# RishabhSri14/Human-Body-Reconstruction

Measured on NVIDIA B200. Metric: train_rays_per_sec, higher is better.
Workload: dtype bf16 MLP operands (f32 accumulate) / f32 encoder+compositor

## Files before the change

human_body_reconstruction_b200/_lib.py:

```python
from __future__ import annotations

import ctypes as C
import os
import subprocess
import sys
import threading

import torch

_HERE = os.path.dirname(os.path.abspath(__file__))
ROOT = os.path.dirname(_HERE)
CSRC = os.path.join(_HERE, "csrc")
SO_PATH = os.path.join(_HERE, "libhbr_b200.so")
INCLUDE = os.path.join(ROOT, "include")

NVCC_FLAGS = [
    "-gencode", "arch=compute_100a,code=sm_100a", "-O3", "-lineinfo", "-std=c++17",
    "--fmad=true",
    "-Xcompiler", "-fPIC", "-Xcompiler", "-O3", "-Xptxas", "-v",
]

HBR_MAX_LEVELS = 32
HBR_MAX_PEERS, HBR_PEER_MAX_CTAS, HBR_PEER_HANDLE_BYTES = 8, 128, 64
HBR_PEER_FLAG_BYTES = HBR_PEER_MAX_CTAS * HBR_MAX_PEERS * 4
# ... 48 lines not shown

def _build_locked(bdir: str, force: bool, verbose: bool) -> str:
    nvcc = os.environ.get("NVCC", "/usr/local/cuda/bin/nvcc")
    objs, procs = [], []
    for src in sources():
        obj = os.path.join(bdir, os.path.basename(src)[:-3] + ".o")
        objs.append(obj)
        if (not force) and os.path.exists(obj) and os.path.getmtime(obj) > max(os.path.getmtime(d) for d in _deps()):
            continue
        cmd = [nvcc, *NVCC_FLAGS, *os.environ.get("HBR_EXTRA_NVCC", "").split(), "-I", INCLUDE, "-c", src, "-o", obj]
        procs.append((src, subprocess.Popen(cmd, stdout=subprocess.PIPE, stderr=subprocess.STDOUT, text=True)))
    log = []
    for src, p in procs:
        out, _ = p.communicate()
        log.append(f"== {os.path.basename(src)}\n{out}")
        if p.returncode != 0:
            raise RuntimeError(f"nvcc failed for {src}:\n{out}")
    with open(os.path.join(bdir, "ptxas.log"), "a" if not force else "w") as f:
        f.write("\n".join(log))
    if verbose:
        print("\n".join(log))
    tmp_so = os.path.join(bdir, f"libhbr_b200.{os.getpid()}.so.tmp")
    cmd = [nvcc, "-shared", "-o", tmp_so, *objs, "-lcudart"]
    r = subprocess.run(cmd, stdout=subprocess.PIPE, stderr=subprocess.STDOUT, text=True)
    if r.returncode != 0:
        raise RuntimeError(f"link failed:\n{r.stdout}")
    os.replace(tmp_so, SO_PATH)
    return SO_PATH


def build_debug(force: bool = False) -> str:
    dbg = os.path.join(CSRC, "debug")
    srcs = sorted(os.path.join(dbg, f) for f in os.listdir(dbg) if f.endswith(".cu")) + [os.path.join(CSRC, "abi.cu")]
    deps = _deps() + [os.path.join(dbg, f) for f in os.listdir(dbg)]
    if not force and os.path.exists(DEBUG_SO_PATH) and os.path.getmtime(DEBUG_SO_PATH) > max(os.path.getmtime(d) for d in deps):
        return DEBUG_SO_PATH
    nvcc = os.environ.get("NVCC", "/usr/local/cuda/bin/nvcc")
    cmd = [nvcc, *[f for f in NVCC_FLAGS if f not in ("-Xptxas", "-v")], "-I", INCLUDE, "-shared", "-o", DEBUG_SO_PATH, *srcs,
           "-lcudart"]
    r = subprocess.run(cmd, stdout=subprocess.PIPE, stderr=subprocess.STDOUT, text=True)
    if r.returncode != 0:
        raise RuntimeError(f"nvcc failed for the debug library:\n{r.stdout}")
    return DEBUG_SO_PATH


_lib = None
_debug_lib = None
_lock = threading.Lock()

_i64, _i32, _f32, _vp = C.c_int64, C.c_int, C.c_float, C.c_void_p
_geom_p, _dims_p = C.POINTER(HashGeom), C.POINTER(MlpDims)

SIGNATURES = {
    "hbr_abi_version": ([], C.c_int),
    "hbr_last_error": ([], C.c_char_p),
    "hbr_mlp_param_count": ([_dims_p], _i64),
    "hbr_mlp_act_floats": ([], _i64),
    "hbr_hash_encode_fwd": ([_vp, _i32, _i64, _vp, _geom_p, _vp, _i64, _vp], C.c_int),
    "hbr_hash_encode_bwd": ([_vp, _i32, _i64, _vp, _i64, _geom_p, _vp, _i32, _i32, _vp], C.c_int),
    "hbr_hash_encode_dx": ([_vp, _i32, _i64, _vp, _geom_p, _vp, _i64, _vp, _vp], C.c_int),
    "hbr_hash_indices": ([_vp, _i32, _i64, _geom_p, _vp, _vp, _vp], C.c_int),
    "hbr_dir_encode": ([_vp, _i32, _i64, _i32, _i32, _vp, _vp], C.c_int),
    "hbr_mlp_fwd_f32": ([_vp, _i64, _vp, _i64, _i64, _vp, _dims_p, _vp, _vp, _vp], C.c_int),
    "hbr_mlp_bwd_f32": ([_vp, _i64, _vp, _i64, _i64, _vp, _dims_p, _vp, _vp, _vp, _vp, _i64, _vp, _vp, _vp], C.c_int),
    "hbr_mlp_tc_scratch_bytes": ([_dims_p], _i64),
    "hbr_mlp_fwd_tc": ([_vp, _i32, _i64, _vp, _i64, _i64, _vp, _dims_p, _i32, _vp, _vp, _i32, _vp, _vp, _vp], C.c_int),
    "hbr_mlp_bwd_tc": ([_vp, _i32, _i64, _vp, _i64, _i64, _vp, _dims_p, _i32, _vp, _vp, _vp, _i64, _vp, _vp, _f32, _vp, _i32, _i32,
                        _vp, _vp, _vp], C.c_int),
    "hbr_occupancy_update": ([_vp, _i64, _vp, _i64, _vp, _i32, C.POINTER(C.c_float), _f32, _vp, _vp], C.c_int),
    "hbr_compact_samples": ([_vp, _vp, _vp, _i64, _i64, _i64, _vp, _i32, C.POINTER(C.c_float), _f32, _vp, _vp, _vp, _vp, _vp],
                            C.c_int),
    "hbr_hash_encode_fwd_pts": ([_vp, _i64, _vp, _vp, _geom_p, _vp, _i64, _i32, _vp], C.c_int),
    "hbr_hash_encode_bwd_pts": ([_vp, _i64, _vp, _vp, _i64, _geom_p, _vp, _i32, _i32, _vp], C.c_int),
    "hbr_mlp_tc_prepare": ([_vp, _dims_p, _i32, _vp, _vp], C.c_int),
    "hbr_mlp_tc_reduce_grads": ([_dims_p, _i64, _vp, _vp, _vp], C.c_int),
    "hbr_strat_depths": ([_vp, _vp, _f32, _f32, _i64, _vp, _vp], C.c_int),
    "hbr_mse_pair_fwd": ([_vp, _vp, _vp, _i64, _f32, _vp, _vp], C.c_int),
    "hbr_mse_pair_bwd": ([_vp, _vp, _vp, _i64, _f32, _vp, _vp, _vp, _vp], C.c_int),
    "hbr_hash_encode_fwd_rays": ([_vp, _vp, _vp, _i64, _i64, _i64, _vp, _geom_p, _vp, _i64, _i32, _vp], C.c_int),
    "hbr_field_bwd_rays_tc": ([_vp, _vp, _vp, _vp, _i64, _i64, _i64, _geom_p, _vp, _vp, _dims_p, _i32, _vp, _vp, _vp, _vp, _vp, _f32,
                               _vp, _i32, _i32, _vp], C.c_int),
    "hbr_field_fwd_rays_tc": ([_vp, _vp, _vp, _i64, _i64, _i64, _vp, _geom_p, _vp, _vp, _dims_p, _i32, _vp, _vp, _vp, _i32, _vp],
                              C.c_int),
    "hbr_hash_encode_bwd_rays": ([_vp, _vp, _vp, _i64, _i64, _i64, _vp, _i64, _geom_p, _vp, _i32, _i32, _vp], C.c_int),
    "hbr_field_fwd_tc": ([_vp, _i64, _vp, _geom_p, _vp, _i64, _vp, _dims_p, _i32, _vp, _vp, _vp, _vp], C.c_int),
    "hbr_field_bwd_tc": ([_vp, _i64, _geom_p, _vp, _i64, _vp, _dims_p, _i32, _vp, _vp, _vp, _vp, _vp, _vp, _f32, _vp, _vp],
                         C.c_int),
    "hbr_adam_step": ([_vp, _vp, _vp, _vp, _i64, C.c_double, C.c_double, C.c_double, C.c_double, C.c_double, _i32, _i64,
                       C.c_double, _vp, _vp], C.c_int),
    "hbr_adam_tick": ([_vp, _vp, _vp], C.c_int),
    "hbr_adam_step_dev": ([_vp, _vp, _vp, _vp, _i64, _vp, C.c_double, C.c_double, C.c_double, C.c_double, _i32, _vp, C.c_double,
                           _vp, _vp, _vp], C.c_int),
    "hbr_ray_gen": ([_vp, _i64, _i32, _i32, _f32, _f32, _f32, _f32, _vp, _i64, _i64, _vp, _i32, _vp, _vp, _vp, _vp, _vp, _vp],
                    C.c_int),
    "hbr_ray_bbox": ([_vp, _i64, _i32, _i32, _f32, _f32, _f32, _f32, _f32, _f32, _vp, _vp], C.c_int),
    "hbr_peer_alloc": ([C.POINTER(_vp), _i64], C.c_int),
    "hbr_peer_free": ([_vp], C.c_int),
    "hbr_peer_export": ([_vp, C.POINTER(C.c_ubyte)], C.c_int),
    "hbr_peer_import": ([C.POINTER(C.c_ubyte), C.POINTER(_vp)], C.c_int),
    "hbr_peer_release": ([_vp], C.c_int),
    "hbr_allreduce_peer": ([C.POINTER(_vp), C.POINTER(_vp), _vp, _i32, _i32, _i64, _f32, _i32, _vp, _vp], C.c_int),
    "hbr_hash_bwd_stream_tiles": ([_i64], _i64),
    "hbr_hash_encode_bwd_stream": ([_vp, _i32, _i64, _vp, _i64, _geom_p, _vp, C.POINTER(C.c_int), _i32, _vp, _vp], C.c_int),
    "hbr_hash_encode_bwd_rays_stream": ([_vp, _vp, _vp, _i64, _i64, _i64, _vp, _i64, _geom_p, _vp, C.POINTER(C.c_int), _i32, _vp,
                                         _vp], C.c_int),
    "hbr_hash_bwd_lm_ctas": ([_i64], _i64),
    "hbr_hash_encode_bwd_lm": ([_vp, _i32, _i64, _vp, _geom_p, _vp, C.POINTER(C.c_int), _i32, _vp, _vp], C.c_int),
    "hbr_hash_encode_bwd_rays_lm": ([_vp, _vp, _vp, _i64, _i64, _i64, _vp, _geom_p, _vp, C.POINTER(C.c_int), _i32, _vp, _vp],
                                    C.c_int),
    "hbr_allreduce_peer_stream": ([C.POINTER(_vp), C.POINTER(_vp), _vp, _i32, _i32, _i32, C.POINTER(_i64), C.POINTER(_i64),
                                   C.POINTER(C.c_uint), C.POINTER(C.c_int), _vp, _f32, _i32, _vp, _vp], C.c_int),
    "hbr_ray_points": ([_vp, _vp, _vp, _i64, _i64, _i64, _vp, _vp], C.c_int),
    "hbr_occupancy_mask": ([_vp, _i64, _vp, _i32, C.POINTER(C.c_float), _f32, _vp, _vp], C.c_int),
    "hbr_composite_fwd": ([_vp, _i64, _vp, _i64, _vp, _i64, _vp, _f32, _vp, _vp, _i64, _i64, _vp, _vp, _f32, _vp], C.c_int),
    "hbr_composite_bwd": ([_vp, _i64, _vp, _i64, _vp, _i64, _vp, _f32, _vp, _vp, _i64, _i64, _vp, _vp, _i64, _vp, _i64, _f32, _vp],
                          C.c_int),
    "hbr_composite_maps_fwd": ([_vp, _i64, _vp, _i64, _vp, _i64, _vp, _f32, _vp, _vp, _i64, _i64, _vp, _vp, _vp, _vp, _f32, _vp],
                               C.c_int),
    "hbr_composite_maps_bwd": ([_vp, _i64, _vp, _i64, _vp, _i64, _vp, _f32, _vp, _vp, _i64, _i64, _vp, _vp, _vp, _vp, _i64, _vp,
                                _i64, _f32, _vp], C.c_int),
    "hbr_hier_sample": ([_vp, _vp, _vp, _vp, _i64, _i64, _i32, _vp, _vp], C.c_int),
    "hbr_composite_sdf_fwd": ([_vp, _i64, _vp, _i64, _i32, _vp, _i64, _i64, _vp, _vp, _vp], C.c_int),
    "hbr_composite_sdf_bwd": ([_vp, _i64, _vp, _i64, _i32, _vp, _i64, _i64, _vp, _vp, _vp, _i64, _vp, _i64, _vp, _vp], C.c_int),
    "hbr_sdf_stencil_points": ([_vp, _i64, _f32, C.POINTER(C.c_float), C.POINTER(C.c_float), _vp, _vp], C.c_int),
    "hbr_sdf_eikonal_fwd": ([_vp, _i64, _f32, _vp, _vp, _vp], C.c_int),
    "hbr_sdf_eikonal_bwd": ([_vp, _i64, _f32, _vp, _vp, _vp], C.c_int),
    "hbr_grid_points": ([C.POINTER(C.c_double), C.POINTER(C.c_double), _i32, _i64, _i64, _vp, _vp], C.c_int),
    "hbr_grid_density": ([C.POINTER(C.c_double), C.POINTER(C.c_double), _i32, _i64, _i64, _vp, _geom_p, _vp, _dims_p,
                          _vp, _vp, _vp, _vp, _i64, _i32, _vp], C.c_int),
    "hbr_mlp_density_tf32x3": ([_vp, _i64, _vp, _dims_p, _vp, _vp], C.c_int),
    "hbr_mc_count": ([_vp, _i32, _i32, _i32, _f32, _i32, _i32, _vp, _vp], C.c_int),
    "hbr_mc_emit": ([_vp, _i32, _i32, _i32, _f32, _i32, _i32, _vp, _vp, _i64, _vp, _i64, _vp, _vp], C.c_int),
    "hbr_grid_interp": ([_vp, _i32, _i32, _i32, _i32, _vp, _i64, _vp, _vp], C.c_int),
}

DEBUG_SIGNATURES = {
    "hbr_debug_umma": ([_i32, _i32, _vp, _vp, _vp, _i32, _i32, _vp], C.c_int),
    "hbr_debug_umma_bench": ([_i32, _i32, _i32, _i32, _i32, _vp, _vp], C.c_int),
    "hbr_debug_umma_chain_bench": ([_i32, _i32, _i32, _vp, _vp], C.c_int),
    "hbr_debug_mlp_trace": ([_vp, _vp, _i64, _i64, _vp, _vp, _vp, _vp], C.c_int),
    "hbr_debug_mlp_trace_bwd": ([_vp, _vp, _i64, _i64, _vp, _vp, _vp, _vp, _vp, _vp, _vp, _vp], C.c_int),
}


KERNELS_PER_CALL = {
    "hbr_hash_encode_fwd": 1, "hbr_hash_encode_bwd": 1, "hbr_hash_encode_dx": 1, "hbr_hash_encode_fwd_rays": 1, "hbr_hash_encode_bwd_rays": 1, "hbr_hash_indices": 1, "hbr_dir_encode": 1,
    "hbr_mlp_fwd_f32": 1, "hbr_mlp_bwd_f32": 2, "hbr_mlp_fwd_tc": 2, "hbr_mlp_bwd_tc": 3, "hbr_field_fwd_tc": 2, "hbr_field_bwd_tc": 3, "hbr_field_bwd_rays_tc": 3, "hbr_field_fwd_rays_tc": 1, "hbr_adam_step": 1, "hbr_adam_tick": 1, "hbr_adam_step_dev": 1, "hbr_allreduce_peer": 1, "hbr_allreduce_peer_stream": 1, "hbr_hash_encode_bwd_stream": 1, "hbr_hash_encode_bwd_rays_stream": 1, "hbr_hash_encode_bwd_lm": 1, "hbr_hash_encode_bwd_rays_lm": 1, "hbr_ray_gen": 1, "hbr_ray_bbox": 1, "hbr_ray_points": 1, "hbr_occupancy_mask": 1, "hbr_occupancy_update": 2, "hbr_compact_samples": 1, "hbr_hash_encode_fwd_pts": 1, "hbr_hash_encode_bwd_pts": 1,
    "hbr_composite_fwd": 1, "hbr_composite_bwd": 1, "hbr_composite_maps_fwd": 1, "hbr_composite_maps_bwd": 1, "hbr_strat_depths": 1, "hbr_mse_pair_fwd": 1, "hbr_mse_pair_bwd": 1, "hbr_mlp_tc_prepare": 1, "hbr_mlp_tc_reduce_grads": 1, "hbr_hier_sample": 1, "hbr_grid_points": 1,
    "hbr_composite_sdf_fwd": 1, "hbr_composite_sdf_bwd": 1, "hbr_sdf_stencil_points": 1, "hbr_sdf_eikonal_fwd": 1, "hbr_sdf_eikonal_bwd": 1,
    "hbr_grid_density": 3, "hbr_mlp_density_tf32x3": 1, "hbr_mc_count": 1, "hbr_mc_emit": 2, "hbr_grid_interp": 1,
}


class _Stats:

    def __init__(self):
        self.launches = 0
        self.calls = {}
        self.timing = False
        self.events = []
        self.graph_events = []

    def reset(self):
        self.launches = 0
        self.calls = {}
        self.events = []
        self.graph_events = []

    def graph_times(self):
        out = {}
        for name, a, b in self.graph_events:
            out.setdefault(name, []).append(a.elapsed_time(b))
        return out

    def summary(self):
        acc = {}
        for name, a, b in self.events:
            c, s = acc.get(name, (0, 0.0))
            acc[name] = (c + 1, s + a.elapsed_time(b))
        return {k: (c, s / c) for k, (c, s) in acc.items()}


STATS = _Stats()


class _Counted:
    __slots__ = ("fn", "name", "k")

    def __init__(self, fn, name):
        self.fn, self.name, self.k = fn, name, KERNELS_PER_CALL.get(name, 0)

    def __call__(self, *a):
        st = STATS
        st.launches += self.k
        st.calls[self.name] = st.calls.get(self.name, 0) + 1
        if st.timing and self.k:
            ext = torch.cuda.is_current_stream_capturing()
            e0 = torch.cuda.Event(enable_timing=True, external=ext)
            e1 = torch.cuda.Event(enable_timing=True, external=ext)
            s = torch.cuda.current_stream()
            e0.record(s)
            rc = self.fn(*a)
            e1.record(s)
            (st.graph_events if ext else st.events).append((self.name, e0, e1))
            return rc
        return self.fn(*a)


class _Lib:
    pass


def lib():
    global _lib
    if _lib is not None:
        return _lib
    with _lock:
        if _lib is None:
            if _stale():
                if os.environ.get("HBR_NO_BUILD") == "1":
                    raise RuntimeError("libhbr_b200.so is missing/stale and HBR_NO_BUILD=1")
                build()
            l = C.CDLL(SO_PATH)
            wrapped = _Lib()
            for name, (args, res) in SIGNATURES.items():
                fn = getattr(l, name)
                fn.argtypes = args
                fn.restype = res
                setattr(wrapped, name, _Counted(fn, name) if name in KERNELS_PER_CALL else fn)
            if l.hbr_abi_version() != HBR_ABI_VERSION:
# ... 42 lines not shown
```

human_body_reconstruction_b200/csrc/composite.cu:

```cuda
#include "common.cuh"
#include <math_constants.h>

namespace hbr {

constexpr int kRaysPerCta = 8;

__global__ void ray_points_kernel(const float* __restrict__ o, const float* __restrict__ d, const float* __restrict__ t,
                                  long long t_rs, long long R, long long S, float* __restrict__ pts) {
  const long long i = (long long)blockIdx.x * blockDim.x + threadIdx.x;
  if (i >= R * S) return;
  const long long r = i / S, s = i - r * S;
  const float tt = __ldg(t + r * t_rs + s);
#pragma unroll
  for (int k = 0; k < 3; ++k) pts[i * 3 + k] = __fadd_rn(__ldg(o + r * 3 + k), __fmul_rn(__ldg(d + r * 3 + k), tt));
}

struct Mu3 { float v[3]; };
__global__ void occupancy_kernel(const float* __restrict__ pts, long long n, const uint8_t* __restrict__ grid, int G,
                                 Mu3 mu, float sigma, uint8_t* __restrict__ mask) {
  const long long i = (long long)blockIdx.x * blockDim.x + threadIdx.x;
  if (i >= n) return;
  long long q[3];
#pragma unroll
  for (int k = 0; k < 3; ++k) {
    const float u = __fmul_rn(__fdiv_rn(__fsub_rn(__ldg(pts + i * 3 + k), mu.v[k]), sigma), (float)G);
    long long c = __float2ll_rz(u);
    if (c < 0) c += G;
    c = c < 0 ? 0 : (c >= G ? G - 1 : c);
    q[k] = c;
  }
  mask[i] = grid[(q[0] * G + q[1]) * G + q[2]] ? 1 : 0;
}

template <typename XT>
__global__ void dir_encode_kernel(const XT* __restrict__ d, long long n, int dim, int nf, float* __restrict__ out) {
  const long long i = (long long)blockIdx.x * blockDim.x + threadIdx.x;
  const long long total = n * dim * nf;
  if (i >= total) return;
  const int k = (int)(i % nf);
  const long long rc = i / nf;
  float s, c;
  if (sizeof(XT) == 2) {
    const float x = __half2float(reinterpret_cast<const __half*>(d)[rc]);
    const float two_x = __half2float(__float2half_rn(2.f * x));
    const float a = __half2float(__float2half_rn(two_x * (float)k));
    s = __half2float(__float2half_rn(sinf(a)));
    c = __half2float(__float2half_rn(cosf(a)));
  } else {
    const float x = reinterpret_cast<const float*>(d)[rc];
    const float a = __fmul_rn(__fmul_rn(2.f, x), (float)k);
    s = sinf(a);
    c = cosf(a);
  }
  float* o = out + rc * (2 * nf);
  o[k] = s;
  o[nf + k] = c;
}

struct SampleIn {
  float delta, sig, p;
  bool keep;
};

__device__ __forceinline__ long long sample_row(const int32_t* __restrict__ rowmap, long long gs, int s, int S) {
  return rowmap == nullptr ? gs : (s < S ? (long long)__ldg(rowmap + gs) : -1);
}

__device__ __forceinline__ SampleIn load_sample(const float* __restrict__ tr, const float* __restrict__ sigma,
                                                long long sig_st, const uint8_t* __restrict__ mask, long long gs,
                                                int s, int S, float dnr, bool& live, long long row) {
  SampleIn q;
  live = s < S && row >= 0 && (mask == nullptr || mask[gs]);
  float delta = 0.f;
  if (s + 1 < S) delta = __fsub_rn(__ldg(tr + s + 1), __ldg(tr + s));
  q.delta = __fmul_rn(delta, dnr);
  const float raw = live ? __ldg(sigma + row * sig_st) : 0.f;
  q.keep = !(raw < -10.f);
  q.sig = q.keep ? raw : -10.f;
  q.p = s < S ? __fmul_rn(q.sig, q.delta) : 0.f;
  return q;
}

template <bool MAPS>
__global__ void __launch_bounds__(kRaysPerCta * 32)
composite_fwd_kernel(const float* __restrict__ t, long long t_rs, const float* __restrict__ rgb, long long rgb_st,
                     const float* __restrict__ sigma, long long sig_st, const float* __restrict__ dn, float dn_scalar,
                     const uint8_t* __restrict__ mask, const int32_t* __restrict__ rowmap, long long R, int S,
                     float* __restrict__ C, float* __restrict__ w_out, float ert_tau, float* __restrict__ depth,
                     float* __restrict__ opac) {
  const int lane = threadIdx.x & 31;
  const long long ray = (long long)blockIdx.x * kRaysPerCta + (threadIdx.x >> 5);
  if (ray >= R) return;
  const float* tr = t + ray * t_rs;
  const float dnr = dn ? __ldg(dn + ray) : dn_scalar;
  float carry = 0.f, c0 = 0.f, c1 = 0.f, c2 = 0.f, dsum = 0.f, asum = 0.f;
  for (int s0 = 0; s0 < S; s0 += 32) {
    const int s = s0 + lane;
    const long long gs = ray * S + s;
    bool live;
    const long long row = sample_row(rowmap, gs, s, S);
    const SampleIn q = load_sample(tr, sigma, sig_st, mask, gs, s, S, dnr, live, row);
    const float incl = carry + warp_incl_scan(q.p, lane);
    float prev = __shfl_up_sync(kFull, incl, 1);
    if (lane == 0) prev = carry;
    const float T = s == 0 ? 1.f : expf(-prev);
    const float alpha = 1.f - expf(-q.p);
    const float w = s < S ? __fmul_rn(T, alpha) : 0.f;
    if (s < S) {
      if (w_out) w_out[gs] = w;
      if (MAPS) {
        dsum += w * __ldg(tr + s);
        asum += w;
      }
      if (live) {
        const float* c = rgb + row * rgb_st;
        c0 += w * __ldg(c + 0);
        c1 += w * __ldg(c + 1);
        c2 += w * __ldg(c + 2);
      }
    }
    carry = __shfl_sync(kFull, incl, 31);
    if (carry > ert_tau) {
      if (w_out)
        for (int s2 = s0 + 32 + lane; s2 < S; s2 += 32) w_out[ray * S + s2] = 0.f;
      break;
    }
  }
  c0 = warp_sum(c0); c1 = warp_sum(c1); c2 = warp_sum(c2);
  if (lane == 0) { C[ray * 3 + 0] = c0; C[ray * 3 + 1] = c1; C[ray * 3 + 2] = c2; }
  if (MAPS) {
    dsum = warp_sum(dsum); asum = warp_sum(asum);
    if (lane == 0) {
      if (depth) depth[ray] = dsum;
      if (opac) opac[ray] = asum;
    }
  }
}

template <int NCH, bool MAPS>
__global__ void __launch_bounds__(kRaysPerCta * 32)
composite_bwd_kernel(const float* __restrict__ t, long long t_rs, const float* __restrict__ rgb, long long rgb_st,
                     const float* __restrict__ sigma, long long sig_st, const float* __restrict__ dn, float dn_scalar,
                     const uint8_t* __restrict__ mask, const int32_t* __restrict__ rowmap, long long R, int S,
                     const float* __restrict__ gC, float* __restrict__ drgb, long long drgb_st, float* __restrict__ dsig,
                     long long dsig_st, float ert_tau, const float* __restrict__ gD, const float* __restrict__ gA) {
  const int lane = threadIdx.x & 31;
  const long long ray = (long long)blockIdx.x * kRaysPerCta + (threadIdx.x >> 5);
  if (ray >= R) return;
  const float* tr = t + ray * t_rs;
  const float dnr = dn ? __ldg(dn + ray) : dn_scalar;
  float g0 = 0.f, g1 = 0.f, g2 = 0.f, gd = 0.f, ga = 0.f;
  if (!MAPS || gC) { g0 = __ldg(gC + ray * 3 + 0); g1 = __ldg(gC + ray * 3 + 1); g2 = __ldg(gC + ray * 3 + 2); }
  if (MAPS) {
    if (gD) gd = __ldg(gD + ray);
    if (gA) ga = __ldg(gA + ray);
  }
  const bool packed = drgb_st == 4 && dsig_st == 4 && dsig == drgb + 3;

  float Tk[NCH], ek[NCH], ck[NCH], dk[NCH];
  float carry = 0.f;
  bool done = false;
#pragma unroll
  for (int i = 0; i < NCH; ++i) {
    const int s = i * 32 + lane;
    Tk[i] = 0.f; ek[i] = 1.f; ck[i] = 0.f; dk[i] = 0.f;
    if (i * 32 < S && !done) {
      const long long gs = ray * S + s;
      bool live;
      const long long row = sample_row(rowmap, gs, s, S);
      const SampleIn q = load_sample(tr, sigma, sig_st, mask, gs, s, S, dnr, live, row);
      const float incl = carry + warp_incl_scan(q.p, lane);
      float prev = __shfl_up_sync(kFull, incl, 1);
      if (lane == 0) prev = carry;
      carry = __shfl_sync(kFull, incl, 31);
      if (s < S) {
        Tk[i] = s == 0 ? 1.f : expf(-prev);
        ek[i] = expf(-q.p);
        if (live) {
          const float* c = rgb + row * rgb_st;
          ck[i] = g0 * __ldg(c + 0) + g1 * __ldg(c + 1) + g2 * __ldg(c + 2);
          dk[i] = q.keep ? q.delta : 0.f;
        }
        if (MAPS) ck[i] = __fadd_rn(__fmaf_rn(gd, __ldg(tr + s), ck[i]), ga);
      }
      done = carry > ert_tau;
    }
  }
  float rcarry = 0.f;
#pragma unroll
  for (int i = NCH - 1; i >= 0; --i) {
    if (i * 32 < S) {
      const int s = i * 32 + lane;
      const long long gs = ray * S + s;
      const float w = Tk[i] * (1.f - ek[i]);
      const float wc = w * ck[i];
      const float rin = warp_rincl_scan(wc, lane);
      float after = __shfl_down_sync(kFull, rin, 1);
      if (lane == 31) after = 0.f;
      const float suffix = rcarry + after;
      rcarry += __shfl_sync(kFull, rin, 0);
      if (s < S) {
        const long long row = sample_row(rowmap, gs, s, S);
        const bool live = row >= 0 && (mask == nullptr || mask[gs]);
        const float dp = Tk[i] * ek[i] * ck[i] - suffix;
        const float ds = live ? dk[i] * dp : 0.f;
        const float r0 = live ? w * g0 : 0.f, r1 = live ? w * g1 : 0.f, r2 = live ? w * g2 : 0.f;
        if (row >= 0) {
          if (packed) {
            *reinterpret_cast<float4*>(drgb + row * 4) = make_float4(r0, r1, r2, ds);
          } else {
            float* o = drgb + row * drgb_st;
            o[0] = r0; o[1] = r1; o[2] = r2;
            dsig[row * dsig_st] = ds;
          }
        }
      }
    }
  }
}

constexpr int kHierWarps = 4;

__global__ void __launch_bounds__(kHierWarps * 32)
hier_sample_kernel(float* __restrict__ w, const float* __restrict__ t, const float* __restrict__ u,
                   const float* __restrict__ cand, long long R, int S, int P2, int clamp_in_place,
                   float* __restrict__ t_fine) {
  extern __shared__ float sm[];
  const int warp = threadIdx.x >> 5, lane = threadIdx.x & 31;
  float* cdf = sm + (size_t)warp * (S + P2);
  float* arr = cdf + S;
  const long long ray = (long long)blockIdx.x * kHierWarps + warp;
  if (ray >= R) return;
  float* wr = w + ray * S;
  float part = 0.f;
  for (int s = lane; s < S; s += 32) {
    float v = wr[s];
    if (v < 0.f) { v = 0.f; if (clamp_in_place) wr[s] = 0.f; }
    v = __fadd_rn(v, 1e-5f);
    cdf[s] = v;
    part += v;
  }
  const float total = warp_sum(part);
  __syncwarp();
  for (int s = lane; s < S; s += 32) cdf[s] = __fdiv_rn(cdf[s], total);
  __syncwarp();
  if (lane == 0) {
    float acc = 0.f;
    for (int s = 0; s < S; ++s) { acc = __fadd_rn(acc, cdf[s]); cdf[s] = acc; }
  }
  __syncwarp();
  for (int s = lane; s < P2; s += 32) {
    float v = CUDART_INF_F;
    if (s < S) {
      v = __ldg(t + s);
    } else if (s < 2 * S) {
      const float uu = __ldg(u + ray * S + (s - S));
      int lo = 0, hi = S;
      while (lo < hi) {
        const int mid = (lo + hi) >> 1;
        if (cdf[mid] <= uu) lo = mid + 1; else hi = mid;
      }
      v = __ldg(cand + min(lo, S - 1));
    }
    arr[s] = v;
  }
  __syncwarp();
  for (int k = 2; k <= P2; k <<= 1) {
    for (int j = k >> 1; j > 0; j >>= 1) {
      for (int i = lane; i < P2; i += 32) {
        const int ixj = i ^ j;
        if (ixj > i) {
          const float a = arr[i], b = arr[ixj];
          const bool asc = (i & k) == 0;
          if ((a > b) == asc) { arr[i] = b; arr[ixj] = a; }
        }
      }
      __syncwarp();
    }
  }
  for (int s = lane; s < 2 * S; s += 32) t_fine[ray * 2 * S + s] = arr[s];
}

}

using namespace hbr;

extern "C" int hbr_ray_points(const float* o, const float* d, const float* t, int64_t t_rs, int64_t R, int64_t S,
                              float* pts, void* stream) {
  HBR_REQUIRE(R >= 0 && S >= 0, "negative size");
// ... 126 lines not shown
```

human_body_reconstruction_b200/csrc/debug/mlp_tc_debug.cu:

```cuda
#define HBR_DEBUG_ENTRY 1
#include "../mlp_layout.cuh"
#include "../tc_common.cuh"
#include "hbr_debug.h"

#define HBR_OP tc::OpBf16
#define HBR_OPNS bf16
#include "../mlp_tc_impl.cuh"
#undef HBR_OP
#undef HBR_OPNS
#define HBR_OP tc::OpF16
#define HBR_OPNS f16
#include "../mlp_tc_impl.cuh"
#undef HBR_OP
#undef HBR_OPNS

using namespace hbr;
using namespace hbr::bf16;

extern "C" int hbr_debug_umma(int mode, int operand, const float* A, const float* B, float* D, int N, int K, void* stream) {
  HBR_REQUIRE(mode >= 0 && mode <= 2, "mode %d", mode);
  HBR_REQUIRE(operand == HBR_BF16 || operand == HBR_F16, "operand %d", operand);
  HBR_REQUIRE(N % 16 == 0 && N >= 16 && N <= 64 && K % 16 == 0 && K >= 16 && K <= 128, "N=%d K=%d", N, K);
  HBR_REQUIRE(mode != 2 || K == 128, "mode 2 needs K=128");
  auto kern = operand == HBR_F16 ? f16::umma_debug_kernel : bf16::umma_debug_kernel;
  HBR_CUDA(cudaFuncSetAttribute(kern, cudaFuncAttributeMaxDynamicSharedMemorySize, 65536));
  kern<<<1, 128, 65536, as_stream(stream)>>>(mode, A, B, D, N, K);
  HBR_LAUNCH_CHECK();
  return HBR_OK;
}

extern "C" int hbr_debug_umma_bench(int M, int N, int reps, int nacc, int mn_major, long long* cycles, void* stream) {
  HBR_REQUIRE((M == 64 || M == 128) && N >= 8 && N <= 256 && N % 8 == 0 && nacc >= 1 && nacc * N <= 512 && reps >= 1,
              "bad shape");
  HBR_CUDA(cudaFuncSetAttribute(umma_bench_kernel, cudaFuncAttributeMaxDynamicSharedMemorySize, 65536));
  umma_bench_kernel<<<1, 128, 65536, as_stream(stream)>>>(M, N, reps, nacc, mn_major, cycles);
  HBR_LAUNCH_CHECK();
  return HBR_OK;
}

extern "C" int hbr_debug_umma_chain_bench(int kind, int reps, int nacc, long long* cycles, void* stream) {
  HBR_REQUIRE(kind >= 0 && kind <= 3 && reps >= 1 && nacc >= 1 && nacc <= 6, "bad arguments");
  HBR_CUDA(cudaFuncSetAttribute(umma_chain_bench_kernel, cudaFuncAttributeMaxDynamicSharedMemorySize, 98304));
  umma_chain_bench_kernel<<<1, 128, 98304, as_stream(stream)>>>(kind, reps, nacc, cycles);
  HBR_LAUNCH_CHECK();
  return HBR_OK;
}

extern "C" int hbr_debug_mlp_trace_bwd(const float* feat, const float* dirs, int64_t dir_group, int64_t n,
                                       const float* params, const float* out, const float* dout, float* dfeat,
                                       float* dparams, void* scratch, long long* trace, void* stream) {
  using SC = Scratch<32, 48>;
  constexpr int smem = BwdSmem<32, 48, 2>::total;
  HBR_CUDA(cudaFuncSetAttribute(mlp_bwd_tc_kernel<32, 48, 2, true>, cudaFuncAttributeMaxDynamicSharedMemorySize, smem));
  const int grid = (int)min64(ceil_div(ceil_div(n, kTile), 2), sm_count());
  uint8_t* sc = static_cast<uint8_t*>(scratch);
  if (sc != nullptr) mlp_prep_kernel<32, 48><<<kPrepCtas, 256, 0, as_stream(stream)>>>(params, 32, 24, sc);
  mlp_bwd_tc_kernel<32, 48, 2, true><<<grid, 2 * kTile + 32, smem, as_stream(stream)>>>(
      feat, 32, dirs, dir_group, n, params, 32, 24, out, dout, dfeat, 32, nullptr, dparams, sc,
      sc != nullptr ? reinterpret_cast<float*>(sc + SC::off_grad) : nullptr, trace, EncArgs{}, HashGeom{}, 1.f, 0, nullptr, nullptr);
  HBR_LAUNCH_CHECK();
  return HBR_OK;
}

extern "C" int hbr_debug_mlp_trace(const float* feat, const float* dirs, int64_t dir_group, int64_t n, const float* params,
                                   float* out, long long* trace, void* stream) {
  constexpr int smem = FwdSmem<32, 48, 4>::total;
  HBR_CUDA(cudaFuncSetAttribute(mlp_fwd_tc_kernel<32, 48, 4, true>, cudaFuncAttributeMaxDynamicSharedMemorySize, smem));
  const int grid = (int)min64(ceil_div(ceil_div(n, kTile), 4), sm_count());
  mlp_fwd_tc_kernel<32, 48, 4, true><<<grid, 4 * kTile, smem, as_stream(stream)>>>(
      feat, 32, dirs, dir_group, n, params, 32, 24, out, nullptr, trace, EncArgs{}, HashGeom{}, 0, nullptr, nullptr);
  HBR_LAUNCH_CHECK();
  return HBR_OK;
}
```

human_body_reconstruction_b200/csrc/mlp_tc.cu:

```cuda
#include "mlp_layout.cuh"
#include "tc_common.cuh"

#define HBR_OP tc::OpBf16
#define HBR_OPNS bf16
#include "mlp_tc_impl.cuh"
#undef HBR_OP
#undef HBR_OPNS
#define HBR_OP tc::OpF16
#define HBR_OPNS f16
#include "mlp_tc_impl.cuh"
#undef HBR_OP
#undef HBR_OPNS

using namespace hbr;
using bf16::narrow_shape;
using bf16::Scratch;
using tc::EncArgs;

static int check_operand(int operand, float grad_scale) {
  HBR_REQUIRE(operand == HBR_BF16 || operand == HBR_F16, "operand format %d (HBR_BF16 or HBR_F16)", operand);
  HBR_REQUIRE(grad_scale > 0.f && grad_scale < 3.0e38f, "grad_scale %g", (double)grad_scale);
  return HBR_OK;
}
#define HBR_BY_OPERAND(...) (operand == HBR_F16 ? f16::__VA_ARGS__ : bf16::__VA_ARGS__)
// ... 112 lines not shown
    return f16::launch_fwd_tc<32, 48, 4, true>(nullptr, 32, dirs, dir_group, n, params, 32, dims->d_view, out,
                                               static_cast<uint8_t*>(scratch), e, to_device_geom(*geom), 0, 0, nullptr, nullptr, as_stream(stream));
  }
  EncArgs e{};
  e.x = x; e.table = table; e.feat16 = static_cast<uint16_t*>(feat16);
  return bf16::launch_fwd_tc<32, 48, 4, true>(nullptr, 32, dirs, dir_group, n, params, 32, dims->d_view, out,
                                              static_cast<uint8_t*>(scratch), e, to_device_geom(*geom), 0, 0, nullptr, nullptr, as_stream(stream));
}

extern "C" int hbr_field_bwd_tc(const float* x, int64_t n, const hbr_hash_geom* geom, const float* dirs, int64_t dir_group,
                                const float* params, const hbr_mlp_dims* dims, int operand, const void* feat16,
                                const float* out, const float* dout, float* dtable, float* ddirs, float* dparams,
                                float grad_scale, void* scratch, void* stream) {
  if (int rc = check_field(geom, dims)) return rc;
  if (int rc = check_operand(operand, grad_scale)) return rc;
  if (n == 0) return HBR_OK;
  HBR_REQUIRE(x && dirs && params && feat16 && out && dout && dtable, "NULL pointer");
  HBR_REQUIRE(dir_group >= 1, "dir_group");
  HBR_REQUIRE((uintptr_t)out % 16 == 0 && (uintptr_t)dout % 16 == 0 && (uintptr_t)dtable % 16 == 0 &&
                  (uintptr_t)feat16 % 16 == 0 && (uintptr_t)scratch % 256 == 0, "alignment");
  uint16_t* f16p = const_cast<uint16_t*>(static_cast<const uint16_t*>(feat16));
  if (operand == HBR_F16) {
    EncArgs e{};
    e.x = x; e.dtable = dtable; e.feat16 = f16p;
    return f16::launch_bwd_tc<32, 48, 2, true>(nullptr, 32, dirs, dir_group, n, params, 32, dims->d_view, out, dout, nullptr, 32,
                                               ddirs, dparams, static_cast<uint8_t*>(scratch), e, to_device_geom(*geom),
                                               grad_scale, 0, 0, 0, nullptr, nullptr, as_stream(stream));
  }
  EncArgs e{};
  e.x = x; e.dtable = dtable; e.feat16 = f16p;
  return bf16::launch_bwd_tc<32, 48, 2, true>(nullptr, 32, dirs, dir_group, n, params, 32, dims->d_view, out, dout, nullptr, 32,
                                              ddirs, dparams, static_cast<uint8_t*>(scratch), e, to_device_geom(*geom),
                                              grad_scale, 0, 0, 0, nullptr, nullptr, as_stream(stream));
}

#ifndef HBR_FWD_GATHER_WARPS
#define HBR_FWD_GATHER_WARPS 8
#endif
extern "C" int hbr_field_fwd_rays_tc(const float* rays_o, const float* rays_d, const float* t, int64_t t_ray_stride, int64_t R,
                                     int64_t S, const float* table, const hbr_hash_geom* geom, const float* dirs,
                                     const float* params, const hbr_mlp_dims* dims, int operand, float* out, void* feat16,
                                     void* scratch, int image_ready, void* stream) {
  if (int rc = check_field(geom, dims)) return rc;
  if (int rc = check_operand(operand, 1.f)) return rc;
  HBR_REQUIRE(R >= 0 && S >= 1 && R < (1LL << 40) / S, "R=%lld S=%lld", (long long)R, (long long)S);
  HBR_REQUIRE(t_ray_stride == 0 || t_ray_stride >= S, "t_ray_stride %lld", (long long)t_ray_stride);
  HBR_REQUIRE(!image_ready || scratch != nullptr, "image_ready without scratch");
  const int64_t n = R * S;
  if (n == 0) return HBR_OK;
  HBR_REQUIRE(rays_o && rays_d && t && table && dirs && params && out && feat16, "NULL pointer");
  HBR_REQUIRE((uintptr_t)out % 16 == 0 && (uintptr_t)table % 16 == 0 && (uintptr_t)feat16 % 16 == 0 &&
                  (uintptr_t)scratch % 256 == 0, "alignment");
  EncArgs e{};
  e.table = table; e.feat16 = static_cast<uint16_t*>(feat16);
  e.ro = rays_o; e.rd = rays_d; e.rt = t; e.S = S; e.t_stride = t_ray_stride;
  const uint8_t* image = image_ready ? static_cast<const uint8_t*>(scratch) : nullptr;
  return HBR_BY_OPERAND(launch_fwd_gather_tc<HBR_FWD_GATHER_WARPS>(dirs, S, n, params, dims->d_view, out, image, e,
                                                                     to_device_geom(*geom), as_stream(stream)));
}

extern "C" int hbr_field_bwd_rays_tc(const void* feat16, const float* rays_o, const float* rays_d, const float* t,
                                     int64_t t_ray_stride, int64_t R, int64_t S, const hbr_hash_geom* geom, const float* dirs,
                                     const float* params, const hbr_mlp_dims* dims, int operand, const float* out,
                                     const float* dout, float* dtable, float* ddirs, float* dparams, float grad_scale,
                                     void* scratch, int image_ready, int defer_reduce, void* stream) {
  if (int rc = check_field(geom, dims)) return rc;
  if (int rc = check_operand(operand, grad_scale)) return rc;
  HBR_REQUIRE(!defer_reduce || (scratch != nullptr && dparams != nullptr), "defer_reduce needs scratch and dparams");
  HBR_REQUIRE(R >= 0 && S >= 1 && R < (1LL << 40) / S, "R=%lld S=%lld", (long long)R, (long long)S);
  HBR_REQUIRE(t_ray_stride == 0 || t_ray_stride >= S, "t_ray_stride %lld", (long long)t_ray_stride);
  const int64_t n = R * S;
  if (n == 0) return HBR_OK;
  HBR_REQUIRE(feat16 && rays_o && rays_d && t && dirs && params && out && dout && dtable, "NULL pointer");
  HBR_REQUIRE((uintptr_t)out % 16 == 0 && (uintptr_t)dout % 16 == 0 && (uintptr_t)dtable % 16 == 0 &&
                  (uintptr_t)feat16 % 16 == 0 && (uintptr_t)scratch % 256 == 0, "alignment");
  EncArgs e{};
  e.dtable = dtable; e.ro = rays_o; e.rd = rays_d; e.rt = t; e.S = S; e.t_stride = t_ray_stride;
  const float* feat = static_cast<const float*>(feat16);
  return HBR_BY_OPERAND(launch_bwd_tc<32, 48, 1, false, 11>(feat, 32, dirs, S, n, params, 32, dims->d_view, out, dout, nullptr, 32,
                                                            ddirs, dparams, static_cast<uint8_t*>(scratch), e,
                                                            to_device_geom(*geom), grad_scale, 1, image_ready, defer_reduce,
                                                            nullptr, nullptr, as_stream(stream)));
}
```

human_body_reconstruction_b200/csrc/mlp_tc_impl.cuh:

```cuda
#ifndef HBR_OP
#error "define HBR_OP (tc::OpBf16 | tc::OpF16) and HBR_OPNS before including mlp_tc_impl.cuh"
#endif

#ifndef HBR_RING_SLOTS
#define HBR_RING_SLOTS 2
#endif

namespace hbr {
namespace HBR_OPNS {
using namespace tc;
using OP = HBR_OP;


constexpr int kTile = 128;
constexpr int kLBO128 = kTile * 16;

template <int K0P, int KCP>
struct WOfs {
  static constexpr int w0 = 0;
  static constexpr int w1 = w0 + 64 * K0P * 2;
  static constexpr int w2 = w1 + 64 * 64 * 2;
  static constexpr int w3 = w2 + 16 * 64 * 2;
  static constexpr int w4 = w3 + 64 * KCP * 2;
  static constexpr int w5 = w4 + 64 * 64 * 2;
  static constexpr int total = w5 + 16 * 64 * 2;
};

struct BOfs {
  __host__ __device__ static constexpr int ofs(int i) {
    return i == 0 ? 0 : i == 1 ? 2048 : i == 2 ? 4096 : i == 3 ? 4608 : i == 4 ? 6656 : 8704;
  }
  static constexpr int total = 9216;
};

template <int K0P, int KCP>
__device__ __forceinline__ void stage_weights_bf16(const float* __restrict__ params, const MlpLayout& m, uint8_t* wsm,
                                                   uint8_t* bias_sm, uint8_t* ones16, float* bias_f32 = nullptr,
                                                   bool skip_weights = false, int tid = -1, int nthr = 0) {
  if (tid < 0) { tid = threadIdx.x; nthr = blockDim.x; }
  const int JP[6] = {64, 64, 16, 64, 64, 16};
  const int KP[6] = {K0P, 64, 64, KCP, 64, 64};
  const int wofs[6] = {WOfs<K0P, KCP>::w0, WOfs<K0P, KCP>::w1, WOfs<K0P, KCP>::w2, WOfs<K0P, KCP>::w3,
                       WOfs<K0P, KCP>::w4, WOfs<K0P, KCP>::w5};
  if (!skip_weights) {
    constexpr int kChunks = WOfs<K0P, KCP>::total / 16;
    const int cbeg[7] = {0, wofs[1] / 16, wofs[2] / 16, wofs[3] / 16, wofs[4] / 16, wofs[5] / 16, kChunks};
#pragma unroll 3
    for (int c = tid; c < kChunks; c += nthr) {
      int i = 0;
#pragma unroll
      for (int t = 1; t < 6; ++t) i += c >= cbeg[t] ? 1 : 0;
      const int J = m.J[i], K = m.K[i];
      const int jp = (i == 2 || i == 5) ? 16 : 64;
      const int e = c - cbeg[i];
      const int cg = e / jp, j = e - cg * jp;
      const float* src = params + m.W[i] + j * K + cg * 8;
      float v[8];
#pragma unroll
      for (int q = 0; q < 8; ++q) v[q] = (j < J && cg * 8 + q < K) ? __ldg(src + q) : 0.f;
      store_chunk<OP>(wsm + wofs[i], j, cg, jp, v);
    }
  }
#pragma unroll
  for (int i = 0; i < 6; ++i) {
    const int J = m.J[i];
    if (bias_f32 == nullptr && bias_sm == nullptr) continue;
    if (bias_f32 != nullptr) {
      for (int j = tid; j < 64; j += nthr) bias_f32[i * 64 + j] = j < J ? __ldg(params + m.b[i] + j) : 0.f;
      continue;
    }
    uint8_t* bt = bias_sm + BOfs::ofs(i);
    for (int e = tid; e < JP[i] * 2; e += nthr) {
      const int cg = e / JP[i], j = e - cg * JP[i];
      float v[8] = {0.f, 0.f, 0.f, 0.f, 0.f, 0.f, 0.f, 0.f};
      if (cg == 0 && j < J) {
        const float b = __ldg(params + m.b[i] + j);
        v[0] = OP::round(b);
        v[1] = b - v[0];
      }
      store_chunk<OP>(bt, j, cg, JP[i], v);
    }
  }
// ... 415 lines not shown
    float a0 = __fmul_rn(v[0][0], w[0]), a1 = __fmul_rn(v[0][1], w[0]);
#pragma unroll
    for (int c = 1; c < 8; ++c) {
      a0 = __fadd_rn(a0, __fmul_rn(v[c][0], w[c]));
      a1 = __fadd_rn(a1, __fmul_rn(v[c][1], w[c]));
    }
    packed[l] = OP::pack(a0, a1);
  }
#pragma unroll
  for (int cg = 0; cg < 4; ++cg) {
    const uint4 q = make_uint4(packed[4 * cg], packed[4 * cg + 1], packed[4 * cg + 2], packed[4 * cg + 3]);
    *reinterpret_cast<uint4*>(x0 + chunk_off(r, cg, kTile)) = q;
    if (gp < n) reinterpret_cast<uint4*>(e.feat16 + gp * 32)[cg] = q;
  }
}

__device__ __forceinline__ void load_feat16_row(const EncArgs& e, long long gp, long long n, int r, uint8_t* x0) {
#pragma unroll
  for (int cg = 0; cg < 4; ++cg) {
    const uint4 q = gp < n ? __ldg(reinterpret_cast<const uint4*>(e.feat16 + gp * 32) + cg) : make_uint4(0, 0, 0, 0);
    *reinterpret_cast<uint4*>(x0 + chunk_off(r, cg, kTile)) = q;
  }
}

__device__ __forceinline__ void scatter_row(const EncArgs& e, const HashGeom& g, const float pt[3], bool valid, int lane,
                                            const float* df) {
#pragma unroll 1
  for (int l = 0; l < 16; ++l) {
    const float s = g.scale[l];
    long long ix, iy, iz;
    float fx, fy, fz;
    cell_of(pt[0], g.mu[0], g.sigma, s, ix, fx);
    cell_of(pt[1], g.mu[1], g.sigma, s, iy, fy);
    cell_of(pt[2], g.mu[2], g.sigma, s, iz, fz);
    float w[8];
    corner_weights(fx, fy, fz, w);
    float g0 = 0.f, g1 = 0.f;
#pragma unroll
    for (int q = 0; q < 16; ++q)
      if (q == l) { g0 = df[2 * q]; g1 = df[2 * q + 1]; }
    float val[8][2];
#pragma unroll
    for (int c = 0; c < 8; ++c) { val[c][0] = w[c] * g0; val[c][1] = w[c] * g1; }
    const long long pix = __shfl_up_sync(kFull, ix, 1);
    const long long piy = __shfl_up_sync(kFull, iy, 1);
    const long long piz = __shfl_up_sync(kFull, iz, 1);
    const int pvalid = __shfl_up_sync(kFull, (int)valid, 1);
    const bool head = lane == 0 || !valid || !pvalid || pix != ix || piy != iy || piz != iz;
    const unsigned heads = __ballot_sync(kFull, head);
    if (heads != kFull) {
      const unsigned above = lane == 31 ? 0u : (heads & (0xfffffffeu << lane));
      const int end = above ? (__ffs(above) - 1) : 32;
      const int maxrun = __reduce_max_sync(kFull, head ? end - lane : 0);
      for (int d = 1; d < maxrun; d <<= 1) {
#pragma unroll
        for (int c = 0; c < 8; ++c)
#pragma unroll
          for (int f = 0; f < 2; ++f) {
            const float t = __shfl_down_sync(kFull, val[c][f], d);
            if (lane + d < end) val[c][f] += t;
          }
      }
    }
    if (head && valid) {
      uint32_t idx[8];
      corner_indices<true>(ix, iy, iz, g.T, idx);
      float* lvl = e.dtable + (size_t)l * g.T * 2;
      if (!(ix & 1)) {
#pragma unroll
        for (int c = 0; c < 8; c += 2) {
          const bool odd = idx[c] & 1;
          const float4 q = odd ? make_float4(val[c + 1][0], val[c + 1][1], val[c][0], val[c][1])
                               : make_float4(val[c][0], val[c][1], val[c + 1][0], val[c + 1][1]);
          atomicAdd(reinterpret_cast<float4*>(lvl) + (idx[c] >> 1), q);
        }
      } else {
#pragma unroll
        for (int c = 0; c < 8; ++c) atomicAdd(reinterpret_cast<float2*>(lvl) + idx[c], make_float2(val[c][0], val[c][1]));
      }
    }
  }
}

template <int K0P, int KCP, int G>
struct FwdSmem {
  static constexpr int off_bias = WOfs<K0P, KCP>::total;
  static constexpr int off_ones16 = off_bias + BOfs::total;
  static constexpr int off_buf = off_ones16 + kTile * 16 * 2;
  static constexpr int buf_bytes = kTile * 64 * 2;
  static constexpr int off_stage = off_buf + G * buf_bytes;
  static constexpr int stage_bytes = K0P == 32 ? kTile * K0P * 4 : 0;
  static constexpr int off_bar = off_stage + G * stage_bytes;
  static constexpr int off_xbar = off_bar + 2 * G * 8 + 16;
  static constexpr int total = off_xbar + 4 * G * 8;
  static_assert(total <= 232448, "shared memory budget exceeded");
};

__device__ __forceinline__ void cell_of_norm(float u0, float scale, long long& cell, float& frac) {
  const float u = __fmul_rn(u0, scale);
  cell = __float2ll_rz(u);
  frac = __fsub_rn(u, __ll2float_rn(cell));
}

template <int NLV>
__device__ __forceinline__ void gather_unit(const EncArgs& e, const HashGeom& g, long long n, long long tile, int slice, int lg,
                                            int lane, uint8_t* x0) {
  const int r = slice * 32 + lane;
  const long long gp = tile * kTile + r;
  float un[3] = {0.f, 0.f, 0.f};
  if (gp < n) {
    long long ray, smp;
    if (n <= 0xffffffffLL) {
      const unsigned q = (unsigned)gp / (unsigned)e.S;
      ray = q;
      smp = (long long)((unsigned)gp - q * (unsigned)e.S);
    } else {
      ray = gp / e.S;
      smp = gp - ray * e.S;
    }
    const float tt = __ldg(e.rt + ray * e.t_stride + smp);
#pragma unroll
    for (int a = 0; a < 3; ++a) {
      const float x = __fadd_rn(__ldg(e.ro + ray * 3 + a), __fmul_rn(__ldg(e.rd + ray * 3 + a), tt));
      un[a] = __fdiv_rn(__fsub_rn(x, g.mu[a]), g.sigma);
    }
  }
  float2 v[NLV][8];
  float fr[NLV][3];
#pragma unroll
  for (int q = 0; q < NLV; ++q) {
    const int l = lg * NLV + q;
    const float s = g.scale[l];
    long long ix, iy, iz;
    float fx, fy, fz;
    cell_of_norm(un[0], s, ix, fx);
    cell_of_norm(un[1], s, iy, fy);
    cell_of_norm(un[2], s, iz, fz);
    uint32_t idx[8];
    corner_indices<true>(ix, iy, iz, g.T, idx);
    const float2* lvl = reinterpret_cast<const float2*>(e.table) + (size_t)l * g.T;
#pragma unroll
    for (int c = 0; c < 8; ++c) v[q][c] = __ldg(lvl + idx[c]);
    fr[q][0] = fx; fr[q][1] = fy; fr[q][2] = fz;
  }
  uint32_t packed[NLV];
#pragma unroll
  for (int q = 0; q < NLV; ++q) {
    float w[8];
    corner_weights(fr[q][0], fr[q][1], fr[q][2], w);
    float a0 = __fmul_rn(v[q][0].x, w[0]), a1 = __fmul_rn(v[q][0].y, w[0]);
#pragma unroll
    for (int c = 1; c < 8; ++c) {
      a0 = __fadd_rn(a0, __fmul_rn(v[q][c].x, w[c]));
      a1 = __fadd_rn(a1, __fmul_rn(v[q][c].y, w[c]));
    }
    packed[q] = OP::pack(a0, a1);
  }
  if constexpr (NLV == 4) {
    const uint4 out4 = make_uint4(packed[0], packed[1], packed[2], packed[3]);
    *reinterpret_cast<uint4*>(x0 + chunk_off(r, lg, kTile)) = out4;
    if (gp < n) reinterpret_cast<uint4*>(e.feat16 + gp * 32)[lg] = out4;
  } else {
    const uint2 out2 = make_uint2(packed[0], packed[1]);
    *reinterpret_cast<uint2*>(x0 + chunk_off(r, lg >> 1, kTile) + (lg & 1) * 8) = out2;
    if (gp < n) reinterpret_cast<uint2*>(e.feat16 + gp * 32)[lg] = out2;
  }
}


template <int K0P, int NT = kTile>
__device__ __forceinline__ void stage_features_async(const float* __restrict__ feat, long long tile0, long long n, int gt,
                                                     uint8_t* stage) {
  constexpr int kQ = K0P / 4;
  const float4* src = reinterpret_cast<const float4*>(feat + tile0 * K0P);
#pragma unroll
  for (int it = 0; it < kTile * kQ / NT; ++it) {
    const int idx = it * NT + gt;
    const bool ok = tile0 + idx / kQ < n;
    cp_async16(stage + idx * 16, ok ? (const void*)(src + idx) : (const void*)feat, ok);
  }
  cp_async_commit();
}
template <int K0P, int NT = kTile>
__device__ __forceinline__ void convert_staged_features(const uint8_t* stage, int gt, uint8_t* x0) {
  constexpr int kQ = K0P / 4;
#pragma unroll
  for (int it = 0; it < kTile * kQ / NT; ++it) {
    const int idx = it * NT + gt, row = idx / kQ, c4 = idx % kQ;
    const float4 q = *reinterpret_cast<const float4*>(stage + idx * 16);
    uint2 o;
    o.x = OP::pack(q.x, q.y);
    o.y = OP::pack(q.z, q.w);
    *reinterpret_cast<uint2*>(x0 + chunk_off(row, c4 >> 1, kTile) + (c4 & 1) * 8) = o;
  }
}

template <int K0P, int NPART>
__device__ __forceinline__ void copy_feat16_async(const uint16_t* __restrict__ feat16, long long tile0, long long n, int r, int part,
                                                  uint8_t* dst_tile) {
  constexpr int kPer = K0P / 8 / NPART;
  const long long gp = tile0 + r;
  const bool ok = gp < n;
  const uint16_t* src = feat16 + (ok ? gp : 0) * K0P;
#pragma unroll
  for (int c = 0; c < kPer; ++c) {
    const int cg = part * kPer + c;
    cp_async16(dst_tile + chunk_off(r, cg, kTile), src + cg * 8, ok);
  }
  cp_async_commit();
}

template <int K0P, int KCP, int G, bool TRACE = false, bool ENC = false, int GATH = 0>
__global__ void __launch_bounds__(G * kTile + GATH * 32, 1)
mlp_fwd_tc_kernel(const float* __restrict__ feat, long long feat_stride, const float* __restrict__ dirs, long long dir_group,
                  long long n_arg, const float* __restrict__ params, int in0, int dv, float* __restrict__ out,
                  const uint8_t* __restrict__ image, long long* __restrict__ trace, const EncArgs enc,
                  const __grid_constant__ HashGeom geom, int feat16, const unsigned long long* __restrict__ n_dev,
                  const int32_t* __restrict__ dir_rows) {
  const long long n = n_dev != nullptr ? min(n_arg, (long long)__ldg(n_dev)) : n_arg;
  using SM = FwdSmem<K0P, KCP, G>;
  using WO = WOfs<K0P, KCP>;
  constexpr int kGrpCols = 96;
  constexpr int kCols = G * kGrpCols <= 128 ? 128 : (G * kGrpCols <= 256 ? 256 : 512);
  static_assert(G * kGrpCols <= 512, "TMEM budget exceeded");
  extern __shared__ __align__(128) uint8_t sm[];
  const MlpLayout m = make_layout(in0, dv);
  uint8_t* wsm = sm;
  uint64_t* bars = reinterpret_cast<uint64_t*>(sm + SM::off_bar);
  uint32_t* tslot = reinterpret_cast<uint32_t*>(bars + 2 * G);
  const int warp = __shfl_sync(kFull, (int)(threadIdx.x >> 5), 0), lane = threadIdx.x & 31;

  uint64_t* xfull = reinterpret_cast<uint64_t*>(sm + SM::off_xbar);
  uint64_t* xempty = xfull + 2 * G;
  constexpr int kXBuf = kTile * K0P * 2;
  static_assert(GATH == 0 || (K0P == 32 && !ENC && 2 * kXBuf <= SM::buf_bytes), "gather variant: 32 features, two buffers");
  if (warp == 0) tmem_alloc<kCols>(tslot);
  if (threadIdx.x == 32) {
    for (int g = 0; g < G; ++g) mbar_init(bars + G + g, 1);
    if (GATH > 0)
      for (int q = 0; q < 2 * G; ++q) {
        mbar_init(xfull + q, GATH * 32);
        mbar_init(xempty + q, 1);
      }
    fence_mbar_init();
  }
  if (GATH == 0) {
    if (image != nullptr) {
      copy_image_async(sm, image, SM::off_buf);
      cp_async_wait_all();
    } else {
      stage_weights_bf16<K0P, KCP>(params, m, wsm, sm + SM::off_bias, sm + SM::off_ones16);
    }
    fence_async_smem();
  }
  fence_before_sync();
  __syncthreads();
  fence_after_sync();
  const uint32_t tbase = *tslot;
  const long long ntiles = (n + kTile - 1) / kTile;
  const long long nslots = (long long)gridDim.x * G;

  constexpr int kNlv = GATH > 8 ? 2 : 4;
  constexpr int kUnits = 64 / kNlv;
  if (GATH > 0 && warp >= 4 * G) {
    if (GATH > 8) asm volatile("setmaxnreg.dec.sync.aligned.u32 %0;\n" ::"n"(56));
    const int gw = warp - 4 * G;
    uint32_t epar = 0;
#pragma unroll 1
    for (long long k = 0;; ++k) {
      bool any = false;
#pragma unroll 1
      for (int g = 0; g < G; ++g) {
        const long long tile = (long long)g * gridDim.x + blockIdx.x + k * nslots;
        if (tile >= ntiles) continue;
        any = true;
        const int slot = (int)(k & 1), q = 2 * g + slot;
        if (k >= 2) {
          mbar_wait(xempty + q, (epar >> q) & 1u);
          epar ^= 1u << q;
        }
        uint8_t* x0 = sm + SM::off_buf + g * SM::buf_bytes + slot * kXBuf;
#pragma unroll 1
        for (int u = gw; u < kUnits; u += GATH) gather_unit<kNlv>(enc, geom, n, tile, u & 3, u >> 2, lane, x0);
        fence_async_smem();
        mbar_arrive(xfull + q);
      }
      if (!any) break;
    }
  } else {
    if (GATH > 8) asm volatile("setmaxnreg.inc.sync.aligned.u32 %0;\n" ::"n"(128));
    if (GATH > 0) {
      if (image != nullptr) {
        for (int e = threadIdx.x; e < SM::off_buf / 16; e += G * kTile) cp_async16(sm + e * 16, image + e * 16, true);
        cp_async_commit();
        cp_async_wait_all();
      } else {
        stage_weights_bf16<K0P, KCP>(params, m, wsm, sm + SM::off_bias, sm + SM::off_ones16, nullptr, false, threadIdx.x,
                                     G * kTile);
      }
      fence_async_smem();
      asm volatile("bar.sync 7, %0;" ::"n"(G * kTile) : "memory");
    }
    const int g = warp >> 2;
    const int r = threadIdx.x & (kTile - 1);
    const bool issuer = (warp & 3) == 0;
    uint8_t* buf = sm + SM::off_buf + g * SM::buf_bytes;
    uint64_t* done = bars + G + g;
    const uint32_t tgrp = tbase + g * kGrpCols;
    const uint32_t taddr = tgrp + ((uint32_t)((warp & 3) * 32) << 16);
    const uint32_t taddr_a = taddr + 64;
    const uint32_t wa = a4_of(wsm), ba = a4_of(sm + SM::off_bias), o16a = a4_of(sm + SM::off_ones16), xa = a4_of(buf);
    uint32_t dphase = 0;
    const bool vec_ok = in0 == K0P && feat_stride == K0P && ((uintptr_t)feat & 15) == 0;
    int tgi = 0, tmi = 0;
    (void)tgi; (void)tmi;
    int tgk = 0;
    uint32_t xpar = 0;
    (void)tgk; (void)xpar;
    uint8_t* stage = sm + SM::off_stage + g * SM::stage_bytes;
    const bool f16in = !ENC && GATH == 0 && feat16 != 0;
    const uint16_t* featq = reinterpret_cast<const uint16_t*>(feat);
    const bool staged = !ENC && GATH == 0 && !f16in && vec_ok && SM::stage_bytes > 0;
    if (staged && (long long)g * gridDim.x + blockIdx.x < ntiles)
      stage_features_async<K0P>(feat, ((long long)g * gridDim.x + blockIdx.x) * kTile, n, r, stage);
    if (f16in && (long long)g * gridDim.x + blockIdx.x < ntiles)
      copy_feat16_async<K0P, 1>(featq, ((long long)g * gridDim.x + blockIdx.x) * kTile, n, r, 0, buf);
#define TR()                                                                                  \
  do {                                                                                        \
    if (TRACE && blockIdx.x == 0 && threadIdx.x == 0 && tgi < 1000) trace[tgi++] = clock64(); \
  } while (0)
#define HBR_LAYER(SMEM, BODY)                                                                           \
  do {                                                                                                  \
    TR();                                                                                               \
    if (SMEM) fence_async_smem();                                                                       \
    fence_before_sync();                                                                                \
    asm volatile("bar.sync %0, 128;" ::"r"(1 + g) : "memory");                                          \
    TR();                                                                                               \
    if (issuer) {                                                                                       \
      if (TRACE && g == 0 && blockIdx.x == 0 && lane == 0 && tmi < 500) trace[1024 + tmi++] = clock64(); \
      fence_after_sync();                                                                               \
      if (elect_one()) {                                                                                \
        BODY;                                                                                           \
        commit(done);                                                                                   \
      }                                                                                                 \
      __syncwarp();                                                                                     \
      if (TRACE && g == 0 && blockIdx.x == 0 && lane == 0 && tmi < 500) trace[1024 + tmi++] = clock64(); \
    }                                                                                                   \
    mbar_wait(done, dphase);                                                                            \
    dphase ^= 1;                                                                                        \
    fence_after_sync();                                                                                 \
    TR();                                                                                               \
  } while (0)
#define HBR_TS_LAYER(I, W, JP, KP)                                      \
  HBR_LAYER(false, {                                                    \
    issue_fwd(tgrp, o16a, ba + BOfs::ofs(I) / 16, JP, 16, false);       \
    issue_fwd_ts(tgrp, tgrp + 64, wa + WO::W / 16, JP, KP, true);       \
  })
    for (long long tile = (long long)g * gridDim.x + blockIdx.x; tile < ntiles; tile += nslots) {
      const long long gp = tile * kTile + r;
      const bool valid = gp < n;
      const long long dir_row = valid ? (dir_rows != nullptr ? (long long)__ldg(dir_rows + gp) : gp / dir_group) : 0;
      if (valid && lane == 0) prefetch_l1(dirs + dir_row * dv);
      TR();
      uint32_t xofs = 0;
      if (GATH > 0) {
        const int slot = tgk & 1;
        mbar_wait(xfull + 2 * g + slot, (xpar >> slot) & 1u);
        xpar ^= 1u << slot;
        xofs = slot * (kXBuf / 16);
      } else if (ENC) {
        encode_row(enc, geom, gp, n, r, buf);
      } else if (f16in) {
        cp_async_wait_all();
      } else if (staged) {
        cp_async_wait_all();
        TR();
        convert_staged_features<K0P>(stage, r, buf);
        TR();
        if (tile + nslots < ntiles) stage_features_async<K0P>(feat, (tile + nslots) * kTile, n, r, stage);
      } else {
        load_features<K0P>(feat, feat_stride, tile * kTile, n, in0, vec_ok, r, r, 0, buf);
      }
      HBR_LAYER(true, issue_layer(tgrp, xa + xofs, wa + WO::w0 / 16, o16a, ba + BOfs::ofs(0) / 16, 64, K0P));
      if (GATH > 0) {
        if (r == 0) mbar_arrive(xempty + 2 * g + (tgk & 1));
        ++tgk;
      }
      if (f16in && tile + nslots < ntiles) copy_feat16_async<K0P, 1>(featq, (tile + nslots) * kTile, n, r, 0, buf);
      relu_epilogue64_tmem(taddr, taddr_a);
      HBR_TS_LAYER(1, w1, 64, 64);
      relu_epilogue64_tmem(taddr, taddr_a);
      HBR_TS_LAYER(2, w2, 16, 64);
      float o16[16];
      tmem_ld<16>(taddr, o16);
      const float density = o16[0] > 0.f ? o16[0] : 0.01f * o16[0];
      {
        uint32_t p[KCP / 2];
#pragma unroll
        for (int q = 0; q < KCP / 2; ++q) {
          float e[2];
#pragma unroll
          for (int j = 0; j < 2; ++j) {
            const int k = 2 * q + j;
            float x = 0.f;
            if (k < kFeat) x = o16[1 + k];
            else if (k < kFeat + dv) x = valid ? __ldg(dirs + dir_row * dv + (k - kFeat)) : 0.f;
            e[j] = x;
          }
          p[q] = OP::pack(e[0], e[1]);
        }
        tmem_st16(taddr_a, p);
        if (KCP == 48) tmem_st8(taddr_a + 16, p + 16);
        else tmem_st16(taddr_a + 16, p + 16);
        tmem_st_wait();
      }
      HBR_TS_LAYER(3, w3, 64, KCP);
      relu_epilogue64_tmem(taddr, taddr_a);
      HBR_TS_LAYER(4, w4, 64, 64);
      relu_epilogue64_tmem(taddr, taddr_a);
      HBR_TS_LAYER(5, w5, 16, 64);
      float c16[16];
      tmem_ld<16>(taddr, c16);
      if (valid) {
        float4 o;
        o.x = elu1(c16[0]);
        o.y = elu1(c16[1]);
        o.z = elu1(c16[2]);
        o.w = density;
        *reinterpret_cast<float4*>(out + gp * 4) = o;
      }
    }
#undef HBR_TS_LAYER
#undef HBR_LAYER
  }
  fence_before_sync();
  __syncthreads();
  if (warp == 0) tmem_dealloc<kCols>(tbase);
}

constexpr int kCg = kTile * 16;

__device__ __forceinline__ void relu_bias_to_tmem64(uint32_t taddr, const float* bias, uint32_t taddr_a, uint4* o) {
  float v[64];
  tmem_ld<64>(taddr, v);
#pragma unroll
  for (int cg = 0; cg < 8; ++cg) {
    const float4 b0 = *reinterpret_cast<const float4*>(bias + cg * 8);
    const float4 b1 = *reinterpret_cast<const float4*>(bias + cg * 8 + 4);
    const float* p = v + cg * 8;
    o[cg].x = OP::pack_relu(p[0] + b0.x, p[1] + b0.y); o[cg].y = OP::pack_relu(p[2] + b0.z, p[3] + b0.w);
    o[cg].z = OP::pack_relu(p[4] + b1.x, p[5] + b1.y); o[cg].w = OP::pack_relu(p[6] + b1.z, p[7] + b1.w);
  }
  if (taddr_a != 0xffffffffu) {
    tmem_st16(taddr_a, reinterpret_cast<const uint32_t*>(o));
    tmem_st16(taddr_a + 16, reinterpret_cast<const uint32_t*>(o) + 16);
    tmem_st_wait();
  }
}

__device__ __forceinline__ void store_dz16_both(const float* dz16, int r, uint8_t* dzs, uint32_t taddr_a) {
  uint32_t p[8];
#pragma unroll
  for (int q = 0; q < 8; ++q) p[q] = OP::pack(dz16[2 * q], dz16[2 * q + 1]);
  *reinterpret_cast<uint4*>(dzs + chunk_off(r, 0, kTile)) = make_uint4(p[0], p[1], p[2], p[3]);
  *reinterpret_cast<uint4*>(dzs + chunk_off(r, 1, kTile)) = make_uint4(p[4], p[5], p[6], p[7]);
  tmem_st8(taddr_a, p);
  tmem_st_wait();
}

__device__ __forceinline__ void issue_dgrad_ts(uint32_t tmem_d, uint32_t tmem_a, uint32_t w4, int JP, int KP) {
  const uint32_t idesc = make_idesc<OP>(128, KP, false, true);
#pragma unroll
  for (int kk = 0; kk < JP / 16; ++kk) {
    const uint64_t b = desc64(w4 + kk * 16, 128, JP * 16);
    mma_f16_ts(tmem_d, tmem_a + kk * 8, b, idesc, kk > 0);
  }
}

template <int K0P, int KCP, int G>
struct BwdSmem {
  static constexpr bool kAliasDzs = KCP == 48;
  static constexpr int off_bias = WOfs<K0P, KCP>::total;
  static constexpr int off_grp = off_bias + 6 * 64 * 4;
  static constexpr int h2 = 0;
  static constexpr int c2 = h2 + 9 * kCg;
  static constexpr int x0 = c2 + 9 * kCg;
  static constexpr int h1 = x0 + kTile * K0P * 2 + kCg;
  static constexpr int c1 = h1 + 9 * kCg;
  static constexpr int cin = c1 + 9 * kCg;
  static constexpr int dzs = kAliasDzs ? cin + 5 * kCg : cin + kTile * KCP * 2;
  static constexpr int grp_bytes = dzs + 2 * kCg;
  static constexpr int ring_slot = kTile * 32 * 4;
  static constexpr int ring_slots = HBR_RING_SLOTS;
  static constexpr int off_ring = off_grp + G * grp_bytes;
  static constexpr int off_bar = off_ring + (G == 1 && K0P == 32 ? ring_slots * ring_slot : 0);
  static constexpr int off_pos = off_bar + (4 * G + 2 * ring_slots) * 8 + 16;
  static constexpr int total = off_pos + 2 * kTile * 3 * 4;
  static_assert(total <= 232448, "shared memory budget exceeded");
};

template <int K0P, int KCP, int WORK = 128>
struct BwdTmem {
  static constexpr bool kCinOne = KCP == 48;
  static constexpr int n0 = K0P + 8, n1 = 72, n3 = KCP + (kCinOne ? 0 : 8), n4 = 72;
  static constexpr int g0 = WORK;
  static constexpr int g1 = g0 + n0;
  static constexpr int g2 = g1 + n1;
  static constexpr int g3 = g2 + 16;
  static constexpr int g4 = g3 + n3;
  static constexpr int g5 = g4 + n4;
  static constexpr int end = g5 + 16;
  static_assert(end <= 512 && g4 + 80 <= 512, "TMEM budget exceeded");
};

template <int K0P, int KCP, int WORK>
__device__ __noinline__ void flush_gradients(uint32_t tbase, int warp, int lane, int ngroups, const MlpLayout& m,
                                             bool has_tiles, float* __restrict__ dparams, float* __restrict__ grad_rows, float ginv,
                                             int nthreads) {
  using TM = BwdTmem<K0P, KCP, WORK>;
  constexpr bool kCinOne = TM::kCinOne;
  if (dparams == nullptr) return;
  float* row = grad_rows != nullptr ? grad_rows + (size_t)blockIdx.x * Scratch<K0P, KCP>::kRowFloats : nullptr;
  if (!has_tiles) {
    if (row != nullptr)
      for (int e = threadIdx.x; e < m.total; e += nthreads) row[e] = 0.f;
    return;
  }
  if (warp >= 4 * ngroups) return;
  const int wq = warp & 3, unit = warp >> 2, units = ngroups;
  const uint32_t trow = tbase + ((uint32_t)(wq * 32) << 16);
  auto put = [&](int idx, float v) {
    if (row != nullptr) row[idx] = v * ginv;
    else atomicAdd(dparams + idx, v * ginv);
  };
  const int q = wq * 16 + lane;
#pragma unroll 1
  for (int t = 0; t < 4; ++t) {
    if ((t % units) != unit) continue;
    const int i = t < 2 ? t : t + 1;
    const int gcol = t == 0 ? TM::g0 : t == 1 ? TM::g1 : t == 2 ? TM::g3 : TM::g4;
    const int ncol = t == 0 ? TM::n0 : t == 1 ? TM::n1 : t == 2 ? TM::n3 : TM::n4;
    const int Ki = m.K[i], Ji = m.J[i], Wi = m.W[i], bi = m.b[i];
    const int bias_col = (i == 3 && kCinOne) ? Ki : (i == 0 ? K0P : (i == 3 ? KCP : 64));
    const bool mine = lane < 16 && q < Ji;
    const bool vec = row != nullptr && (Ki & 3) == 0 && (Wi & 3) == 0;
    const int base = Wi + q * Ki;
#pragma unroll 1
    for (int c = 0; c < ncol; c += 8) {
      float v[8];
      tmem_ld8_wait(trow + gcol + c, v);
      if (mine) {
        if (vec) {
          if (c < Ki) *reinterpret_cast<float4*>(row + base + c) = make_float4(v[0] * ginv, v[1] * ginv, v[2] * ginv, v[3] * ginv);
          if (c + 4 < Ki) *reinterpret_cast<float4*>(row + base + c + 4) = make_float4(v[4] * ginv, v[5] * ginv, v[6] * ginv, v[7] * ginv);
        } else {
#pragma unroll
          for (int j = 0; j < 8; ++j)
            if (c + j < Ki) put(base + c + j, v[j]);
        }
        if ((bias_col & ~7) == c) {
          float bv = v[0];
#pragma unroll
          for (int j = 1; j < 8; ++j)
            if ((bias_col & 7) == j) bv = v[j];
          put(bi + q, bv);
        }
      }
    }
  }
  const int r = wq * 32 + lane;
#pragma unroll 1
  for (int t = 0; t < 2; ++t) {
    if (((t + 2) % units) != unit) continue;
    const int i = t == 0 ? 2 : 5;
    const int Ji = m.J[i], Wi = m.W[i], bi = m.b[i];
    float gacc[16];
    tmem_ld<16>(trow + (t == 0 ? TM::g2 : TM::g5), gacc);
#pragma unroll
    for (int j = 0; j < 16; ++j) {
      if (j < Ji) {
        if (r < 64) put(Wi + j * 64 + r, gacc[j]);
        else if (r == 64) put(bi + j, gacc[j]);
      }
    }
  }
}

constexpr int kGroupRegs = 168;
__host__ __device__ constexpr int scat_regs(int G) { return G == 2 ? 88 : 112; }


template <int K0P, int KCP, int G, bool TRACE = false, bool ENC = false, int SCAT = 0>
__global__ void __launch_bounds__(G * kTile + SCAT * 32 + 32, 1)
mlp_bwd_tc_kernel(const float* __restrict__ feat, long long feat_stride, const float* __restrict__ dirs, long long dir_group,
                  long long n_arg, const float* __restrict__ params, int in0, int dv, const float* __restrict__ out,
                  const float* __restrict__ dout, float* __restrict__ dfeat, long long dfeat_stride,
                  float* __restrict__ ddirs, float* __restrict__ dparams, const uint8_t* __restrict__ image,
                  float* __restrict__ grad_rows, long long* __restrict__ trace, const EncArgs enc,
                  const __grid_constant__ HashGeom geom, float gscale, int feat16, const unsigned long long* __restrict__ n_dev,
                  const int32_t* __restrict__ dir_rows) {
  const long long n = n_dev != nullptr ? min(n_arg, (long long)__ldg(n_dev)) : n_arg;
  const float ginv = 1.f / gscale;
  using SM = BwdSmem<K0P, KCP, G>;
  using WO = WOfs<K0P, KCP>;
  constexpr int kGrpCols = 96;
  using TM = BwdTmem<K0P, KCP, 2 * kGrpCols>;
  constexpr bool kCinOne = TM::kCinOne;
  static_assert(G >= 1 && G <= 2, "two work accumulators");
  extern __shared__ __align__(128) uint8_t sm[];
  const MlpLayout m = make_layout(in0, dv);
  uint8_t* wsm = sm;
  float* bias = reinterpret_cast<float*>(sm + SM::off_bias);
  uint64_t* bars = reinterpret_cast<uint64_t*>(sm + SM::off_bar);
  constexpr int kSlots = SM::ring_slots;
  uint32_t* tslot = reinterpret_cast<uint32_t*>(bars + 4 * G + 2 * kSlots);
  uint64_t* dfull = bars + 4 * G;
  uint64_t* dempty = bars + 4 * G + kSlots;
  const int warp = __shfl_sync(kFull, (int)(threadIdx.x >> 5), 0), lane = threadIdx.x & 31;
  constexpr int kIssuerWarp = 4 * G + SCAT;
  if (TRACE && blockIdx.x == 0 && threadIdx.x == 0) trace[2000] = clock64();

  if (warp == 0) tmem_alloc<512>(tslot);
  if (threadIdx.x == 32) {
    for (int g = 0; g < G; ++g) {
      mbar_init(bars + G + g, 1);
      mbar_init(bars + 2 * G + g, 1);
      mbar_init(bars + 3 * G + g, 1);
    }
    for (int q = 0; q < kSlots; ++q) {
      mbar_init(dfull + q, kTile);
      mbar_init(dempty + q, SCAT > 0 ? SCAT * 32 : 1);
    }
    fence_mbar_init();
  }
  if (image != nullptr) {
    copy_image_async(wsm, image, WO::total);
    copy_image_async(sm + SM::off_bias, image + Scratch<K0P, KCP>::off_bias_f32, 6 * 64 * 4);
  } else {
    stage_weights_bf16<K0P, KCP>(params, m, wsm, nullptr, nullptr, bias);
  }
  {
    for (int e = threadIdx.x; e < G * SM::grp_bytes / 16; e += blockDim.x)
      reinterpret_cast<uint4*>(sm + SM::off_grp)[e] = make_uint4(0, 0, 0, 0);
    __syncthreads();
    const uint32_t one2 = OP::pack(1.f, 1.f);
    const uint4 ones4 = make_uint4(one2, one2, one2, one2);
    for (int e = threadIdx.x; e < kTile; e += blockDim.x) {
      for (int g = 0; g < G; ++g) {
        uint8_t* gb = sm + SM::off_grp + g * SM::grp_bytes;
        reinterpret_cast<uint4*>(gb + SM::h2 + 8 * kCg)[e] = ones4;
        reinterpret_cast<uint4*>(gb + SM::c2 + 8 * kCg)[e] = ones4;
        reinterpret_cast<uint4*>(gb + SM::x0 + kTile * K0P * 2)[e] = ones4;
        reinterpret_cast<uint4*>(gb + SM::h1 + 8 * kCg)[e] = ones4;
        reinterpret_cast<uint4*>(gb + SM::c1 + 8 * kCg)[e] = ones4;
      }
    }
  }
  cp_async_wait_all();
  fence_async_smem();
  fence_before_sync();
  __syncthreads();
  fence_after_sync();
  const uint32_t tbase = *tslot;
  if (TRACE && blockIdx.x == 0 && threadIdx.x == 0) trace[2001] = clock64();
  const long long ntiles = (n + kTile - 1) / kTile;
  const long long nslots = (long long)gridDim.x * G;
  long long nt[G];
  long long cta_tiles = 0;
#pragma unroll
  for (int g = 0; g < G; ++g) {
    nt[g] = tiles_of_slot(ntiles, (long long)g * gridDim.x + blockIdx.x, nslots);
    cta_tiles += nt[g];
  }
  const long long kmax = nt[0];

  auto wgrad_issuer = [&]() {
    const uint32_t tb0 = __shfl_sync(kFull, tbase, 0);
    const uint32_t sm0 = a4_of(sm);
    uint32_t par[G];
#pragma unroll
    for (int g = 0; g < G; ++g) par[g] = 0;
    bool first = true;
#define HBR_WGRAD_STAGE(BODY)                                              \
  _Pragma("unroll") for (int g = 0; g < G; ++g) {                          \
    if (k < nt[g]) {                                                       \
      mbar_wait(bars + 3 * G + g, par[g]);                                 \
// ... 171 lines not shown
    uint64_t* startb = bars + 3 * G + g;
    const bool issuer = (warp & 3) == 0;
    const uint32_t tgrp = tbase + g * kGrpCols, tgrp_a = tgrp + 64;
    const uint32_t taddr = tgrp + ((uint32_t)((warp & 3) * 32) << 16);
    const uint32_t taddr_a = taddr + 64;
    const uint32_t wa = a4_of(wsm), x0a = a4_of(x0);
    uint32_t dphase = 0, bphase = 0, ephase = 0;
    (void)ephase;
#define HBR_BSTAGE(BWD, BODY) HBR_BSTAGE_T(BODY, {})
#define HBR_BSTAGE_T(BODY, ...)                                            \
  do {                                                                     \
    HBR_STAMP(0);                                                          \
    fence_async_smem();                                                    \
    fence_before_sync();                                                   \
    asm volatile("bar.sync %0, 128;" ::"r"(1 + g) : "memory");             \
    if (issuer) {                                                          \
      fence_after_sync();                                                  \
      if (elect_one()) {                                                   \
        BODY;                                                              \
        commit(done);                                                      \
      }                                                                    \
      __syncwarp();                                                        \
    }                                                                      \
    __VA_ARGS__;                                                           \
    mbar_wait(done, dphase);                                               \
    dphase ^= 1;                                                           \
    fence_after_sync();                                                    \
    HBR_STAMP(1);                                                          \
  } while (0)
#define HBR_STAMP(j)                                                       \
  do {                                                                     \
    if (TRACE && blockIdx.x == 0 && threadIdx.x == 0 && tgi < 12) trace[tgi * 80 + stamp_i++] = clock64(); \
  } while (0)
#define HBR_BSTAGE_BWD(BODY, ...)                                          \
  do {                                                                     \
    HBR_STAMP(0);                                                          \
    fence_before_sync();                                                   \
    asm volatile("bar.sync %0, 128;" ::"r"(1 + g) : "memory");             \
    HBR_STAMP(1);                                                          \
    if (issuer) {                                                          \
      fence_after_sync();                                                  \
      if (elect_one()) {                                                   \
        BODY;                                                              \
        commit(done);                                                      \
      }                                                                    \
      __syncwarp();                                                        \
    }                                                                      \
    HBR_STAMP(2);                                                          \
    __VA_ARGS__;                                                           \
    HBR_STAMP(3);                                                          \
    fence_async_smem();                                                    \
    asm volatile("bar.sync %0, 128;" ::"r"(1 + g) : "memory");             \
    if (r == 0) mbar_arrive(startb);                                       \
    HBR_STAMP(4);                                                          \
    mbar_wait(done, dphase);                                               \
    dphase ^= 1;                                                           \
    fence_after_sync();                                                    \
    HBR_STAMP(5);                                                          \
  } while (0)
#define HBR_WAIT_B()           \
  do {                         \
    mbar_wait(doneb, bphase);  \
    bphase ^= 1;               \
  } while (0)
    const bool vec_ok = in0 == K0P && feat_stride == K0P && ((uintptr_t)feat & 15) == 0;
    const bool dvec_ok = dfeat != nullptr && in0 == K0P && dfeat_stride == K0P && ((uintptr_t)dfeat & 15) == 0 && K0P <= 32;
    const bool dlm = dfeat != nullptr && dfeat_stride == HBR_DFEAT_LEVEL_MAJOR && K0P <= 32;
    int tgi = 0;
    (void)tgi;
    constexpr bool kStage = K0P == 32 && !ENC;
    const bool f16in = !ENC && feat16 != 0;
    const uint16_t* featq = reinterpret_cast<const uint16_t*>(feat);
    const bool stage_ok = kStage && (vec_ok || f16in);
    bool staged = false;
    for (long long tile = (long long)g * gridDim.x + blockIdx.x; tile < ntiles; tile += nslots, ++tgi) {
      int stamp_i = 0;
      (void)stamp_i;
      HBR_STAMP(0);
      const long long gp = tile * kTile + r;
      const bool valid = gp < n;
      const long long dir_row = valid ? (dir_rows != nullptr ? (long long)__ldg(dir_rows + gp) : gp / dir_group) : 0;
      if (valid && lane == 0) prefetch_l1(dirs + dir_row * dv);
      float4 fo = make_float4(0.f, 0.f, 0.f, 0.f), go = fo;
      if (valid) {
        fo = __ldg(reinterpret_cast<const float4*>(out + gp * 4));
        go = __ldg(reinterpret_cast<const float4*>(dout + gp * 4));
        go.x *= gscale; go.y *= gscale; go.z *= gscale; go.w *= gscale;
      }
      float pt[3] = {0.f, 0.f, 0.f};
      if (ENC) {
        if (valid) { pt[0] = __ldg(enc.x + gp * 3 + 0); pt[1] = __ldg(enc.x + gp * 3 + 1); pt[2] = __ldg(enc.x + gp * 3 + 2); }
        load_feat16_row(enc, gp, n, r, x0);
      } else if (staged && f16in) {
        cp_async_wait_all();
#pragma unroll
        for (int cg = 0; cg < K0P / 8; ++cg) {
          const uint32_t o = chunk_off(r, cg, kTile);
          *reinterpret_cast<uint4*>(x0 + o) = *reinterpret_cast<const uint4*>(c2 + o);
        }
      } else if (f16in) {
        copy_feat16_async<K0P, 1>(featq, tile * kTile, n, r, 0, x0);
        cp_async_wait_all();
      } else if (staged) {
        cp_async_wait_all();
        convert_staged_features<K0P>(c2, r, x0);
      } else {
        load_features<K0P>(feat, feat_stride, tile * kTile, n, in0, vec_ok, r, r, 0, x0);
      }
      if ((tile + nslots) * kTile + r < n) {
        if (ENC) prefetch_l2(enc.feat16 + ((tile + nslots) * kTile + r) * 32);
        else if (!stage_ok && !f16in) prefetch_l2(feat + ((tile + nslots) * kTile + r) * feat_stride);
        if ((r & 7) == 0) {
          prefetch_l2(out + ((tile + nslots) * kTile + r) * 4);
          prefetch_l2(dout + ((tile + nslots) * kTile + r) * 4);
        }
      }
      uint4 dzt[8];
      HBR_BSTAGE(false, issue_fwd(tgrp, x0a, wa + WO::w0 / 16, 64, K0P));
      relu_bias_to_tmem64(taddr, bias + 0, taddr_a, dzt);
      HBR_BSTAGE_T(issue_fwd_ts(tgrp, tgrp_a, wa + WO::w1 / 16, 64, 64, false),
                   { store_tile64(r, h1, dzt); });
      relu_bias_to_tmem64(taddr, bias + 64, taddr_a, dzt);
      HBR_BSTAGE_T(issue_fwd_ts(tgrp, tgrp_a, wa + WO::w2 / 16, 16, 64, false),
                   {
                     if (SCAT > 0 && G == 2 && tgi > 0) {
                       mbar_wait(dempty + g, ephase & 1u);
                       ephase ^= 1u;
                     }
                     store_tile64(r, h2, dzt);
                   });
      {
        float o16[16];
        tmem_ld<16>(taddr, o16);
#pragma unroll
        for (int k = 0; k < 16; ++k) o16[k] += bias[128 + k];
        build_cin<KCP, kCinOne>(o16, dirs, dir_row, dv, valid, r, cin);
        uint32_t p[KCP / 2];
#pragma unroll
        for (int cg = 0; cg < KCP / 8; ++cg) {
          const uint4 q = *reinterpret_cast<const uint4*>(cin + chunk_off(r, cg, kTile));
          p[4 * cg] = q.x; p[4 * cg + 1] = q.y; p[4 * cg + 2] = q.z; p[4 * cg + 3] = q.w;
        }
        tmem_st16(taddr_a, p);
        if (KCP == 48) tmem_st8(taddr_a + 16, p + 16);
        else tmem_st16(taddr_a + 16, p + 16);
        tmem_st_wait();
      }
      HBR_BSTAGE(false, issue_fwd_ts(tgrp, tgrp_a, wa + WO::w3 / 16, 64, KCP, false));
      relu_bias_to_tmem64(taddr, bias + 192, taddr_a, dzt);
      HBR_BSTAGE_T(issue_fwd_ts(tgrp, tgrp_a, wa + WO::w4 / 16, 64, 64, false),
                   { store_tile64(r, c1, dzt); });
      relu_bias_to_tmem64(taddr, bias + 256, 0xffffffffu, dzt);
      {
        float dz16[16];
#pragma unroll
        for (int c = 0; c < 16; ++c) dz16[c] = 0.f;
        dz16[0] = go.x * (fo.x > 0.f ? 1.f : fo.x + 1.f);
        dz16[1] = go.y * (fo.y > 0.f ? 1.f : fo.y + 1.f);
        dz16[2] = go.z * (fo.z > 0.f ? 1.f : fo.z + 1.f);
        store_dz16_both(dz16, r, dzs, taddr_a);
      }
      HBR_BSTAGE_BWD(issue_dgrad_ts(tgrp, tgrp_a, wa + WO::w5 / 16, 16, 64),
                     { store_tile64(r, c2, dzt); });
      masked_dz_to_tmem64(taddr, r, c2, taddr_a, dzt);
      HBR_BSTAGE_BWD(issue_dgrad_ts(tgrp, tgrp_a, wa + WO::w4 / 16, 64, 64),
                     { HBR_WAIT_B(); store_tile64(r, c2, dzt); });
      masked_dz_to_tmem64(taddr, r, c1, taddr_a, dzt);
      staged = stage_ok && tile + nslots < ntiles;
      HBR_BSTAGE_BWD(issue_dgrad_ts(tgrp, tgrp_a, wa + WO::w3 / 16, 64, KCP), {
        HBR_WAIT_B();
        store_tile64(r, c1, dzt);
        if (staged && f16in) copy_feat16_async<K0P, 1>(featq, (tile + nslots) * kTile, n, r, 0, c2);
        else if (staged) stage_features_async<K0P>(feat, (tile + nslots) * kTile, n, r, c2);
      });
      float dd[KCP - kFeat];
      uint32_t dzp[8];
      {
        float dc[KCP], dz16[16];
        tmem_ld<KCP>(taddr, dc);
        dz16[0] = go.w * (fo.w > 0.f ? 1.f : 0.01f);
#pragma unroll
        for (int k = 0; k < kFeat; ++k) dz16[1 + k] = dc[k];
#pragma unroll
        for (int k = kFeat; k < KCP; ++k) dd[k - kFeat] = dc[k] * ginv;
#pragma unroll
        for (int q = 0; q < 8; ++q) dzp[q] = OP::pack(dz16[2 * q], dz16[2 * q + 1]);
        tmem_st8(taddr_a, dzp);
        tmem_st_wait();
      }
      HBR_BSTAGE_BWD(issue_dgrad_ts(tgrp, tgrp_a, wa + WO::w2 / 16, 16, 64), {
        HBR_WAIT_B();
        *reinterpret_cast<uint4*>(dzs + chunk_off(r, 0, kTile)) = make_uint4(dzp[0], dzp[1], dzp[2], dzp[3]);
        *reinterpret_cast<uint4*>(dzs + chunk_off(r, 1, kTile)) = make_uint4(dzp[4], dzp[5], dzp[6], dzp[7]);
        if (ddirs != nullptr) {
          const long long row0 = __shfl_sync(kFull, dir_row, 0);
          const bool uniform = __all_sync(kFull, dir_row == row0 && valid);
          _Pragma("unroll") for (int k = kFeat; k < KCP; ++k) {
            if (k < kFeat + dv) {
              if (uniform) {
                const float sdd = warp_sum(dd[k - kFeat]);
                if (lane == 0) atomicAdd(ddirs + row0 * dv + (k - kFeat), sdd);
              } else if (valid) {
                atomicAdd(ddirs + dir_row * dv + (k - kFeat), dd[k - kFeat]);
              }
            }
          }
        }
      });
      masked_dz_to_tmem64(taddr, r, h2, taddr_a, dzt);
      HBR_BSTAGE_BWD(issue_dgrad_ts(tgrp, tgrp_a, wa + WO::w1 / 16, 64, 64),
                     { HBR_WAIT_B(); store_tile64(r, h2, dzt); });
      masked_dz_to_tmem64(taddr, r, h1, taddr_a, dzt);
      HBR_BSTAGE_BWD(issue_dgrad_ts(tgrp, tgrp_a, wa + WO::w0 / 16, 64, K0P),
                     { HBR_WAIT_B(); store_tile64(r, h1, dzt); });
      if (SCAT > 0) {
        float df[K0P];
        tmem_ld<K0P>(taddr, df);
        const int slot = G == 2 ? g : (tgi % kSlots);
        if (G == 1 && tgi >= kSlots) {
          mbar_wait(dempty + slot, (ephase >> slot) & 1u);
          ephase ^= 1u << slot;
        }
        float2* stg = reinterpret_cast<float2*>(G == 2 ? h2 : sm + SM::off_ring + slot * SM::ring_slot);
#pragma unroll
        for (int l = 0; l < K0P / 2; ++l) stg[l * kTile + r] = make_float2(df[2 * l] * ginv, df[2 * l + 1] * ginv);
        mbar_arrive(dfull + slot);
      } else if (ENC) {
        float df[K0P];
        tmem_ld<K0P>(taddr, df);
#pragma unroll
        for (int k = 0; k < K0P; ++k) df[k] *= ginv;
        scatter_row(enc, geom, pt, valid, lane, df);
      } else if (dfeat != nullptr) {
        float df[K0P];
        tmem_ld<K0P>(taddr, df);
#pragma unroll
        for (int k = 0; k < K0P; ++k) df[k] *= ginv;
        if (dlm) {
          float2* stg = reinterpret_cast<float2*>(h2);
#pragma unroll
          for (int l = 0; l < K0P / 2; ++l) stg[l * kTile + r] = make_float2(df[2 * l], df[2 * l + 1]);
          asm volatile("bar.sync %0, 128;" ::"r"(1 + g) : "memory");
          const float4* s4 = reinterpret_cast<const float4*>(h2);
#pragma unroll
          for (int it = 0; it < K0P / 4; ++it) {
            const int idx = it * kTile + r, l = idx >> 6, j = idx & 63;
            if (tile * kTile + 2 * j < n)
              reinterpret_cast<float4*>(dfeat + ((size_t)l * n + tile * kTile) * 2)[j] = s4[idx];
          }
        } else if (dvec_ok) {
          constexpr int kQ = K0P / 4;
          float4* stg = reinterpret_cast<float4*>(h2);
#pragma unroll
          for (int c = 0; c < kQ; ++c)
            stg[r * kQ + (c ^ (r & 7))] = make_float4(df[4 * c], df[4 * c + 1], df[4 * c + 2], df[4 * c + 3]);
          asm volatile("bar.sync %0, 128;" ::"r"(1 + g) : "memory");
          float4* dst = reinterpret_cast<float4*>(dfeat + tile * kTile * K0P);
#pragma unroll
          for (int it = 0; it < kQ; ++it) {
            const int idx = it * kTile + r, row = idx / kQ, c = idx % kQ;
            if (tile * kTile + row < n) dst[idx] = stg[row * kQ + (c ^ (row & 7))];
          }
        } else if (valid) {
#pragma unroll
          for (int k = 0; k < K0P; ++k)
            if (k < in0) dfeat[gp * dfeat_stride + k] = df[k];
        }
      }
      HBR_STAMP(0);
      HBR_WAIT_B();
      HBR_STAMP(0);
    }
    if (TRACE && blockIdx.x == 0 && threadIdx.x == 0) trace[2004] = clock64();
  }
  fence_before_sync();
  __syncthreads();
  fence_after_sync();
  if (TRACE && blockIdx.x == 0 && threadIdx.x == 0) trace[2002] = clock64();

  if (warp < 4 * G) flush_gradients<K0P, KCP, 2 * kGrpCols>(tbase, warp, lane, G, m, cta_tiles > 0, dparams, grad_rows, ginv, 4 * G * 32);
  fence_before_sync();
  __syncthreads();
  if (TRACE && blockIdx.x == 0 && threadIdx.x == 0) trace[2003] = clock64();
  if (warp == 0) tmem_dealloc<512>(tbase);
}

static inline bool narrow_shape(const hbr_mlp_dims* d) { return d->in0 <= 32 && d->d_view + kFeat <= 40; }

template <int K0P, int KCP, int G, bool ENC>
static int launch_fwd_tc(const float* feat, int64_t feat_stride, const float* dirs, int64_t dir_group, int64_t n,
                         const float* params, int in0, int dv, float* out, uint8_t* scratch, const EncArgs& enc,
                         const HashGeom& geom, int feat16, int image_ready, const unsigned long long* n_dev, const int32_t* dir_rows,
                         cudaStream_t st) {
  constexpr int smem = FwdSmem<K0P, KCP, G>::total;
  const int grid = (int)min64(ceil_div(ceil_div(n, kTile), G), sm_count());
  if (scratch != nullptr && !image_ready) mlp_prep_kernel<K0P, KCP><<<kPrepCtas, 256, 0, st>>>(params, in0, dv, scratch);
  auto kern = mlp_fwd_tc_kernel<K0P, KCP, G, false, ENC>;
  HBR_CUDA(cudaFuncSetAttribute(kern, cudaFuncAttributeMaxDynamicSharedMemorySize, smem));
  kern<<<grid, G * kTile, smem, st>>>(feat, feat_stride, dirs, dir_group, n, params, in0, dv, out, scratch, nullptr, enc,
                                             geom, feat16, n_dev, dir_rows);
  HBR_LAUNCH_CHECK();
  return HBR_OK;
}

template <int GATH>
static int launch_fwd_gather_tc(const float* dirs, int64_t dir_group, int64_t n, const float* params, int dv, float* out,
                                const uint8_t* image, const EncArgs& enc, const HashGeom& geom, cudaStream_t st) {
  constexpr int G = 2;
  constexpr int smem = FwdSmem<32, 48, G>::total;
  const int grid = (int)min64(ceil_div(ceil_div(n, kTile), G), sm_count());
  auto kern = mlp_fwd_tc_kernel<32, 48, G, false, false, GATH>;
  HBR_CUDA(cudaFuncSetAttribute(kern, cudaFuncAttributeMaxDynamicSharedMemorySize, smem));
  kern<<<grid, G * kTile + GATH * 32, smem, st>>>(nullptr, 32, dirs, dir_group, n, params, 32, dv, out, image, nullptr, enc, geom,
                                                  1, nullptr, nullptr);
  HBR_LAUNCH_CHECK();
  return HBR_OK;
}

template <int K0P, int KCP, int G, bool ENC, int SCAT = 0>
static int launch_bwd_tc(const float* feat, int64_t feat_stride, const float* dirs, int64_t dir_group, int64_t n,
                         const float* params, int in0, int dv, const float* out, const float* dout, float* dfeat,
                         int64_t dfeat_stride, float* ddirs, float* dparams, uint8_t* scratch, const EncArgs& enc,
                         const HashGeom& geom, float gscale, int feat16, int image_ready, int defer_reduce,
                         const unsigned long long* n_dev, const int32_t* dir_rows, cudaStream_t st) {
  using SC = Scratch<K0P, KCP>;
  constexpr int smem = BwdSmem<K0P, KCP, G>::total;
  const int grid = (int)min64(ceil_div(ceil_div(n, kTile), G), sm_count());
  const bool rows = scratch != nullptr && dparams != nullptr && grid <= SC::kMaxRows;
  if (scratch != nullptr && !image_ready) mlp_prep_kernel<K0P, KCP><<<kPrepCtas, 256, 0, st>>>(params, in0, dv, scratch);
  auto kern = mlp_bwd_tc_kernel<K0P, KCP, G, false, ENC, SCAT>;
  HBR_CUDA(cudaFuncSetAttribute(kern, cudaFuncAttributeMaxDynamicSharedMemorySize, smem));
  if constexpr (SCAT > 0) {
    static_assert((G == 2 && SCAT == 7) || (G == 1 && SCAT == 11), "register budget: 16 warps, 4 per sub-partition");
    constexpr int kScatRegs = scat_regs(G);
    static int regs = 0;
    if (regs == 0) {
      cudaFuncAttributes fa;
      HBR_CUDA(cudaFuncGetAttributes(&fa, kern));
      regs = fa.numRegs;
    }
    HBR_REQUIRE(regs >= kScatRegs && regs <= kGroupRegs && 4 * regs <= 512 && G * kGroupRegs + (4 - G) * kScatRegs <= 4 * regs,
                "fused backward kernel compiled with %d registers per thread: the setmaxnreg budget does not hold", regs);
  }
  kern<<<grid, G * kTile + SCAT * 32 + 32, smem, st>>>(feat, feat_stride, dirs, dir_group, n, params, in0, dv, out, dout, dfeat,
                                           dfeat_stride, ddirs, dparams, scratch,
                                           rows ? reinterpret_cast<float*>(scratch + SC::off_grad) : nullptr, nullptr, enc, geom, gscale, feat16, n_dev, dir_rows);
  if (rows && !defer_reduce) {
    const int total = make_layout(in0, dv).total;
    mlp_grad_reduce_kernel<<<dim3((total + 255) / 256, kReduceSlices), 256, 0, st>>>(
        reinterpret_cast<const float*>(scratch + SC::off_grad), grid, SC::kRowFloats, total, dparams);
  }
  HBR_LAUNCH_CHECK();
  return HBR_OK;
}

template <int K0P, int KCP, int G>
static int reduce_grads_tc(int64_t n, int in0, int dv, uint8_t* scratch, float* dparams, cudaStream_t st) {
  using SC = Scratch<K0P, KCP>;
  const int grid = (int)min64(ceil_div(ceil_div(n, kTile), G), sm_count());
  HBR_REQUIRE(grid <= SC::kMaxRows, "grid %d exceeds the gradient rows", grid);
  const int total = make_layout(in0, dv).total;
  mlp_grad_reduce_kernel<<<dim3((total + 255) / 256, kReduceSlices), 256, 0, st>>>(
      reinterpret_cast<const float*>(scratch + SC::off_grad), grid, SC::kRowFloats, total, dparams);
  HBR_LAUNCH_CHECK();
  return HBR_OK;
}
template <int K0P, int KCP>
static int prepare_tc(const float* params, int in0, int dv, uint8_t* scratch, cudaStream_t st) {
  mlp_prep_kernel<K0P, KCP><<<kPrepCtas, 256, 0, st>>>(params, in0, dv, scratch);
  HBR_LAUNCH_CHECK();
  return HBR_OK;
}


}
}
```

human_body_reconstruction_b200/ops.py:

```python
from __future__ import annotations

import ctypes as C
from typing import Optional, Sequence

import torch

from . import _lib
HAS_TC = True

from ._lib import HBR_BF16, HBR_F16, HBR_F32, HashGeom, MlpDims, check, lib, ptr, require_cuda, stream


def make_geom(mu, sigma, scales: Sequence[float], L: int, F: int, T: int, E: int = 0) -> HashGeom:
    g = HashGeom()
    for i in range(3):
        g.mu[i] = float(mu[i])
    g.sigma = float(sigma)
    g.L, g.F, g.E, g.T = int(L), int(F), int(E), int(T)
    for i in range(L):
        g.scale[i] = float(scales[i])
    return g


def _xdtype(x: torch.Tensor) -> int:
# ... 632 lines not shown


def mlp_tc_reduce_grads(dims: MlpDims, n: int, dparams, device):
    check(lib().hbr_mlp_tc_reduce_grads(C.byref(dims), int(n), ptr(mlp_tc_scratch(dims, device)), ptr(dparams), stream()))


def mlp_bwd_tc(feat, dirs, dir_group, params, dims: MlpDims, out, dout, want_dfeat, want_ddirs, dparams,
               operand: int = HBR_BF16, grad_scale: float = 1.0, defer_reduce: bool = False, n_dev=None, dir_rows=None,
               level_major: bool = False):
    n = feat.shape[0]
    if level_major and want_dfeat:
        dfeat = torch.empty((dims.in0 // 2, n, 2), device=feat.device, dtype=torch.float32)
    else:
        level_major = False
        dfeat = torch.empty((n, dims.in0), device=feat.device, dtype=torch.float32) if want_dfeat else None
    ddirs = torch.zeros_like(dirs) if want_ddirs else None
    scratch = mlp_tc_scratch(dims, feat.device)
    key = _image_key(params, operand)
    ready = 1 if _tc_image.get(id(scratch)) == key else 0
    check(lib().hbr_mlp_bwd_tc(ptr(feat), _feat_dtype(feat, operand), feat.stride(0), ptr(dirs), dir_group, n, ptr(params),
                               C.byref(dims), operand, ptr(out), ptr(dout), ptr(dfeat),
                               _lib.HBR_DFEAT_LEVEL_MAJOR if level_major else dims.in0, ptr(ddirs), ptr(dparams),
                               float(grad_scale), ptr(scratch), ready, 1 if defer_reduce else 0, ptr(n_dev), ptr(dir_rows),
                               stream()))
    _lib.STATS.launches -= ready + (1 if defer_reduce else 0)
    _tc_image[id(scratch)] = key
    return dfeat, ddirs


def mlp_level_major_ok(geom: HashGeom, dims: MlpDims, n_points: int) -> bool:
    return geom.F == 2 and geom.L == 16 and geom.E == 0 and dims.in0 == 32 and n_points % 2 == 0 and n_points > 0


def field_fwd_tc(x, table, geom: HashGeom, dirs, dir_group, params, dims: MlpDims, operand: int = HBR_BF16):
    require_cuda(x, table, dirs, params)
    n = x.shape[0]
    out = torch.empty((n, 4), device=x.device, dtype=torch.float32)
    feat16 = torch.empty((n, 32), device=x.device, dtype=_operand_torch_dtype(operand))
    check(lib().hbr_field_fwd_tc(ptr(x), n, ptr(table), C.byref(geom), ptr(dirs), dir_group, ptr(params), C.byref(dims),
                                 operand, ptr(out), ptr(feat16), ptr(mlp_tc_scratch(dims, x.device)), stream()))
    return out, feat16


def field_fwd_rays_tc(rays_o, rays_d, t, table, geom: HashGeom, dirs, params, dims: MlpDims, operand: int = HBR_BF16):
    require_cuda(rays_o, rays_d, t, table, dirs, params)
    R, S = rays_o.shape[0], t.shape[-1]
    n = R * S
    out = torch.empty((n, 4), device=table.device, dtype=torch.float32)
    feat16 = torch.empty((n, 32), device=table.device, dtype=_operand_torch_dtype(operand))
    scratch = mlp_tc_scratch(dims, table.device)
    ready = 1 if _tc_image.get(id(scratch)) == _image_key(params, operand) else 0
    check(lib().hbr_field_fwd_rays_tc(ptr(rays_o), ptr(rays_d), ptr(t), _t_stride(t, S), R, S, ptr(table), C.byref(geom),
                                      ptr(dirs), ptr(params), C.byref(dims), operand, ptr(out), ptr(feat16), ptr(scratch), ready,
                                      stream()))
    return out, feat16


def field_bwd_tc(x, geom: HashGeom, dirs, dir_group, params, dims: MlpDims, feat16, out, dout, dtable, want_ddirs, dparams,
                 operand: int = HBR_BF16, grad_scale: float = 1.0):
    ddirs = torch.zeros_like(dirs) if want_ddirs else None
    check(lib().hbr_field_bwd_tc(ptr(x), x.shape[0], C.byref(geom), ptr(dirs), dir_group, ptr(params), C.byref(dims),
                                 operand, ptr(feat16), ptr(out), ptr(dout), ptr(dtable), ptr(ddirs), ptr(dparams),
                                 float(grad_scale), ptr(mlp_tc_scratch(dims, x.device)), stream()))
    return ddirs


def field_bwd_rays_tc(feat16, rays_o, rays_d, t, geom: HashGeom, dirs, params, dims: MlpDims, out, dout, dtable, want_ddirs,
                      dparams, operand: int = HBR_BF16, grad_scale: float = 1.0, defer_reduce: bool = False):
    require_cuda(feat16, rays_o, rays_d, t, dirs, params, out, dout, dtable)
    R, S = rays_o.shape[0], t.shape[-1]
    ddirs = torch.zeros_like(dirs) if want_ddirs else None
    scratch = mlp_tc_scratch(dims, feat16.device)
    key = _image_key(params, operand)
    ready = 1 if _tc_image.get(id(scratch)) == key else 0
    check(lib().hbr_field_bwd_rays_tc(ptr(feat16), ptr(rays_o), ptr(rays_d), ptr(t), _t_stride(t, S), R, S, C.byref(geom),
                                      ptr(dirs), ptr(params), C.byref(dims), operand, ptr(out), ptr(dout), ptr(dtable),
                                      ptr(ddirs), ptr(dparams), float(grad_scale), ptr(scratch), ready,
                                      1 if defer_reduce else 0, stream()))
    _lib.STATS.launches -= ready + (1 if defer_reduce else 0)
    _tc_image[id(scratch)] = key
    return ddirs


def field_scatter_supported(geom: HashGeom, dims: MlpDims) -> bool:
    T = int(geom.T)
    return (geom.F == 2 and geom.L == 16 and geom.E == 0 and T >= 2 and (T & (T - 1)) == 0 and dims.in0 == 32
            and dims.d_view + 15 <= 40)


def debug_umma(mode: int, A: torch.Tensor, B: torch.Tensor, M: int, N: int, K: int, operand: int = HBR_BF16) -> torch.Tensor:
    D = torch.empty((M, N), device=A.device, dtype=torch.float32)
    dl = _lib.debug_lib()
    rc = dl.hbr_debug_umma(mode, operand, ptr(A.contiguous()), ptr(B.contiguous()), ptr(D), N, K, stream())
    if rc != 0:
        raise RuntimeError(f"libhbr_b200_debug: {dl.cdll.hbr_last_error().decode()} (status {rc})")
    return D


def grid_points(min_bound, max_bound, res: int, p0: int, count: int, device) -> torch.Tensor:
    mn = (C.c_double * 3)(*[float(v) for v in min_bound])
    mx = (C.c_double * 3)(*[float(v) for v in max_bound])
    pts = torch.empty((count, 3), device=device, dtype=torch.float16)
    with torch.cuda.device(pts.device):
        check(lib().hbr_grid_points(mn, mx, res, p0, count, ptr(pts), stream()))
    return pts


def mlp_density_tf32x3(feat, params, dims: MlpDims):
    require_cuda(feat, params)
    feat = _f32c(feat)
    out = torch.empty((feat.shape[0],), device=feat.device, dtype=torch.float32)
    check(lib().hbr_mlp_density_tf32x3(ptr(feat), feat.shape[0], ptr(params), C.byref(dims), ptr(out), stream()))
    return out


def grid_density(min_bound, max_bound, res, p0, count, table, geom, params, dims, dir_enc, chunk=1 << 19, cuda_core_mlp=False):
    require_cuda(table, params)
    mn = (C.c_double * 3)(*[float(v) for v in min_bound])
    mx = (C.c_double * 3)(*[float(v) for v in max_bound])
    chunk = max(1, min(chunk, count))
    dev = table.device
    out = torch.empty((count, 4) if dir_enc is not None else (count,), device=dev, dtype=torch.float32)
    pts = torch.empty((chunk, 3), device=dev, dtype=torch.float16)
    feat = torch.empty((chunk, dims.in0), device=dev, dtype=torch.float32)
    check(lib().hbr_grid_density(mn, mx, res, p0, count, ptr(table), C.byref(geom), ptr(params), C.byref(dims),
                                 ptr(dir_enc), ptr(out), ptr(pts), ptr(feat), chunk, 1 if cuda_core_mlp else 0, stream()))
    return out


def mc_count(density: torch.Tensor, iso: float, i_begin: int = 0, i_end: Optional[int] = None):
    require_cuda(density)
    density = _f32c(density)
    n0, n1, n2 = density.shape
    i_end = n0 if i_end is None else i_end
    counts = torch.zeros(2, device=density.device, dtype=torch.int64)
    check(lib().hbr_mc_count(ptr(density), n0, n1, n2, float(iso), i_begin, i_end, ptr(counts), stream()))
    return counts


def mc_emit(density: torch.Tensor, iso: float, n_verts: int, n_faces: int):
    require_cuda(density)
    density = _f32c(density)
    n0, n1, n2 = density.shape
    dev = density.device
    edge_id = torch.empty((3, n0, n1, n2), device=dev, dtype=torch.int32)
    verts = torch.empty((max(n_verts, 1), 3), device=dev, dtype=torch.float32)
    faces = torch.empty((max(n_faces, 1), 3), device=dev, dtype=torch.int32)
    cursors = torch.zeros(2, device=dev, dtype=torch.int64)
    check(lib().hbr_mc_emit(ptr(density), n0, n1, n2, float(iso), 0, n0, ptr(edge_id), ptr(verts), n_verts, ptr(faces),
                            n_faces, ptr(cursors), stream()))
    return verts[:n_verts], faces[:n_faces], cursors


def grid_interp(vol: torch.Tensor, pts: torch.Tensor) -> torch.Tensor:
    require_cuda(vol, pts)
    vol, pts = _f32c(vol), _f32c(pts)
    C_, n0, n1, n2 = vol.shape
    n = pts.shape[0]
    out = torch.empty((n, C_), device=vol.device, dtype=torch.float32)
    check(lib().hbr_grid_interp(ptr(vol), C_, n0, n1, n2, ptr(pts), n, ptr(out), stream()))
    return out
```

human_body_reconstruction_b200/vol_renderer.py:

```python
from __future__ import annotations

import os
from collections import namedtuple
from typing import Optional, Tuple

import torch
import torch.nn as nn

from . import ops
from .encoder import PositionalEncoder
from .hash_encoding import HashEncoder
from .helper import calc_color, hierarchical_sampling, strat_sampler
from .test_hash import MLP_3D


class _FieldFn(torch.autograd.Function):

    @staticmethod
    def forward(ctx, pts, dirs, dir_group, enc, mlp, *params):
        geom, dims = enc._geom(), mlp._dims()
        dirs = dirs.float().contiguous()
        operand = ops.tc_operand()
        out, feat16 = ops.field_fwd_tc(pts, enc._flat_table(), geom, dirs, dir_group, mlp._flat_params(), dims, operand)
        ctx.enc, ctx.mlp, ctx.geom, ctx.dims, ctx.dir_group, ctx.operand = enc, mlp, geom, dims, dir_group, operand
# ... 69 lines not shown
        enc, mlp = ctx.enc, ctx.mlp
        L, T, F = enc.L, enc.T, enc.F
        flat = mlp._flat_params()
        dpm = mlp._dp if ctx.want_mlp else None
        if dpm is not None:
            dflat, last_m = dpm.enter_backward(mlp)
        else:
            dflat, last_m = torch.zeros_like(flat), False
        if (FUSE_SCATTER and ctx.want_tab and ctx.want_mlp and enc._dp is None and dpm is None
                and feat16.shape[0] <= FUSE_SCATTER_MAX_POINTS and ops.field_scatter_supported(ctx.geom, ctx.dims)):
            if ctx.g is not None:
                g, ev = ctx.g
                ctx.g = None
                torch.cuda.current_stream().wait_event(ev)
            else:
                g = torch.zeros((L, T, F), device=dout.device, dtype=torch.float32)
            ddirs = ops.field_bwd_rays_tc(feat16, rays_o, rays_d, t, ctx.geom, dirs, flat, ctx.dims, out.detach(),
                                          dout.float().contiguous(), g, ctx.needs_input_grad[3], dflat, operand=ctx.operand,
                                          grad_scale=mlp.tc_grad_scale, defer_reduce=False)
            return (None, None, None, ddirs, None, None) + tuple(g[i] for i in range(L)) + tuple(mlp._grad_views(dflat))
        defer = ctx.want_tab
        n_pts = feat16.shape[0]
        dpe = enc._dp if ctx.want_tab else None
        plan, lm = None, False
        if dpe is not None:
            g, last = dpe.enter_backward(enc)
            plan = dpe.stream_plan(enc, L, n_pts) if last else None
            lm = plan is not None and STREAM_LEVEL_MAJOR and ops.mlp_level_major_ok(ctx.geom, ctx.dims, n_pts)
        dfeat, ddirs = ops.mlp_bwd_tc(feat16, dirs, ctx.S, flat, ctx.dims, out.detach(), dout.float().contiguous(), ctx.want_tab,
                                      ctx.needs_input_grad[3], dflat, operand=ctx.operand, grad_scale=mlp.tc_grad_scale,
                                      defer_reduce=defer, level_major=lm)
        cur, side = torch.cuda.current_stream(), _side_stream(dout.device)
        if defer:
            side.wait_stream(cur)
            with torch.cuda.stream(side):
                ops.mlp_tc_reduce_grads(ctx.dims, feat16.shape[0], dflat, dout.device)
            dflat.record_stream(side)

        def join_mlp():
            if defer:
                cur.wait_stream(side)
            if dpm is not None and last_m:
                dpm.publish(mlp, dflat)

        gm = (None,) * len(mlp._ordered()) if (dpm is not None or not ctx.want_mlp) else tuple(mlp._grad_views(dflat))
        if not ctx.want_tab:
            join_mlp()
            return (None, None, None, ddirs, None, None) + (None,) * L + gm
        if dpe is not None:
            if plan is not None:
                ev_pre = cur.record_event()
                if lm:
                    ops.hash_encode_bwd_rays_lm(rays_o, rays_d, t, dfeat, ctx.geom, g, plan, dpe.done)
                    need = ops.hash_bwd_lm_ctas(n_pts)
                else:
                    ops.hash_encode_bwd_rays_stream(rays_o, rays_d, t, dfeat, ctx.geom, g, plan, dpe.done)
                    need = ops.hash_bwd_stream_tiles(n_pts)
                with_mlp = dpm is dpe and last_m
                ev_mlp = side.record_event() if (defer and with_mlp) else None
                dpe.exchange_streamed(plan, need, after=(ev_pre, ev_mlp), include_mlp=with_mlp)
                if defer:
                    cur.wait_stream(side)
                if dpm is not None and last_m and not with_mlp:
                    dpm.publish(mlp, dflat)
                return (None, None, None, ddirs, None, None) + (None,) * L + gm
            for l0, l1 in (dpe.level_chunks(enc, L, feat16.shape[0]) if last else [(0, L)]):
                ops.hash_encode_bwd_rays(rays_o, rays_d, t, dfeat, ctx.geom, g, l0, l1)
                if l0 == 0:
                    join_mlp()
                if last:
                    dpe.publish(enc, g[l0:l1])
            return (None, None, None, ddirs, None, None) + (None,) * L + gm
        if ctx.g is not None:
            g, ev = ctx.g
            ctx.g = None
            torch.cuda.current_stream().wait_event(ev)
        else:
            g = torch.zeros((L, T, F), device=dout.device, dtype=torch.float32)
        ops.hash_encode_bwd_rays(rays_o, rays_d, t, dfeat, ctx.geom, g, 0, L)
        join_mlp()
        return (None, None, None, ddirs, None, None) + tuple(g[i] for i in range(L)) + gm


class _FieldCompactFn(torch.autograd.Function):

    @staticmethod
    def forward(ctx, rays_o, rays_d, t, dirs, grid, mu, sigma, enc, mlp, *params):
        geom, dims = enc._geom(), mlp._dims()
        operand = ops.tc_operand()
        pts_c, ray_c, rowmap, count = ops.compact_samples(rays_o, rays_d, t, grid, mu, sigma)
        cur, side = torch.cuda.current_stream(), _side_stream(rays_o.device)
        flat = mlp._flat_params()
        side.wait_stream(cur)
        with torch.cuda.stream(side):
            ops.mlp_tc_prepare(flat, dims, operand)
        feat16 = ops.hash_encode_fwd_pts(pts_c, count, enc._flat_table(), geom, operand)
        cur.wait_stream(side)
        out, _ = ops.mlp_fwd_tc(feat16, dirs, 1, flat, dims, operand=operand, image_ready=True, n_dev=count, dir_rows=ray_c)
        ctx.enc, ctx.mlp, ctx.geom, ctx.dims, ctx.operand = enc, mlp, geom, dims, operand
        ctx.save_for_backward(pts_c, ray_c, count, dirs, feat16, out)
        ctx.want_tab = any(ctx.needs_input_grad[9:9 + enc.L])
        ctx.want_mlp = any(ctx.needs_input_grad[9 + enc.L:])
        ctx.g = None
        if ctx.want_tab:
            if enc._dp is not None:
                enc._dp.note_forward(enc)
            else:
                ctx.g = enc._zeroed_grad_async()
        if ctx.want_mlp and mlp._dp is not None:
            mlp._dp.note_forward(mlp)
        ctx.mark_non_differentiable(rowmap, count)
        return out, rowmap, count

    @staticmethod
    def backward(ctx, dout, _g_rowmap, _g_count):
        pts_c, ray_c, count, dirs, feat16, out = ctx.saved_tensors
        enc, mlp = ctx.enc, ctx.mlp
        L, T, F = enc.L, enc.T, enc.F
        flat = mlp._flat_params()
        dpm = mlp._dp if ctx.want_mlp else None
        if dpm is not None:
            dflat, last_m = dpm.enter_backward(mlp)
        else:
            dflat, last_m = torch.zeros_like(flat), False
        dfeat, ddirs = ops.mlp_bwd_tc(feat16, dirs, 1, flat, ctx.dims, out.detach(), dout.float().contiguous(), ctx.want_tab,
                                      ctx.needs_input_grad[3], dflat, operand=ctx.operand, grad_scale=mlp.tc_grad_scale,
                                      n_dev=count, dir_rows=ray_c)
        if dpm is not None and last_m:
            dpm.publish(mlp, dflat)
        gm = (None,) * len(mlp._ordered()) if (dpm is not None or not ctx.want_mlp) else tuple(mlp._grad_views(dflat))
        head = (None, None, None, ddirs, None, None, None, None, None)
        if not ctx.want_tab:
            return head + (None,) * L + gm
        dpe = enc._dp
        if dpe is not None:
            g, last = dpe.enter_backward(enc)
            ops.hash_encode_bwd_pts(pts_c, count, dfeat, ctx.geom, g, 0, L)
            if last:
                dpe.publish(enc, g)
            return head + (None,) * L + gm
        if ctx.g is not None:
            g, ev = ctx.g
            ctx.g = None
            torch.cuda.current_stream().wait_event(ev)
        else:
            g = torch.zeros((L, T, F), device=dout.device, dtype=torch.float32)
        ops.hash_encode_bwd_pts(pts_c, count, dfeat, ctx.geom, g, 0, L)
        return head + tuple(g[i] for i in range(L)) + gm


FUSE_SCATTER = os.environ.get("HBR_FUSE_SCATTER", "1") != "0"
FUSE_SCATTER_MAX_POINTS = 1 << 21
FUSE_GATHER = os.environ.get("HBR_FUSE_GATHER", "0") != "0"
FUSE_GATHER_MAX_POINTS = 1 << 21
STREAM_LEVEL_MAJOR = os.environ.get("HBR_STREAM_LEVEL_MAJOR", "0") != "0"

_SIDE = {}


def _side_stream(device) -> torch.cuda.Stream:
    dev = torch.device(device)
    idx = dev.index if dev.index is not None else torch.cuda.current_device()
    s = _SIDE.get(idx)
    if s is None:
        s = _SIDE[idx] = torch.cuda.Stream(device=idx)
    return s


def _field_params(enc, mlp):
    ps = [*[e.weight for e in enc.Embedding_list], *mlp._ordered()]
    return ps if torch.is_grad_enabled() else [p.detach() for p in ps]


RenderOut = namedtuple("RenderOut", "rgb_coarse rgb_fine depth_coarse depth_fine opacity_coarse opacity_fine norm")


def _unwrap(model):
    if isinstance(model, nn.DataParallel) and len(model.device_ids) <= 1:
        return model.module
    return model


class Volume_Renderer:
    def __init__(self, H, W, K, near=0., far=1., device=None, Pos_encode=None, Dir_encode=None, max_dim=1024,
                 sigma_val=torch.as_tensor(1), mu=torch.as_tensor(0), use_sdf: Optional[bool] = False,
                 var_model: Optional[nn.Module] = None):
        self.H, self.W, self.K = H, W, K
        self.near, self.far = near, far
        self.device = device
        if device is None:
            self.device = "cuda" if torch.cuda.is_available() else "cpu"
        self.coods_x, self.coords_y = torch.meshgrid(torch.arange(W, device=self.device), torch.arange(H, device=self.device),
                                                     indexing="xy")
        self.Pos_encode = Pos_encode
        self.Dir_encode = Dir_encode
        self.grid_size = max_dim // 4
        g = self.grid_size
        self.bool_grid = torch.ones((g, g, g), device=self.device, dtype=torch.bool)
        self.sigma_val = sigma_val.to(self.device)
        self.mu = mu.to(self.device)
        self.epislon = 1e-5
        self.tmp_arr = torch.zeros((g, g, g), device=self.device, dtype=torch.int8)
        self.reset_mask = False
        self.use_sdf = use_sdf
        self.var_model = var_model
        self._dp_checked = False
        self._grid_flags = None
        self.max_points = 1 << 26
        self.compact = False
        self._grid_state = (None, True)
        self._host_norm = None
        self.fuse_field = False
        self.chain_field = True
        self.ert = False
        self.sdf_native = True

    def update_grid(self, points: torch.Tensor, alpha: torch.Tensor):
        if points.is_cuda and self.bool_grid.is_cuda and self.mu.numel() in (1, 3):
            alpha[alpha <= 0] = 0
            mu, sig = self._norm_host()
            if self._grid_flags is None or self._grid_flags.device != self.bool_grid.device:
                self._grid_flags = torch.zeros(2, dtype=torch.int32, device=self.bool_grid.device)
            ops.occupancy_update(points, alpha, self.bool_grid, mu, sig, self._grid_flags)
            self._grid_state = (None, True)
            return
        points = (points - self.mu) / self.sigma_val
        points = (points * self.grid_size).long()
        alpha[alpha <= 0] = 0
        self.tmp_arr[points[..., 0], points[..., 1], points[..., 2]] += torch.ceil(alpha).int()
        if torch.sum(self.tmp_arr > 0) == 0:
            self.bool_grid[...] = True
        else:
            self.bool_grid[self.tmp_arr > 0] = True
        self.tmp_arr[self.tmp_arr > 0] = 0

    def _norm_host(self):
        if self._host_norm is None:
            mu = self.mu.detach().reshape(-1).float().cpu().tolist()
            if len(mu) == 1:
                mu = mu * 3
            self._host_norm = (mu, float(self.sigma_val.detach().cpu()))
        return self._host_norm

    @torch.no_grad()
    def update_grid_from_field(self, model, threshold: float = 0.01, chunk: int = 1 << 21, reset: bool = True):
        mlp = self._native(model)
        if mlp is None:
            raise TypeError("update_grid_from_field needs the native HashEncoder / MLP_3D")
        G = self.grid_size
        dev = self.bool_grid.device
        mu, sig = self._norm_host()
        if reset:
            self.bool_grid[...] = False
        idx = torch.arange(G, device=dev, dtype=torch.float32) + 0.5
        mu_t = torch.tensor(mu, device=dev)
        flat = self.bool_grid.view(-1)
        for i0 in range(0, G, max(1, chunk // (G * G))):
            i1 = min(G, i0 + max(1, chunk // (G * G)))
            ii, jj, kk = torch.meshgrid(idx[i0:i1], idx, idx, indexing="ij")
            p = torch.stack((ii, jj, kk), dim=-1).reshape(-1, 3) / G * sig + mu_t
            dens = mlp(self.Pos_encode(p))
            flat[i0 * G * G:i1 * G * G] |= dens.reshape(-1) > threshold
        self._grid_state = (None, True)
        return float(self.bool_grid.float().mean())

    def get_mask(self, points: torch.Tensor) -> torch.Tensor:
        mu, sig = self._norm_host()
        return ops.occupancy_mask(points, self.bool_grid, mu, sig)

    def _grid_all_true(self) -> bool:
        ver = self.bool_grid._version
        if self._grid_state[0] != (ver, self.bool_grid.data_ptr()):
            self._grid_state = ((ver, self.bool_grid.data_ptr()), bool(self.bool_grid.all()))
        return self._grid_state[1]

    def _native(self, model):
        m = _unwrap(model)
        ok = (isinstance(self.Pos_encode, HashEncoder) and isinstance(self.Dir_encode, PositionalEncoder)
              and isinstance(m, MLP_3D) and m._native and not m.use_sdf and not self.use_sdf)
        return m if ok else None

    def _can_fuse(self, mlp) -> bool:
        enc = self.Pos_encode
        if self.fuse_field is False or not (torch.is_autocast_enabled() and ops.HAS_TC):
            return False
        ok = (enc.F == 2 and enc.L == 16 and enc.E == 0 and enc.T >= 2 and (enc.T & (enc.T - 1)) == 0
              and mlp._in0 == 32 and mlp.d_view <= 25)
        if self.fuse_field == "auto":
            ok = ok and enc._dp is None
        return ok

    def _ert_tau(self) -> float:
        return ops.ERT_TAU if self.ert else 0.0

    def _can_chain(self, mlp) -> bool:
        enc = self.Pos_encode
        if not (self.chain_field and torch.is_autocast_enabled() and ops.HAS_TC):
            return False
        width = enc.L * enc.F + enc.E
        return width == mlp._in0 and (width % 2 == 0) and ((width == 32 and mlp.d_view <= 25) or width == 64)

    def _composite(self, out4, t, dir_norm, mask, R, S, rowmap=None, maps=False):
        if maps:
            return ops.CompositeMapsPacked.apply(out4, t, dir_norm, mask, R, S, self._ert_tau(), rowmap)
        return ops.CompositePacked.apply(out4, t, dir_norm, mask, R, S, self._ert_tau(), rowmap)

    def _field_pass(self, mlp, rays_o, rays_d, t, dir_enc, dir_norm, mask_needed, maps=False):
        R, S = rays_o.shape[0], t.shape[-1]
        if not self._can_fuse(mlp) and self._can_chain(mlp):
            enc = self.Pos_encode
            if enc._flat_table().device != rays_o.device:
                raise RuntimeError(f"encoder tables are on {enc._flat_table().device}, rays on {rays_o.device}")
            if mask_needed and self.compact and S <= 1024 and R * S < 2 ** 31:
                mu, sig = self._norm_host()
                out4, rowmap, _ = _FieldCompactFn.apply(rays_o, rays_d, t.float().contiguous(), dir_enc.float().contiguous(),
                                                        self.bool_grid, mu, sig, enc, mlp, *_field_params(enc, mlp))
                return self._composite(out4, t, dir_norm, None, R, S, rowmap, maps)
            mask = self.get_mask(ops.ray_points(rays_o, rays_d, t).view(-1, 3)) if mask_needed else None
            out4 = _FieldRaysFn.apply(rays_o, rays_d, t.float().contiguous(), dir_enc.float().contiguous(), enc, mlp,
                                      *_field_params(enc, mlp))
            return self._composite(out4, t, dir_norm, mask, R, S, None, maps)
        pts = ops.ray_points(rays_o, rays_d, t).view(-1, 3)
        mask = self.get_mask(pts) if mask_needed else None
        if self._can_fuse(mlp):
            enc = self.Pos_encode
            if enc._flat_table().device != pts.device:
                raise RuntimeError(f"encoder tables are on {enc._flat_table().device}, rays on {pts.device}")
            out4 = _FieldFn.apply(pts, dir_enc, S, enc, mlp, *_field_params(enc, mlp))
        else:
            feat = self.Pos_encode(pts)
            out4 = mlp.field(feat, dir_enc, S)
        return self._composite(out4, t, dir_norm, mask, R, S, None, maps)

    def vol_render(self, model, rays_d: torch.Tensor, rays_o: torch.Tensor, num_samples=100,
                   t: Optional[torch.Tensor] = None, update_mask=False, dir_norm=1, hierarchical=True,
                   _u=None, _u_cand=None) -> Tuple[torch.Tensor, torch.Tensor, Optional[torch.Tensor]]:
        if not rays_d.is_cuda:
            raise RuntimeError("Volume_Renderer.vol_render needs CUDA tensors (there is no CPU fallback)")
        near, far = self.near, self.far
        device = "cuda"
        if t is None:
            t = strat_sampler(near, far, num_samples, device=rays_d.device)
        if self.use_sdf and self.sdf_native and hierarchical is not True and update_mask is not True and t.shape[-1] <= 1024:
            sdf_mlp = self._native_sdf(model)
            if sdf_mlp is not None and self._grid_all_true():
                self._auto_dp(sdf_mlp)
                return self._render_sdf(sdf_mlp, rays_o, rays_d, t)
        mlp = self._native(model)
        if mlp is not None:
            self._auto_dp(mlp)
        if mlp is None:
            return self._generic(model, rays_d, rays_o, t, update_mask, dir_norm, hierarchical, _u, _u_cand)

        rays_o = rays_o.float().contiguous()
        rays_d = rays_d.float().contiguous()
        dir_enc = self.Dir_encode(rays_d)
        if update_mask is True:
            if self.reset_mask is True:
                self.bool_grid[...] = False
                self.reset_mask = False
            mask_needed = False
        else:
            mask_needed = not self._grid_all_true()
        R, S = rays_o.shape[0], t.shape[-1]
        per = max(1, int(self.max_points) // (S * (3 if hierarchical is True else 1)))
        if R > per:
            if hierarchical is True and _u is None:
                _u = torch.rand((R, S), device=rays_o.device)
                _u_cand = torch.rand(S, device=rays_o.device)
            dn_rows = torch.is_tensor(dir_norm) and dir_norm.numel() == R
            Crs, Cfs = [], []
            for r0 in range(0, R, per):
                sl = slice(r0, min(R, r0 + per))
                cr, cf = self._render_rays(mlp, rays_o[sl], rays_d[sl], t, dir_enc[sl], dir_norm[sl] if dn_rows else dir_norm,
                                           mask_needed, hierarchical, _u[sl] if _u is not None else None, _u_cand)
                Crs.append(cr)
                Cfs.append(cf)
            Cr = torch.cat(Crs)
            return Cr, (Cr if hierarchical is not True else torch.cat(Cfs)), None
        Cr, Cf = self._render_rays(mlp, rays_o, rays_d, t, dir_enc, dir_norm, mask_needed, hierarchical, _u, _u_cand)
        return Cr, Cf, None

    def render(self, model, rays_d: torch.Tensor, rays_o: torch.Tensor, num_samples=100, t: Optional[torch.Tensor] = None,
               dir_norm=1, hierarchical=True) -> RenderOut:
        if not rays_d.is_cuda:
            raise RuntimeError("Volume_Renderer.render needs CUDA tensors (there is no CPU fallback)")
        if t is None:
            t = strat_sampler(self.near, self.far, num_samples, device=rays_d.device)
        if self.use_sdf:
            sdf_mlp = self._native_sdf(model) if (self.sdf_native and hierarchical is not True and t.shape[-1] <= 1024) else None
            if sdf_mlp is None or not self._grid_all_true():
                raise TypeError("Volume_Renderer.render in SDF mode needs the native SDF route: HashEncoder / "
                                "PositionalEncoder / MLP_3D with the reference's VarModel, hierarchical=False, at most 1024 "
                                "samples and an all-True occupancy grid")
            self._auto_dp(sdf_mlp)
            Cr, w, norm = self._sdf_pass(sdf_mlp, rays_o, rays_d, t)
            D, A = (w * t).sum(-1), w.sum(-1)
            return RenderOut(Cr, Cr, D, D, A, A, norm)
        mlp = self._native(model)
        if mlp is None:
# ... 144 lines not shown
```

include/hbr.h:

```cpp
#ifndef HBR_B200_H_
#define HBR_B200_H_

#include <stdint.h>

#ifdef __cplusplus
extern "C" {
#endif

#define HBR_ABI_VERSION 2
#define HBR_MAX_LEVELS 32

typedef enum {
  HBR_OK = 0,
  HBR_ERR_ARG = -1,
  HBR_ERR_CUDA = -2,
  HBR_ERR_UNSUPPORTED = -3
} hbr_status;

typedef enum { HBR_F32 = 0, HBR_F16 = 1, HBR_U8 = 2, HBR_BF16 = 3 } hbr_dtype;

typedef struct {
  float mu[3];
  float sigma;
  int32_t L;
// ... 3 lines not shown
  float scale[HBR_MAX_LEVELS];
} hbr_hash_geom;

typedef struct {
  int32_t in0;
  int32_t d_view;
} hbr_mlp_dims;

int hbr_abi_version(void);
const char* hbr_last_error(void);
int64_t hbr_mlp_param_count(const hbr_mlp_dims* dims);
int64_t hbr_mlp_act_floats(void);

int hbr_hash_encode_fwd(const void* x, int x_dtype, int64_t n, const float* table,
                        const hbr_hash_geom* geom_host, float* y, int64_t y_stride, void* stream);

int hbr_hash_encode_bwd(const void* x, int x_dtype, int64_t n, const float* dy, int64_t dy_stride,
                        const hbr_hash_geom* geom_host, float* dtable, int level_begin, int level_end, void* stream);

int hbr_hash_encode_dx(const void* x, int x_dtype, int64_t n, const float* table, const hbr_hash_geom* geom_host,
                       const float* dy, int64_t dy_stride, float* dx, void* stream);

int hbr_hash_encode_fwd_rays(const float* rays_o, const float* rays_d, const float* t, int64_t t_ray_stride, int64_t R,
                             int64_t S, const float* table, const hbr_hash_geom* geom_host, void* y, int64_t y_stride,
                             int y_dtype, void* stream);
int hbr_hash_encode_bwd_rays(const float* rays_o, const float* rays_d, const float* t, int64_t t_ray_stride, int64_t R,
                             int64_t S, const float* dy, int64_t dy_stride, const hbr_hash_geom* geom_host, float* dtable,
                             int level_begin, int level_end, void* stream);

int64_t hbr_hash_bwd_stream_tiles(int64_t n);
int hbr_hash_encode_bwd_stream(const void* x, int x_dtype, int64_t n, const float* dy, int64_t dy_stride,
                               const hbr_hash_geom* geom_host, float* dtable, const int* level_bounds, int nchunks,
                               unsigned int* done, void* stream);
int hbr_hash_encode_bwd_rays_stream(const float* rays_o, const float* rays_d, const float* t, int64_t t_ray_stride, int64_t R,
                                    int64_t S, const float* dy, int64_t dy_stride, const hbr_hash_geom* geom_host,
                                    float* dtable, const int* level_bounds, int nchunks, unsigned int* done, void* stream);

int64_t hbr_hash_bwd_lm_ctas(int64_t n);
int hbr_hash_encode_bwd_lm(const void* x, int x_dtype, int64_t n, const float* dy_lm, const hbr_hash_geom* geom_host,
                           float* dtable, const int* level_bounds, int nchunks, unsigned int* done, void* stream);
int hbr_hash_encode_bwd_rays_lm(const float* rays_o, const float* rays_d, const float* t, int64_t t_ray_stride, int64_t R,
                                int64_t S, const float* dy_lm, const hbr_hash_geom* geom_host, float* dtable,
                                const int* level_bounds, int nchunks, unsigned int* done, void* stream);

int hbr_hash_indices(const void* x, int x_dtype, int64_t n, const hbr_hash_geom* geom_host,
                     int32_t* idx, float* w, void* stream);

int hbr_dir_encode(const void* d, int d_dtype, int64_t n, int dim, int num_freq, float* out, void* stream);

int hbr_mlp_fwd_f32(const float* feat, int64_t feat_stride, const float* dirs, int64_t dir_group, int64_t n,
                    const float* params, const hbr_mlp_dims* dims, float* out, float* act, void* stream);

int hbr_mlp_bwd_f32(const float* feat, int64_t feat_stride, const float* dirs, int64_t dir_group, int64_t n,
                    const float* params, const hbr_mlp_dims* dims, const float* dout, const float* act,
                    float* dz, float* dfeat, int64_t dfeat_stride, float* ddirs, float* dparams, void* stream);

int64_t hbr_mlp_tc_scratch_bytes(const hbr_mlp_dims* dims);
int hbr_mlp_tc_prepare(const float* params, const hbr_mlp_dims* dims, int operand, void* scratch, void* stream);
int hbr_mlp_tc_reduce_grads(const hbr_mlp_dims* dims, int64_t n, void* scratch, float* dparams, void* stream);
int hbr_mlp_fwd_tc(const void* feat, int feat_dtype, int64_t feat_stride, const float* dirs, int64_t dir_group, int64_t n,
                   const float* params, const hbr_mlp_dims* dims, int operand, float* out, void* scratch, int image_ready,
                   const unsigned long long* n_dev, const int32_t* dir_rows, void* stream);
#define HBR_DFEAT_LEVEL_MAJOR (-1)
int hbr_mlp_bwd_tc(const void* feat, int feat_dtype, int64_t feat_stride, const float* dirs, int64_t dir_group, int64_t n,
                   const float* params, const hbr_mlp_dims* dims, int operand, const float* out, const float* dout,
                   float* dfeat, int64_t dfeat_stride, float* ddirs, float* dparams, float grad_scale, void* scratch,
                   int image_ready, int defer_reduce, const unsigned long long* n_dev, const int32_t* dir_rows, void* stream);
int hbr_field_fwd_tc(const float* x, int64_t n, const float* table, const hbr_hash_geom* geom_host, const float* dirs,
                     int64_t dir_group, const float* params, const hbr_mlp_dims* dims, int operand, float* out,
                     void* feat16, void* scratch, void* stream);
int hbr_field_bwd_tc(const float* x, int64_t n, const hbr_hash_geom* geom_host, const float* dirs, int64_t dir_group,
                     const float* params, const hbr_mlp_dims* dims, int operand, const void* feat16, const float* out,
                     const float* dout, float* dtable, float* ddirs, float* dparams, float grad_scale, void* scratch,
                     void* stream);
int hbr_field_fwd_rays_tc(const float* rays_o, const float* rays_d, const float* t, int64_t t_ray_stride, int64_t R, int64_t S,
                          const float* table, const hbr_hash_geom* geom_host, const float* dirs, const float* params,
                          const hbr_mlp_dims* dims, int operand, float* out, void* feat16, void* scratch, int image_ready,
                          void* stream);
int hbr_field_bwd_rays_tc(const void* feat16, const float* rays_o, const float* rays_d, const float* t, int64_t t_ray_stride,
                          int64_t R, int64_t S, const hbr_hash_geom* geom_host, const float* dirs, const float* params,
                          const hbr_mlp_dims* dims, int operand, const float* out, const float* dout, float* dtable,
                          float* ddirs, float* dparams, float grad_scale, void* scratch, int image_ready, int defer_reduce,
                          void* stream);
int hbr_strat_depths(const float* lin, const float* u, float span, float count, int64_t S, float* t, void* stream);

int hbr_mse_pair_fwd(const float* a, const float* b, const float* gt, int64_t n, float scale, float* loss, void* stream);
int hbr_mse_pair_bwd(const float* a, const float* b, const float* gt, int64_t n, float scale, const float* gout, float* da,
                     float* db, void* stream);

int hbr_ray_points(const float* rays_o, const float* rays_d, const float* t, int64_t t_ray_stride,
                   int64_t R, int64_t S, float* pts, void* stream);

int hbr_occupancy_mask(const float* pts, int64_t n, const uint8_t* grid, int G, const float* mu3_host,
                       float sigma, uint8_t* mask, void* stream);

int hbr_occupancy_update(const float* pts, int64_t n, const float* alpha, int64_t alpha_stride, uint8_t* grid, int G,
                         const float* mu3_host, float sigma, unsigned int* flags2, void* stream);
int hbr_compact_samples(const float* rays_o, const float* rays_d, const float* t, int64_t t_ray_stride, int64_t R, int64_t S,
                        const uint8_t* grid, int G, const float* mu3_host, float sigma, float* pts_c, int32_t* ray_c,
                        int32_t* rowmap, unsigned long long* count, void* stream);
int hbr_hash_encode_fwd_pts(const float* x, int64_t n_max, const unsigned long long* n_dev, const float* table,
                            const hbr_hash_geom* geom_host, void* y, int64_t y_stride, int y_dtype, void* stream);
int hbr_hash_encode_bwd_pts(const float* x, int64_t n_max, const unsigned long long* n_dev, const float* dy, int64_t dy_stride,
                            const hbr_hash_geom* geom_host, float* dtable, int level_begin, int level_end, void* stream);

int hbr_composite_fwd(const float* t, int64_t t_ray_stride, const float* rgb, int64_t rgb_stride,
                      const float* sigma, int64_t sigma_stride, const float* dir_norm, float dir_norm_scalar,
                      const uint8_t* mask, const int32_t* rowmap, int64_t R, int64_t S, float* C, float* w, float ert_tau,
                      void* stream);
int hbr_composite_bwd(const float* t, int64_t t_ray_stride, const float* rgb, int64_t rgb_stride,
                      const float* sigma, int64_t sigma_stride, const float* dir_norm, float dir_norm_scalar,
                      const uint8_t* mask, const int32_t* rowmap, int64_t R, int64_t S, const float* gC,
                      float* drgb, int64_t drgb_stride, float* dsigma, int64_t dsigma_stride, float ert_tau,
                      void* stream);
int hbr_composite_maps_fwd(const float* t, int64_t t_ray_stride, const float* rgb, int64_t rgb_stride,
                           const float* sigma, int64_t sigma_stride, const float* dir_norm, float dir_norm_scalar,
                           const uint8_t* mask, const int32_t* rowmap, int64_t R, int64_t S, float* C, float* w,
                           float* depth, float* opacity, float ert_tau, void* stream);
int hbr_composite_maps_bwd(const float* t, int64_t t_ray_stride, const float* rgb, int64_t rgb_stride,
                           const float* sigma, int64_t sigma_stride, const float* dir_norm, float dir_norm_scalar,
                           const uint8_t* mask, const int32_t* rowmap, int64_t R, int64_t S, const float* gC,
                           const float* gD, const float* gA, float* drgb, int64_t drgb_stride, float* dsigma,
                           int64_t dsigma_stride, float ert_tau, void* stream);

int hbr_hier_sample(float* w, const float* t, const float* u, const float* cand, int64_t R, int64_t S,
                    int clamp_in_place, float* t_fine, void* stream);

int hbr_composite_sdf_fwd(const float* rgb, int64_t rgb_stride, const float* sdf, int64_t sdf_stride, int from_density,
                          const float* b, int64_t R, int64_t S, float* C, float* w, void* stream);
int hbr_composite_sdf_bwd(const float* rgb, int64_t rgb_stride, const float* sdf, int64_t sdf_stride, int from_density,
                          const float* b, int64_t R, int64_t S, const float* gC, const float* gw, float* drgb,
                          int64_t drgb_stride, float* dsdf, int64_t dsdf_stride, float* db_ray, void* stream);
int hbr_sdf_stencil_points(const float* x, int64_t n, float eps, const float* lo3_host, const float* hi3_host, float* pts,
                           void* stream);
int hbr_sdf_eikonal_fwd(const float* dens6, int64_t n, float eps, float* norm, float* grads, void* stream);
int hbr_sdf_eikonal_bwd(const float* dens6, int64_t n, float eps, const float* gnorm, float* ddens6, void* stream);

int hbr_grid_points(const double* min3_host, const double* max3_host, int res, int64_t p0, int64_t count,
                    void* pts_f16, void* stream);
int hbr_grid_density(const double* min3_host, const double* max3_host, int res, int64_t p0, int64_t count,
                     const float* table, const hbr_hash_geom* geom_host, const float* params,
                     const hbr_mlp_dims* dims, const float* dir_enc, float* out, void* pts_scratch,
                     float* feat_scratch, int64_t chunk, int field_mode, void* stream);
int hbr_mlp_density_tf32x3(const float* feat, int64_t n, const float* params, const hbr_mlp_dims* dims, float* out,
                           void* stream);

int hbr_mc_count(const float* density, int n0, int n1, int n2, float iso, int i_begin, int i_end,
                 unsigned long long* counts, void* stream);
int hbr_mc_emit(const float* density, int n0, int n1, int n2, float iso, int i_begin, int i_end,
                int32_t* edge_id, float* verts, int64_t max_verts, int32_t* faces, int64_t max_faces,
                unsigned long long* cursors, void* stream);

int hbr_grid_interp(const float* vol, int C, int n0, int n1, int n2, const float* pts, int64_t n, float* out, void* stream);

int hbr_adam_step(float* param, const float* grad, float* exp_avg, float* exp_avg_sq, int64_t n, double lr, double beta1,
                  double beta2, double eps, double weight_decay, int decoupled_weight_decay, int64_t step,
                  double inv_scale, const float* found_inf, void* stream);
int hbr_adam_tick(long long* step_dev, const float* found_inf, void* stream);
int hbr_adam_step_dev(float* param, const float* grad, float* exp_avg, float* exp_avg_sq, int64_t n, const float* lr_dev,
                      double beta1, double beta2, double eps, double weight_decay, int decoupled_weight_decay,
                      const long long* step_dev, double inv_scale, const float* grad_scale_dev, const float* found_inf,
                      void* stream);

int hbr_ray_gen(const float* c2w, int64_t n_views, int H, int W, float fx, float fy, float cx, float cy,
                const int64_t* ray_ids, int64_t first, int64_t n_rays, const void* images, int image_dtype, float* rays_o,
                float* rays_d, float* dir_norm, float* gt, int* bad_id, void* stream);
// ... 25 lines not shown
```

Measured before the change: 8.797 million.

## Fold volume compositing into tensor-core MLP forward and backward kernels

Adds fused entry points that run the ray compositor, meaning transmittance scan, weights and colour accumulation, inside the tcgen05 MLP forward kernel, and fold the compositor backward into the fused field backward kernel. The scan runs per 128-thread group using named barriers and shared-memory scratch. This removes the separate composite forward and backward launches and the round trip of the per-sample sigma/rgb outputs and their gradients through global memory. The path is enabled by default when S is 32, 64 or 128 and no mask or maps are needed. The cost is extra barriers and shared memory in the MLP kernels, and the rounding order changes slightly because explicit _rn intrinsics are used.

Result: slower. 8.523 million, median of 6 (-3.1%).

```diff
diff --git a/human_body_reconstruction_b200/_lib.py b/human_body_reconstruction_b200/_lib.py
--- a/human_body_reconstruction_b200/_lib.py
+++ b/human_body_reconstruction_b200/_lib.py
@@ -154,6 +154,10 @@
                                _vp, _i32, _i32, _vp], C.c_int),
     "hbr_field_fwd_rays_tc": ([_vp, _vp, _vp, _i64, _i64, _i64, _vp, _geom_p, _vp, _vp, _dims_p, _i32, _vp, _vp, _vp, _i32, _vp],
                               C.c_int),
+    "hbr_mlp_fwd_tc_composite": ([_vp, _vp, _vp, _dims_p, _i32, _vp, _i64, _i64, _i64, _vp, _f32, _vp, _vp, _vp, _vp, _i32, _vp],
+                                 C.c_int),
+    "hbr_field_bwd_rays_tc_composite": ([_vp, _vp, _vp, _vp, _i64, _i64, _i64, _geom_p, _vp, _vp, _dims_p, _i32, _vp, _vp, _vp,
+                                         _f32, _vp, _vp, _vp, _f32, _vp, _i32, _i32, _vp], C.c_int),
     "hbr_hash_encode_bwd_rays": ([_vp, _vp, _vp, _i64, _i64, _i64, _vp, _i64, _geom_p, _vp, _i32, _i32, _vp], C.c_int),
     "hbr_field_fwd_tc": ([_vp, _i64, _vp, _geom_p, _vp, _i64, _vp, _dims_p, _i32, _vp, _vp, _vp, _vp], C.c_int),
     "hbr_field_bwd_tc": ([_vp, _i64, _geom_p, _vp, _i64, _vp, _dims_p, _i32, _vp, _vp, _vp, _vp, _vp, _vp, _f32, _vp, _vp],
@@ -217,7 +221,7 @@
 
 KERNELS_PER_CALL = {
     "hbr_hash_encode_fwd": 1, "hbr_hash_encode_bwd": 1, "hbr_hash_encode_dx": 1, "hbr_hash_encode_fwd_rays": 1, "hbr_hash_encode_bwd_rays": 1, "hbr_hash_indices": 1, "hbr_dir_encode": 1,
-    "hbr_mlp_fwd_f32": 1, "hbr_mlp_bwd_f32": 2, "hbr_mlp_fwd_tc": 2, "hbr_mlp_bwd_tc": 3, "hbr_field_fwd_tc": 2, "hbr_field_bwd_tc": 3, "hbr_field_bwd_rays_tc": 3, "hbr_field_fwd_rays_tc": 1, "hbr_adam_step": 1, "hbr_adam_tick": 1, "hbr_adam_step_dev": 1, "hbr_allreduce_peer": 1, "hbr_allreduce_peer_stream": 1, "hbr_hash_encode_bwd_stream": 1, "hbr_hash_encode_bwd_rays_stream": 1, "hbr_hash_encode_bwd_lm": 1, "hbr_hash_encode_bwd_rays_lm": 1, "hbr_ray_gen": 1, "hbr_ray_bbox": 1, "hbr_ray_points": 1, "hbr_occupancy_mask": 1, "hbr_occupancy_update": 2, "hbr_compact_samples": 1, "hbr_hash_encode_fwd_pts": 1, "hbr_hash_encode_bwd_pts": 1,
+    "hbr_mlp_fwd_f32": 1, "hbr_mlp_bwd_f32": 2, "hbr_mlp_fwd_tc": 2, "hbr_mlp_bwd_tc": 3, "hbr_field_fwd_tc": 2, "hbr_field_bwd_tc": 3, "hbr_field_bwd_rays_tc": 3, "hbr_field_fwd_rays_tc": 1, "hbr_mlp_fwd_tc_composite": 2, "hbr_field_bwd_rays_tc_composite": 3, "hbr_adam_step": 1, "hbr_adam_tick": 1, "hbr_adam_step_dev": 1, "hbr_allreduce_peer": 1, "hbr_allreduce_peer_stream": 1, "hbr_hash_encode_bwd_stream": 1, "hbr_hash_encode_bwd_rays_stream": 1, "hbr_hash_encode_bwd_lm": 1, "hbr_hash_encode_bwd_rays_lm": 1, "hbr_ray_gen": 1, "hbr_ray_bbox": 1, "hbr_ray_points": 1, "hbr_occupancy_mask": 1, "hbr_occupancy_update": 2, "hbr_compact_samples": 1, "hbr_hash_encode_fwd_pts": 1, "hbr_hash_encode_bwd_pts": 1,
     "hbr_composite_fwd": 1, "hbr_composite_bwd": 1, "hbr_composite_maps_fwd": 1, "hbr_composite_maps_bwd": 1, "hbr_strat_depths": 1, "hbr_mse_pair_fwd": 1, "hbr_mse_pair_bwd": 1, "hbr_mlp_tc_prepare": 1, "hbr_mlp_tc_reduce_grads": 1, "hbr_hier_sample": 1, "hbr_grid_points": 1,
     "hbr_composite_sdf_fwd": 1, "hbr_composite_sdf_bwd": 1, "hbr_sdf_stencil_points": 1, "hbr_sdf_eikonal_fwd": 1, "hbr_sdf_eikonal_bwd": 1,
     "hbr_grid_density": 3, "hbr_mlp_density_tf32x3": 1, "hbr_mc_count": 1, "hbr_mc_emit": 2, "hbr_grid_interp": 1,
diff --git a/human_body_reconstruction_b200/csrc/composite.cu b/human_body_reconstruction_b200/csrc/composite.cu
--- a/human_body_reconstruction_b200/csrc/composite.cu
+++ b/human_body_reconstruction_b200/csrc/composite.cu
@@ -1,4 +1,5 @@
 #include "common.cuh"
+#include "composite_math.cuh"
 #include <math_constants.h>
 
 namespace hbr {
@@ -57,11 +58,6 @@
   o[nf + k] = c;
 }
 
-struct SampleIn {
-  float delta, sig, p;
-  bool keep;
-};
-
 __device__ __forceinline__ long long sample_row(const int32_t* __restrict__ rowmap, long long gs, int s, int S) {
   return rowmap == nullptr ? gs : (s < S ? (long long)__ldg(rowmap + gs) : -1);
 }
@@ -69,16 +65,8 @@
 __device__ __forceinline__ SampleIn load_sample(const float* __restrict__ tr, const float* __restrict__ sigma,
                                                 long long sig_st, const uint8_t* __restrict__ mask, long long gs,
                                                 int s, int S, float dnr, bool& live, long long row) {
-  SampleIn q;
   live = s < S && row >= 0 && (mask == nullptr || mask[gs]);
-  float delta = 0.f;
-  if (s + 1 < S) delta = __fsub_rn(__ldg(tr + s + 1), __ldg(tr + s));
-  q.delta = __fmul_rn(delta, dnr);
-  const float raw = live ? __ldg(sigma + row * sig_st) : 0.f;
-  q.keep = !(raw < -10.f);
-  q.sig = q.keep ? raw : -10.f;
-  q.p = s < S ? __fmul_rn(q.sig, q.delta) : 0.f;
-  return q;
+  return sample_terms(tr, s, S, dnr, live ? __ldg(sigma + row * sig_st) : 0.f);
 }
 
 template <bool MAPS>
@@ -100,12 +88,10 @@
     bool live;
     const long long row = sample_row(rowmap, gs, s, S);
     const SampleIn q = load_sample(tr, sigma, sig_st, mask, gs, s, S, dnr, live, row);
-    const float incl = carry + warp_incl_scan(q.p, lane);
+    const float incl = chunk_incl(carry, q.p, lane);
     float prev = __shfl_up_sync(kFull, incl, 1);
     if (lane == 0) prev = carry;
-    const float T = s == 0 ? 1.f : expf(-prev);
-    const float alpha = 1.f - expf(-q.p);
-    const float w = s < S ? __fmul_rn(T, alpha) : 0.f;
+    const float w = s < S ? sample_weight(transmittance(s, prev), q.p) : 0.f;
     if (s < S) {
       if (w_out) w_out[gs] = w;
       if (MAPS) {
@@ -114,9 +100,9 @@
       }
       if (live) {
         const float* c = rgb + row * rgb_st;
-        c0 += w * __ldg(c + 0);
-        c1 += w * __ldg(c + 1);
-        c2 += w * __ldg(c + 2);
+        c0 = colour_acc(c0, w, __ldg(c + 0));
+        c1 = colour_acc(c1, w, __ldg(c + 1));
+        c2 = colour_acc(c2, w, __ldg(c + 2));
       }
     }
     carry = __shfl_sync(kFull, incl, 31);
@@ -169,16 +155,16 @@
       bool live;
       const long long row = sample_row(rowmap, gs, s, S);
       const SampleIn q = load_sample(tr, sigma, sig_st, mask, gs, s, S, dnr, live, row);
-      const float incl = carry + warp_incl_scan(q.p, lane);
+      const float incl = chunk_incl(carry, q.p, lane);
       float prev = __shfl_up_sync(kFull, incl, 1);
       if (lane == 0) prev = carry;
       carry = __shfl_sync(kFull, incl, 31);
       if (s < S) {
-        Tk[i] = s == 0 ? 1.f : expf(-prev);
+        Tk[i] = transmittance(s, prev);
         ek[i] = expf(-q.p);
         if (live) {
           const float* c = rgb + row * rgb_st;
-          ck[i] = g0 * __ldg(c + 0) + g1 * __ldg(c + 1) + g2 * __ldg(c + 2);
+          ck[i] = colour_dot(g0, g1, g2, __ldg(c + 0), __ldg(c + 1), __ldg(c + 2));
           dk[i] = q.keep ? q.delta : 0.f;
         }
         if (MAPS) ck[i] = __fadd_rn(__fmaf_rn(gd, __ldg(tr + s), ck[i]), ga);
@@ -192,19 +178,18 @@
     if (i * 32 < S) {
       const int s = i * 32 + lane;
       const long long gs = ray * S + s;
-      const float w = Tk[i] * (1.f - ek[i]);
-      const float wc = w * ck[i];
-      const float rin = warp_rincl_scan(wc, lane);
+      const float w = bwd_weight(Tk[i], ek[i]);
+      const float rin = warp_rincl_scan(__fmul_rn(w, ck[i]), lane);
       float after = __shfl_down_sync(kFull, rin, 1);
       if (lane == 31) after = 0.f;
-      const float suffix = rcarry + after;
-      rcarry += __shfl_sync(kFull, rin, 0);
+      const float suffix = __fadd_rn(rcarry, after);
+      rcarry = __fadd_rn(rcarry, __shfl_sync(kFull, rin, 0));
       if (s < S) {
         const long long row = sample_row(rowmap, gs, s, S);
         const bool live = row >= 0 && (mask == nullptr || mask[gs]);
-        const float dp = Tk[i] * ek[i] * ck[i] - suffix;
-        const float ds = live ? dk[i] * dp : 0.f;
-        const float r0 = live ? w * g0 : 0.f, r1 = live ? w * g1 : 0.f, r2 = live ? w * g2 : 0.f;
+        const float dp = bwd_dp(bwd_te(Tk[i], ek[i]), ck[i], suffix);
+        const float ds = live ? __fmul_rn(dk[i], dp) : 0.f;
+        const float r0 = live ? __fmul_rn(w, g0) : 0.f, r1 = live ? __fmul_rn(w, g1) : 0.f, r2 = live ? __fmul_rn(w, g2) : 0.f;
         if (row >= 0) {
           if (packed) {
             *reinterpret_cast<float4*>(drgb + row * 4) = make_float4(r0, r1, r2, ds);
diff --git a/human_body_reconstruction_b200/csrc/composite_math.cuh b/human_body_reconstruction_b200/csrc/composite_math.cuh
--- /dev/null
+++ b/human_body_reconstruction_b200/csrc/composite_math.cuh
@@ -0,0 +1,155 @@
+#pragma once
+#include "common.cuh"
+
+namespace hbr {
+
+struct SampleIn {
+  float delta, sig, p;
+  bool keep;
+};
+
+__device__ __forceinline__ float sample_delta(const float* __restrict__ tr, int s, int S, float dnr) {
+  float delta = 0.f;
+  if (s + 1 < S) delta = __fsub_rn(__ldg(tr + s + 1), __ldg(tr + s));
+  return __fmul_rn(delta, dnr);
+}
+__device__ __forceinline__ SampleIn sample_from_delta(float delta, int s, int S, float raw) {
+  SampleIn q;
+  q.delta = delta;
+  q.keep = !(raw < -10.f);
+  q.sig = q.keep ? raw : -10.f;
+  q.p = s < S ? __fmul_rn(q.sig, q.delta) : 0.f;
+  return q;
+}
+__device__ __forceinline__ SampleIn sample_terms(const float* __restrict__ tr, int s, int S, float dnr, float raw) {
+  return sample_from_delta(sample_delta(tr, s, S, dnr), s, S, raw);
+}
+
+__device__ __forceinline__ float chunk_incl(float carry, float p, int lane) { return __fadd_rn(carry, warp_incl_scan(p, lane)); }
+
+__device__ __forceinline__ float transmittance(int s, float prev) { return s == 0 ? 1.f : expf(-prev); }
+
+__device__ __forceinline__ float sample_weight(float T, float p) { return __fmul_rn(T, 1.f - expf(-p)); }
+
+__device__ __forceinline__ float colour_acc(float acc, float w, float c) { return __fmaf_rn(w, c, acc); }
+
+__device__ __forceinline__ float colour_dot(float g0, float g1, float g2, float c0, float c1, float c2) {
+  return __fmaf_rn(g2, c2, __fmaf_rn(g0, c0, __fmul_rn(g1, c1)));
+}
+__device__ __forceinline__ float bwd_weight(float T, float e) { return __fmul_rn(T, __fsub_rn(1.f, e)); }
+__device__ __forceinline__ float bwd_te(float T, float e) { return __fmul_rn(T, e); }
+__device__ __forceinline__ float bwd_dp(float te, float c, float suffix) { return __fmaf_rn(te, c, -suffix); }
+
+struct CompArgs {
+  const float* t;
+  long long t_stride;
+  const float* dn;
+  float dn_scalar;
+  int S;
+  float* C;
+  float* w;
+  const float* gC;
+};
+constexpr int kCompScratchFloats = 8 + 128 * 4;
+
+__device__ __forceinline__ void group_bar(int bar) { asm volatile("bar.sync %0, 128;" ::"r"(bar) : "memory"); }
+
+struct CompPos {
+  long long ray;
+  int s, k, k0, nch;
+};
+__device__ __forceinline__ CompPos comp_pos(const CompArgs& c, long long gp, int r) {
+  CompPos q;
+  const int sh = __ffs(c.S) - 1;
+  q.ray = gp >> sh;
+  q.s = r & (c.S - 1);
+  q.k = r >> 5;
+  q.nch = c.S >> 5;
+  q.k0 = q.k & ~(q.nch - 1);
+  return q;
+}
+
+struct CompPre {
+  float delta, g0, g1, g2;
+};
+__device__ __forceinline__ CompPre comp_preload(const CompArgs& c, long long gp, bool valid, int r, bool with_grad) {
+  CompPre p{0.f, 0.f, 0.f, 0.f};
+  if (valid) {
+    const CompPos q = comp_pos(c, gp, r);
+    p.delta = sample_delta(c.t + q.ray * c.t_stride, q.s, c.S, c.dn ? __ldg(c.dn + q.ray) : c.dn_scalar);
+    if (with_grad) { p.g0 = __ldg(c.gC + q.ray * 3 + 0); p.g1 = __ldg(c.gC + q.ray * 3 + 1); p.g2 = __ldg(c.gC + q.ray * 3 + 2); }
+  }
+  return p;
+}
+
+__device__ __forceinline__ SampleIn group_scan(const CompArgs& c, const CompPos& q, bool valid, float delta, float sigma, int lane,
+                                               float* scr, int bar, float& prev) {
+  SampleIn in{0.f, 0.f, 0.f, true};
+  if (valid) in = sample_from_delta(delta, q.s, c.S, sigma);
+  const float scan = warp_incl_scan(in.p, lane);
+  if (lane == 31) scr[q.k] = scan;
+  group_bar(bar);
+  float carry = 0.f;
+  for (int j = q.k0; j < q.k; ++j) carry = __fadd_rn(carry, scr[j]);
+  const float incl = __fadd_rn(carry, scan);
+  prev = __shfl_up_sync(kFull, incl, 1);
+  if (lane == 0) prev = carry;
+  return in;
+}
+
+__device__ __forceinline__ void composite_group_fwd(const CompArgs& c, long long gp, bool valid, int r, int lane, float4 o,
+                                                    const CompPre& pre, float* scr, int bar) {
+  const CompPos q = comp_pos(c, gp, r);
+  float prev;
+  const SampleIn in = group_scan(c, q, valid, pre.delta, o.w, lane, scr, bar, prev);
+  const float w = sample_weight(transmittance(q.s, prev), in.p);
+  if (valid && c.w != nullptr) c.w[gp] = w;
+  float4* pw = reinterpret_cast<float4*>(scr + 8);
+  pw[r] = make_float4(w, o.x, o.y, o.z);
+  group_bar(bar);
+  if (valid && q.s < 32) {
+    float c0 = 0.f, c1 = 0.f, c2 = 0.f;
+    for (int j = 0; j < q.nch; ++j) {
+      const float4 v = pw[r + 32 * j];
+      c0 = colour_acc(c0, v.x, v.y);
+      c1 = colour_acc(c1, v.x, v.z);
+      c2 = colour_acc(c2, v.x, v.w);
+    }
+    c0 = warp_sum(c0); c1 = warp_sum(c1); c2 = warp_sum(c2);
+    if (lane == 0) { c.C[q.ray * 3 + 0] = c0; c.C[q.ray * 3 + 1] = c1; c.C[q.ray * 3 + 2] = c2; }
+  }
+}
+
+struct CompBwd {
+  float te, ck, after, dk, r0, r1, r2;
+  int k, kend;
+};
+__device__ __forceinline__ CompBwd composite_group_bwd_scan(const CompArgs& c, long long gp, bool valid, int r, int lane,
+                                                             float4 o, const CompPre& pre, float* scr, int bar) {
+  const CompPos q = comp_pos(c, gp, r);
+  float prev;
+  const SampleIn in = group_scan(c, q, valid, pre.delta, o.w, lane, scr, bar, prev);
+  CompBwd b;
+  const float g0 = pre.g0, g1 = pre.g1, g2 = pre.g2;
+  const float T = transmittance(q.s, prev), e = expf(-in.p);
+  b.ck = colour_dot(g0, g1, g2, o.x, o.y, o.z);
+  const float w = bwd_weight(T, e);
+  b.te = bwd_te(T, e);
+  b.r0 = __fmul_rn(w, g0); b.r1 = __fmul_rn(w, g1); b.r2 = __fmul_rn(w, g2);
+  b.dk = in.keep ? in.delta : 0.f;
+  const float rin = warp_rincl_scan(__fmul_rn(w, b.ck), lane);
+  b.after = __shfl_down_sync(kFull, rin, 1);
+  if (lane == 31) b.after = 0.f;
+  if (lane == 0) scr[4 + q.k] = rin;
+  b.k = q.k;
+  b.kend = q.k0 + q.nch;
+  return b;
+}
+__device__ __forceinline__ float4 composite_group_bwd_finish(const CompBwd& b, const float* scr, int bar) {
+  group_bar(bar);
+  float rcarry = 0.f;
+  for (int j = b.kend - 1; j > b.k; --j) rcarry = __fadd_rn(rcarry, scr[4 + j]);
+  return make_float4(b.r0, b.r1, b.r2, __fmul_rn(b.dk, bwd_dp(b.te, b.ck, __fadd_rn(rcarry, b.after))));
+}
+
+}
diff --git a/human_body_reconstruction_b200/csrc/debug/mlp_tc_debug.cu b/human_body_reconstruction_b200/csrc/debug/mlp_tc_debug.cu
--- a/human_body_reconstruction_b200/csrc/debug/mlp_tc_debug.cu
+++ b/human_body_reconstruction_b200/csrc/debug/mlp_tc_debug.cu
@@ -57,7 +57,7 @@
   if (sc != nullptr) mlp_prep_kernel<32, 48><<<kPrepCtas, 256, 0, as_stream(stream)>>>(params, 32, 24, sc);
   mlp_bwd_tc_kernel<32, 48, 2, true><<<grid, 2 * kTile + 32, smem, as_stream(stream)>>>(
       feat, 32, dirs, dir_group, n, params, 32, 24, out, dout, dfeat, 32, nullptr, dparams, sc,
-      sc != nullptr ? reinterpret_cast<float*>(sc + SC::off_grad) : nullptr, trace, EncArgs{}, HashGeom{}, 1.f, 0, nullptr, nullptr);
+      sc != nullptr ? reinterpret_cast<float*>(sc + SC::off_grad) : nullptr, trace, EncArgs{}, HashGeom{}, 1.f, 0, nullptr, nullptr, CompArgs{});
   HBR_LAUNCH_CHECK();
   return HBR_OK;
 }
@@ -68,7 +68,7 @@
   HBR_CUDA(cudaFuncSetAttribute(mlp_fwd_tc_kernel<32, 48, 4, true>, cudaFuncAttributeMaxDynamicSharedMemorySize, smem));
   const int grid = (int)min64(ceil_div(ceil_div(n, kTile), 4), sm_count());
   mlp_fwd_tc_kernel<32, 48, 4, true><<<grid, 4 * kTile, smem, as_stream(stream)>>>(
-      feat, 32, dirs, dir_group, n, params, 32, 24, out, nullptr, trace, EncArgs{}, HashGeom{}, 0, nullptr, nullptr);
+      feat, 32, dirs, dir_group, n, params, 32, 24, out, nullptr, trace, EncArgs{}, HashGeom{}, 0, nullptr, nullptr, CompArgs{});
   HBR_LAUNCH_CHECK();
   return HBR_OK;
 }
diff --git a/human_body_reconstruction_b200/csrc/mlp_tc.cu b/human_body_reconstruction_b200/csrc/mlp_tc.cu
--- a/human_body_reconstruction_b200/csrc/mlp_tc.cu
+++ b/human_body_reconstruction_b200/csrc/mlp_tc.cu
@@ -218,3 +218,60 @@
                                                             to_device_geom(*geom), grad_scale, 1, image_ready, defer_reduce,
                                                             nullptr, nullptr, as_stream(stream)));
 }
+
+static int check_comp(const float* t, int64_t t_ray_stride, int64_t R, int64_t S) {
+  HBR_REQUIRE(S == 32 || S == 64 || S == 128, "S=%lld: the compositor fold needs S in {32, 64, 128}", (long long)S);
+  HBR_REQUIRE(R >= 0 && R < (1LL << 40) / S, "R=%lld", (long long)R);
+  HBR_REQUIRE(t != nullptr && (t_ray_stride == 0 || t_ray_stride >= S), "t / t_ray_stride %lld", (long long)t_ray_stride);
+  return HBR_OK;
+}
+static CompArgs comp_args(const float* t, int64_t t_ray_stride, int64_t S, const float* dn, float dn_scalar) {
+  CompArgs c{};
+  c.t = t; c.t_stride = t_ray_stride; c.S = (int)S; c.dn = dn; c.dn_scalar = dn_scalar;
+  return c;
+}
+
+extern "C" int hbr_mlp_fwd_tc_composite(const void* feat16, const float* dirs, const float* params, const hbr_mlp_dims* dims,
+                                        int operand, const float* t, int64_t t_ray_stride, int64_t R, int64_t S, const float* dn,
+                                        float dn_scalar, float* out, float* C, float* w, void* scratch, int image_ready,
+                                        void* stream) {
+  if (int rc = check_dims(dims)) return rc;
+  if (int rc = check_operand(operand, 1.f)) return rc;
+  if (int rc = check_comp(t, t_ray_stride, R, S)) return rc;
+  HBR_REQUIRE(narrow_shape(dims) && dims->in0 == 32, "the compositor fold covers in0 = 32, d_view <= 25");
+  const int64_t n = R * S;
+  if (n == 0) return HBR_OK;
+  HBR_REQUIRE(feat16 && dirs && params && out && C, "NULL pointer");
+  HBR_REQUIRE((uintptr_t)feat16 % 16 == 0 && (uintptr_t)out % 16 == 0 && (uintptr_t)scratch % 256 == 0, "alignment");
+  CompArgs c = comp_args(t, t_ray_stride, S, dn, dn_scalar);
+  c.C = C; c.w = w;
+  return HBR_BY_OPERAND(launch_fwd_tc<32, 48, 4, false, true>(static_cast<const float*>(feat16), 32, dirs, S, n, params, 32,
+                                                              dims->d_view, out, static_cast<uint8_t*>(scratch), EncArgs{},
+                                                              HashGeom{}, 1, image_ready, nullptr, nullptr, as_stream(stream), c));
+}
+
+extern "C" int hbr_field_bwd_rays_tc_composite(const void* feat16, const float* rays_o, const float* rays_d, const float* t,
+                                               int64_t t_ray_stride, int64_t R, int64_t S, const hbr_hash_geom* geom,
+                                               const float* dirs, const float* params, const hbr_mlp_dims* dims, int operand,
+                                               const float* out, const float* gC, const float* dn, float dn_scalar, float* dtable,
+                                               float* ddirs, float* dparams, float grad_scale, void* scratch, int image_ready,
+                                               int defer_reduce, void* stream) {
+  if (int rc = check_field(geom, dims)) return rc;
+  if (int rc = check_operand(operand, grad_scale)) return rc;
+  if (int rc = check_comp(t, t_ray_stride, R, S)) return rc;
+  HBR_REQUIRE(!defer_reduce || (scratch != nullptr && dparams != nullptr), "defer_reduce needs scratch and dparams");
+  const int64_t n = R * S;
+  if (n == 0) return HBR_OK;
+  HBR_REQUIRE(feat16 && rays_o && rays_d && dirs && params && out && gC && dtable, "NULL pointer");
+  HBR_REQUIRE((uintptr_t)out % 16 == 0 && (uintptr_t)dtable % 16 == 0 && (uintptr_t)feat16 % 16 == 0 &&
+                  (uintptr_t)scratch % 256 == 0, "alignment");
+  EncArgs e{};
+  e.dtable = dtable; e.ro = rays_o; e.rd = rays_d; e.rt = t; e.S = S; e.t_stride = t_ray_stride;
+  CompArgs c = comp_args(t, t_ray_stride, S, dn, dn_scalar);
+  c.gC = gC;
+  return HBR_BY_OPERAND(launch_bwd_tc<32, 48, 1, false, 11, true>(static_cast<const float*>(feat16), 32, dirs, S, n, params, 32,
+                                                                  dims->d_view, out, nullptr, nullptr, 32, ddirs, dparams,
+                                                                  static_cast<uint8_t*>(scratch), e, to_device_geom(*geom),
+                                                                  grad_scale, 1, image_ready, defer_reduce, nullptr, nullptr,
+                                                                  as_stream(stream), c));
+}
diff --git a/human_body_reconstruction_b200/csrc/mlp_tc_impl.cuh b/human_body_reconstruction_b200/csrc/mlp_tc_impl.cuh
--- a/human_body_reconstruction_b200/csrc/mlp_tc_impl.cuh
+++ b/human_body_reconstruction_b200/csrc/mlp_tc_impl.cuh
@@ -1,3 +1,4 @@
+#include "composite_math.cuh"
 #ifndef HBR_OP
 #error "define HBR_OP (tc::OpBf16 | tc::OpF16) and HBR_OPNS before including mlp_tc_impl.cuh"
 #endif
@@ -579,7 +580,7 @@
   }
 }
 
-template <int K0P, int KCP, int G>
+template <int K0P, int KCP, int G, bool COMP = false>
 struct FwdSmem {
   static constexpr int off_bias = WOfs<K0P, KCP>::total;
   static constexpr int off_ones16 = off_bias + BOfs::total;
@@ -589,7 +590,8 @@
   static constexpr int stage_bytes = K0P == 32 ? kTile * K0P * 4 : 0;
   static constexpr int off_bar = off_stage + G * stage_bytes;
   static constexpr int off_xbar = off_bar + 2 * G * 8 + 16;
-  static constexpr int total = off_xbar + 4 * G * 8;
+  static constexpr int off_comp = (off_xbar + 4 * G * 8 + 15) & ~15;
+  static constexpr int total = off_comp + (COMP ? G * kCompScratchFloats * 4 : 0);
   static_assert(total <= 232448, "shared memory budget exceeded");
 };
 
@@ -707,15 +709,15 @@
   cp_async_commit();
 }
 
-template <int K0P, int KCP, int G, bool TRACE = false, bool ENC = false, int GATH = 0>
+template <int K0P, int KCP, int G, bool TRACE = false, bool ENC = false, int GATH = 0, bool COMP = false>
 __global__ void __launch_bounds__(G * kTile + GATH * 32, 1)
 mlp_fwd_tc_kernel(const float* __restrict__ feat, long long feat_stride, const float* __restrict__ dirs, long long dir_group,
                   long long n_arg, const float* __restrict__ params, int in0, int dv, float* __restrict__ out,
                   const uint8_t* __restrict__ image, long long* __restrict__ trace, const EncArgs enc,
                   const __grid_constant__ HashGeom geom, int feat16, const unsigned long long* __restrict__ n_dev,
-                  const int32_t* __restrict__ dir_rows) {
+                  const int32_t* __restrict__ dir_rows, const CompArgs comp) {
   const long long n = n_dev != nullptr ? min(n_arg, (long long)__ldg(n_dev)) : n_arg;
-  using SM = FwdSmem<K0P, KCP, G>;
+  using SM = FwdSmem<K0P, KCP, G, COMP>;
   using WO = WOfs<K0P, KCP>;
   constexpr int kGrpCols = 96;
   constexpr int kCols = G * kGrpCols <= 128 ? 128 : (G * kGrpCols <= 256 ? 256 : 512);
@@ -858,6 +860,9 @@
       const bool valid = gp < n;
       const long long dir_row = valid ? (dir_rows != nullptr ? (long long)__ldg(dir_rows + gp) : gp / dir_group) : 0;
       if (valid && lane == 0) prefetch_l1(dirs + dir_row * dv);
+      CompPre cpre;
+      if constexpr (COMP) cpre = comp_preload(comp, gp, valid, r, false);
+      (void)cpre;
       TR();
       uint32_t xofs = 0;
       if (GATH > 0) {
@@ -918,14 +923,14 @@
       HBR_TS_LAYER(5, w5, 16, 64);
       float c16[16];
       tmem_ld<16>(taddr, c16);
-      if (valid) {
-        float4 o;
-        o.x = elu1(c16[0]);
-        o.y = elu1(c16[1]);
-        o.z = elu1(c16[2]);
-        o.w = density;
-        *reinterpret_cast<float4*>(out + gp * 4) = o;
-      }
+      float4 o;
+      o.x = elu1(c16[0]);
+      o.y = elu1(c16[1]);
+      o.z = elu1(c16[2]);
+      o.w = density;
+      if (valid) *reinterpret_cast<float4*>(out + gp * 4) = o;
+      if constexpr (COMP)
+        composite_group_fwd(comp, gp, valid, r, lane, o, cpre, reinterpret_cast<float*>(sm + SM::off_comp) + g * kCompScratchFloats, 1 + g);
     }
 #undef HBR_TS_LAYER
 #undef HBR_LAYER
@@ -974,7 +979,7 @@
   }
 }
 
-template <int K0P, int KCP, int G>
+template <int K0P, int KCP, int G, bool COMP = false>
 struct BwdSmem {
   static constexpr bool kAliasDzs = KCP == 48;
   static constexpr int off_bias = WOfs<K0P, KCP>::total;
@@ -992,7 +997,8 @@
   static constexpr int off_ring = off_grp + G * grp_bytes;
   static constexpr int off_bar = off_ring + (G == 1 && K0P == 32 ? ring_slots * ring_slot : 0);
   static constexpr int off_pos = off_bar + (4 * G + 2 * ring_slots) * 8 + 16;
-  static constexpr int total = off_pos + 2 * kTile * 3 * 4;
+  static constexpr int off_comp = off_pos + 2 * kTile * 3 * 4;
+  static constexpr int total = off_comp + (COMP ? G * 8 * 4 : 0);
   static_assert(total <= 232448, "shared memory budget exceeded");
 };
 
@@ -1087,7 +1093,7 @@
 __host__ __device__ constexpr int scat_regs(int G) { return G == 2 ? 88 : 112; }
 
 
-template <int K0P, int KCP, int G, bool TRACE = false, bool ENC = false, int SCAT = 0>
+template <int K0P, int KCP, int G, bool TRACE = false, bool ENC = false, int SCAT = 0, bool COMP = false>
 __global__ void __launch_bounds__(G * kTile + SCAT * 32 + 32, 1)
 mlp_bwd_tc_kernel(const float* __restrict__ feat, long long feat_stride, const float* __restrict__ dirs, long long dir_group,
                   long long n_arg, const float* __restrict__ params, int in0, int dv, const float* __restrict__ out,
@@ -1095,10 +1101,10 @@
                   float* __restrict__ ddirs, float* __restrict__ dparams, const uint8_t* __restrict__ image,
                   float* __restrict__ grad_rows, long long* __restrict__ trace, const EncArgs enc,
                   const __grid_constant__ HashGeom geom, float gscale, int feat16, const unsigned long long* __restrict__ n_dev,
-                  const int32_t* __restrict__ dir_rows) {
+                  const int32_t* __restrict__ dir_rows, const CompArgs comp) {
   const long long n = n_dev != nullptr ? min(n_arg, (long long)__ldg(n_dev)) : n_arg;
   const float ginv = 1.f / gscale;
-  using SM = BwdSmem<K0P, KCP, G>;
+  using SM = BwdSmem<K0P, KCP, G, COMP>;
   using WO = WOfs<K0P, KCP>;
   constexpr int kGrpCols = 96;
   using TM = BwdTmem<K0P, KCP, 2 * kGrpCols>;
@@ -1436,11 +1442,16 @@
       const long long dir_row = valid ? (dir_rows != nullptr ? (long long)__ldg(dir_rows + gp) : gp / dir_group) : 0;
       if (valid && lane == 0) prefetch_l1(dirs + dir_row * dv);
       float4 fo = make_float4(0.f, 0.f, 0.f, 0.f), go = fo;
-      if (valid) {
-        fo = __ldg(reinterpret_cast<const float4*>(out + gp * 4));
+      if (valid) fo = __ldg(reinterpret_cast<const float4*>(out + gp * 4));
+      if (!COMP && valid) {
         go = __ldg(reinterpret_cast<const float4*>(dout + gp * 4));
         go.x *= gscale; go.y *= gscale; go.z *= gscale; go.w *= gscale;
       }
+      float* cscr = reinterpret_cast<float*>(sm + SM::off_comp) + g * 8;
+      CompBwd cb;
+      CompPre cpre;
+      if constexpr (COMP) cpre = comp_preload(comp, gp, valid, r, true);
+      (void)cscr; (void)cb; (void)cpre;
       float pt[3] = {0.f, 0.f, 0.f};
       if (ENC) {
         if (valid) { pt[0] = __ldg(enc.x + gp * 3 + 0); pt[1] = __ldg(enc.x + gp * 3 + 1); pt[2] = __ldg(enc.x + gp * 3 + 2); }
@@ -1466,7 +1477,7 @@
         else if (!stage_ok && !f16in) prefetch_l2(feat + ((tile + nslots) * kTile + r) * feat_stride);
         if ((r & 7) == 0) {
           prefetch_l2(out + ((tile + nslots) * kTile + r) * 4);
-          prefetch_l2(dout + ((tile + nslots) * kTile + r) * 4);
+          if (!COMP) prefetch_l2(dout + ((tile + nslots) * kTile + r) * 4);
         }
       }
       uint4 dzt[8];
@@ -1500,10 +1511,17 @@
         else tmem_st16(taddr_a + 16, p + 16);
         tmem_st_wait();
       }
-      HBR_BSTAGE(false, issue_fwd_ts(tgrp, tgrp_a, wa + WO::w3 / 16, 64, KCP, false));
+      HBR_BSTAGE_T(issue_fwd_ts(tgrp, tgrp_a, wa + WO::w3 / 16, 64, KCP, false),
+                   { if constexpr (COMP) cb = composite_group_bwd_scan(comp, gp, valid, r, lane, fo, cpre, cscr, 1 + g); });
       relu_bias_to_tmem64(taddr, bias + 192, taddr_a, dzt);
       HBR_BSTAGE_T(issue_fwd_ts(tgrp, tgrp_a, wa + WO::w4 / 16, 64, 64, false),
-                   { store_tile64(r, c1, dzt); });
+                   {
+                     store_tile64(r, c1, dzt);
+                     if constexpr (COMP) {
+                       go = composite_group_bwd_finish(cb, cscr, 1 + g);
+                       if (valid) { go.x *= gscale; go.y *= gscale; go.z *= gscale; go.w *= gscale; }
+                     }
+                   });
       relu_bias_to_tmem64(taddr, bias + 256, 0xffffffffu, dzt);
       {
         float dz16[16];
@@ -1641,18 +1659,18 @@
 
 static inline bool narrow_shape(const hbr_mlp_dims* d) { return d->in0 <= 32 && d->d_view + kFeat <= 40; }
 
-template <int K0P, int KCP, int G, bool ENC>
+template <int K0P, int KCP, int G, bool ENC, bool COMP = false>
 static int launch_fwd_tc(const float* feat, int64_t feat_stride, const float* dirs, int64_t dir_group, int64_t n,
                          const float* params, int in0, int dv, float* out, uint8_t* scratch, const EncArgs& enc,
                          const HashGeom& geom, int feat16, int image_ready, const unsigned long long* n_dev, const int32_t* dir_rows,
-                         cudaStream_t st) {
-  constexpr int smem = FwdSmem<K0P, KCP, G>::total;
+                         cudaStream_t st, const CompArgs& comp = CompArgs{}) {
+  constexpr int smem = FwdSmem<K0P, KCP, G, COMP>::total;
   const int grid = (int)min64(ceil_div(ceil_div(n, kTile), G), sm_count());
   if (scratch != nullptr && !image_ready) mlp_prep_kernel<K0P, KCP><<<kPrepCtas, 256, 0, st>>>(params, in0, dv, scratch);
-  auto kern = mlp_fwd_tc_kernel<K0P, KCP, G, false, ENC>;
+  auto kern = mlp_fwd_tc_kernel<K0P, KCP, G, false, ENC, 0, COMP>;
   HBR_CUDA(cudaFuncSetAttribute(kern, cudaFuncAttributeMaxDynamicSharedMemorySize, smem));
   kern<<<grid, G * kTile, smem, st>>>(feat, feat_stride, dirs, dir_group, n, params, in0, dv, out, scratch, nullptr, enc,
-                                             geom, feat16, n_dev, dir_rows);
+                                             geom, feat16, n_dev, dir_rows, comp);
   HBR_LAUNCH_CHECK();
   return HBR_OK;
 }
@@ -1666,23 +1684,24 @@
   auto kern = mlp_fwd_tc_kernel<32, 48, G, false, false, GATH>;
   HBR_CUDA(cudaFuncSetAttribute(kern, cudaFuncAttributeMaxDynamicSharedMemorySize, smem));
   kern<<<grid, G * kTile + GATH * 32, smem, st>>>(nullptr, 32, dirs, dir_group, n, params, 32, dv, out, image, nullptr, enc, geom,
-                                                  1, nullptr, nullptr);
+                                                  1, nullptr, nullptr, CompArgs{});
   HBR_LAUNCH_CHECK();
   return HBR_OK;
 }
 
-template <int K0P, int KCP, int G, bool ENC, int SCAT = 0>
+template <int K0P, int KCP, int G, bool ENC, int SCAT = 0, bool COMP = false>
 static int launch_bwd_tc(const float* feat, int64_t feat_stride, const float* dirs, int64_t dir_group, int64_t n,
                          const float* params, int in0, int dv, const float* out, const float* dout, float* dfeat,
                          int64_t dfeat_stride, float* ddirs, float* dparams, uint8_t* scratch, const EncArgs& enc,
                          const HashGeom& geom, float gscale, int feat16, int image_ready, int defer_reduce,
-                         const unsigned long long* n_dev, const int32_t* dir_rows, cudaStream_t st) {
+                         const unsigned long long* n_dev, const int32_t* dir_rows, cudaStream_t st,
+                         const CompArgs& comp = CompArgs{}) {
   using SC = Scratch<K0P, KCP>;
-  constexpr int smem = BwdSmem<K0P, KCP, G>::total;
+  constexpr int smem = BwdSmem<K0P, KCP, G, COMP>::total;
   const int grid = (int)min64(ceil_div(ceil_div(n, kTile), G), sm_count());
   const bool rows = scratch != nullptr && dparams != nullptr && grid <= SC::kMaxRows;
   if (scratch != nullptr && !image_ready) mlp_prep_kernel<K0P, KCP><<<kPrepCtas, 256, 0, st>>>(params, in0, dv, scratch);
-  auto kern = mlp_bwd_tc_kernel<K0P, KCP, G, false, ENC, SCAT>;
+  auto kern = mlp_bwd_tc_kernel<K0P, KCP, G, false, ENC, SCAT, COMP>;
   HBR_CUDA(cudaFuncSetAttribute(kern, cudaFuncAttributeMaxDynamicSharedMemorySize, smem));
   if constexpr (SCAT > 0) {
     static_assert((G == 2 && SCAT == 7) || (G == 1 && SCAT == 11), "register budget: 16 warps, 4 per sub-partition");
@@ -1698,7 +1717,8 @@
   }
   kern<<<grid, G * kTile + SCAT * 32 + 32, smem, st>>>(feat, feat_stride, dirs, dir_group, n, params, in0, dv, out, dout, dfeat,
                                            dfeat_stride, ddirs, dparams, scratch,
-                                           rows ? reinterpret_cast<float*>(scratch + SC::off_grad) : nullptr, nullptr, enc, geom, gscale, feat16, n_dev, dir_rows);
+                                           rows ? reinterpret_cast<float*>(scratch + SC::off_grad) : nullptr, nullptr, enc, geom, gscale, feat16, n_dev, dir_rows,
+                                           comp);
   if (rows && !defer_reduce) {
     const int total = make_layout(in0, dv).total;
     mlp_grad_reduce_kernel<<<dim3((total + 255) / 256, kReduceSlices), 256, 0, st>>>(
diff --git a/human_body_reconstruction_b200/ops.py b/human_body_reconstruction_b200/ops.py
--- a/human_body_reconstruction_b200/ops.py
+++ b/human_body_reconstruction_b200/ops.py
@@ -738,6 +738,42 @@
     return ddirs
 
 
+def mlp_fwd_tc_composite(feat16, dirs, params, dims: MlpDims, t, dir_norm, R: int, S: int, operand: int = HBR_BF16,
+                         image_ready: bool = False):
+    require_cuda(feat16, dirs, params, t)
+    dev = feat16.device
+    out = torch.empty((R * S, 4), device=dev, dtype=torch.float32)
+    Cc = torch.empty((R, 3), device=dev, dtype=torch.float32)
+    w = torch.empty((R, S), device=dev, dtype=torch.float32)
+    dn, dns = _dn_args(dir_norm, R, dev)
+    scratch = mlp_tc_scratch(dims, dev)
+    ready = 1 if (image_ready and _tc_image.get(id(scratch)) == _image_key(params, operand)) else 0
+    check(lib().hbr_mlp_fwd_tc_composite(ptr(feat16), ptr(dirs), ptr(params), C.byref(dims), operand, ptr(t), _t_stride(t, S), R, S,
+                                         ptr(dn), dns, ptr(out), ptr(Cc), ptr(w), ptr(scratch), ready, stream()))
+    if ready:
+        _lib.STATS.launches -= 1
+    _tc_image[id(scratch)] = _image_key(params, operand)
+    return out, Cc, w
+
+
+def field_bwd_rays_tc_composite(feat16, rays_o, rays_d, t, geom: HashGeom, dirs, params, dims: MlpDims, out, gC, dir_norm,
+                                dtable, want_ddirs, dparams, operand: int = HBR_BF16, grad_scale: float = 1.0):
+    require_cuda(feat16, rays_o, rays_d, t, dirs, params, out, gC, dtable)
+    R, S = rays_o.shape[0], t.shape[-1]
+    dn, dns = _dn_args(dir_norm, R, feat16.device)
+    ddirs = torch.zeros_like(dirs) if want_ddirs else None
+    scratch = mlp_tc_scratch(dims, feat16.device)
+    key = _image_key(params, operand)
+    ready = 1 if _tc_image.get(id(scratch)) == key else 0
+    check(lib().hbr_field_bwd_rays_tc_composite(ptr(feat16), ptr(rays_o), ptr(rays_d), ptr(t), _t_stride(t, S), R, S,
+                                                C.byref(geom), ptr(dirs), ptr(params), C.byref(dims), operand, ptr(out), ptr(gC),
+                                                ptr(dn), dns, ptr(dtable), ptr(ddirs), ptr(dparams), float(grad_scale),
+                                                ptr(scratch), ready, 0, stream()))
+    _lib.STATS.launches -= ready
+    _tc_image[id(scratch)] = key
+    return ddirs
+
+
 def field_scatter_supported(geom: HashGeom, dims: MlpDims) -> bool:
     T = int(geom.T)
     return (geom.F == 2 and geom.L == 16 and geom.E == 0 and T >= 2 and (T & (T - 1)) == 0 and dims.in0 == 32
diff --git a/human_body_reconstruction_b200/vol_renderer.py b/human_body_reconstruction_b200/vol_renderer.py
--- a/human_body_reconstruction_b200/vol_renderer.py
+++ b/human_body_reconstruction_b200/vol_renderer.py
@@ -175,6 +175,43 @@
         return (None, None, None, ddirs, None, None) + tuple(g[i] for i in range(L)) + gm
 
 
+class _FieldRaysCompositeFn(torch.autograd.Function):
+
+    @staticmethod
+    def forward(ctx, rays_o, rays_d, t, dirs, dir_norm, enc, mlp, *params):
+        geom, dims = enc._geom(), mlp._dims()
+        operand = ops.tc_operand()
+        R, S = rays_o.shape[0], t.shape[-1]
+        cur, side = torch.cuda.current_stream(), _side_stream(rays_o.device)
+        flat = mlp._flat_params()
+        side.wait_stream(cur)
+        with torch.cuda.stream(side):
+            ops.mlp_tc_prepare(flat, dims, operand)
+        feat16 = ops.hash_encode_fwd_rays(rays_o, rays_d, t, enc._flat_table(), geom, operand)
+        cur.wait_stream(side)
+        out, Cc, w = ops.mlp_fwd_tc_composite(feat16, dirs, flat, dims, t, dir_norm, R, S, operand=operand, image_ready=True)
+        ctx.enc, ctx.mlp, ctx.geom, ctx.dims, ctx.operand = enc, mlp, geom, dims, operand
+        ctx.dn_scalar = None if torch.is_tensor(dir_norm) else dir_norm
+        ctx.save_for_backward(rays_o, rays_d, t, dirs, dir_norm if torch.is_tensor(dir_norm) else None, feat16, out)
+        ctx.g = enc._zeroed_grad_async()
+        ctx.mark_non_differentiable(w)
+        return Cc, w
+
+    @staticmethod
+    def backward(ctx, gC, _gw):
+        rays_o, rays_d, t, dirs, dn, feat16, out = ctx.saved_tensors
+        enc, mlp = ctx.enc, ctx.mlp
+        flat = mlp._flat_params()
+        dflat = torch.zeros_like(flat)
+        g, ev = ctx.g
+        ctx.g = None
+        torch.cuda.current_stream().wait_event(ev)
+        ddirs = ops.field_bwd_rays_tc_composite(feat16, rays_o, rays_d, t, ctx.geom, dirs, flat, ctx.dims, out,
+                                                gC.float().contiguous(), dn if dn is not None else ctx.dn_scalar, g,
+                                                ctx.needs_input_grad[3], dflat, operand=ctx.operand, grad_scale=mlp.tc_grad_scale)
+        return (None, None, None, ddirs, None, None, None) + tuple(g[i] for i in range(enc.L)) + tuple(mlp._grad_views(dflat))
+
+
 class _FieldCompactFn(torch.autograd.Function):
 
     @staticmethod
@@ -246,6 +283,7 @@
 FUSE_SCATTER_MAX_POINTS = 1 << 21
 FUSE_GATHER = os.environ.get("HBR_FUSE_GATHER", "0") != "0"
 FUSE_GATHER_MAX_POINTS = 1 << 21
+FOLD_COMPOSITE = os.environ.get("HBR_FOLD_COMPOSITE", "1") != "0"
 STREAM_LEVEL_MAJOR = os.environ.get("HBR_STREAM_LEVEL_MAJOR", "0") != "0"
 
 _SIDE = {}
@@ -393,6 +431,15 @@
         width = enc.L * enc.F + enc.E
         return width == mlp._in0 and (width % 2 == 0) and ((width == 32 and mlp.d_view <= 25) or width == 64)
 
+    def _can_fold_composite(self, mlp, R, S) -> bool:
+        enc = self.Pos_encode
+        if not (FOLD_COMPOSITE and FUSE_SCATTER and not FUSE_GATHER and S in (32, 64, 128) and not self.ert
+                and R * S <= FUSE_SCATTER_MAX_POINTS and torch.is_grad_enabled() and enc._dp is None and mlp._dp is None):
+            return False
+        if not (any(e.weight.requires_grad for e in enc.Embedding_list) and any(p.requires_grad for p in mlp._ordered())):
+            return False
+        return ops.field_scatter_supported(enc._geom(), mlp._dims())
+
     def _composite(self, out4, t, dir_norm, mask, R, S, rowmap=None, maps=False):
         if maps:
             return ops.CompositeMapsPacked.apply(out4, t, dir_norm, mask, R, S, self._ert_tau(), rowmap)
@@ -409,6 +456,9 @@
                 out4, rowmap, _ = _FieldCompactFn.apply(rays_o, rays_d, t.float().contiguous(), dir_enc.float().contiguous(),
                                                         self.bool_grid, mu, sig, enc, mlp, *_field_params(enc, mlp))
                 return self._composite(out4, t, dir_norm, None, R, S, rowmap, maps)
+            if not mask_needed and not maps and self._can_fold_composite(mlp, R, S):
+                return _FieldRaysCompositeFn.apply(rays_o, rays_d, t.float().contiguous(), dir_enc.float().contiguous(), dir_norm,
+                                                   enc, mlp, *_field_params(enc, mlp))
             mask = self.get_mask(ops.ray_points(rays_o, rays_d, t).view(-1, 3)) if mask_needed else None
             out4 = _FieldRaysFn.apply(rays_o, rays_d, t.float().contiguous(), dir_enc.float().contiguous(), enc, mlp,
                                       *_field_params(enc, mlp))
diff --git a/include/hbr.h b/include/hbr.h
--- a/include/hbr.h
+++ b/include/hbr.h
@@ -109,6 +109,14 @@
                           const hbr_mlp_dims* dims, int operand, const float* out, const float* dout, float* dtable,
                           float* ddirs, float* dparams, float grad_scale, void* scratch, int image_ready, int defer_reduce,
                           void* stream);
+int hbr_mlp_fwd_tc_composite(const void* feat16, const float* dirs, const float* params, const hbr_mlp_dims* dims, int operand,
+                             const float* t, int64_t t_ray_stride, int64_t R, int64_t S, const float* dn, float dn_scalar,
+                             float* out, float* C, float* w, void* scratch, int image_ready, void* stream);
+int hbr_field_bwd_rays_tc_composite(const void* feat16, const float* rays_o, const float* rays_d, const float* t,
+                                    int64_t t_ray_stride, int64_t R, int64_t S, const hbr_hash_geom* geom_host, const float* dirs,
+                                    const float* params, const hbr_mlp_dims* dims, int operand, const float* out, const float* gC,
+                                    const float* dn, float dn_scalar, float* dtable, float* ddirs, float* dparams, float grad_scale,
+                                    void* scratch, int image_ready, int defer_reduce, void* stream);
 int hbr_strat_depths(const float* lin, const float* u, float span, float count, int64_t S, float* t, void* stream);
 
 int hbr_mse_pair_fwd(const float* a, const float* b, const float* gt, int64_t n, float scale, float* loss, void* stream);
```
